# jatinagwal/kyverno

Measured on AMD Instinct MI355X. Metric: resource×rule evals/sec (background scan, PSS+best-practices) at 1/2/4/8 GPUs, higher is better.
Workload: dtype u32

## Files before the change

### __graft_entry__.py

```python
import os
import subprocess
import sys

ROOT = os.path.dirname(os.path.abspath(__file__))
if ROOT not in sys.path:
    sys.path.insert(0, ROOT)


def build():
    from kyverno_amd import build as B
    B.build()
    subprocess.run(["make", "-C", os.path.join(ROOT, "oracle"), "-j8"], check=True)
    import kyverno_amd
    from kyverno_amd import _lib
    _lib.lib()
    try:
        import concurrent.futures
        cache = os.path.join(ROOT, "kyverno_amd", "jitcache")
        jobs = [(wl, a) for wl in ("c3", "tests-c3", "c5", "c4", "c2") for a in (False, True)]
        try:
            sys.path.insert(0, os.path.join(ROOT, "tests"))
            import table_edge_cases
            jobs += [("tests-edges:%d" % i, False) for i in range(len(table_edge_cases.compiled_rulesets()))]
            import meta_keys_cases
            jobs += [("tests-metakeys%s:%d" % (off, i), a) for i in range(len(meta_keys_cases.compiled_rulesets()))
                     for off in ("", "-off") for a in (False, True)]
            import cond_preload_cases
            jobs += [("tests-condpre%s:%d" % (off, i), a) for i in range(len(cond_preload_cases.compiled_rulesets()))
                     for off in ("", "-off") for a in (False, True)]
            import pattern_vars_cases
            jobs += [("tests-patvars:%d" % i, False) for i in range(len(pattern_vars_cases.compiled_rulesets()))]
        except Exception as e:
            print("build: test rulesets not compiled ahead of time: %s" % e, file=sys.stderr)
        ctx = __import__("multiprocessing").get_context("spawn")
        with concurrent.futures.ProcessPoolExecutor(max_workers=min(len(jobs), os.cpu_count() or 1, 16), mp_context=ctx) as ex:
            list(ex.map(_aot_compile, jobs))
        t_start = {}
        ents = [f for f in os.listdir(cache) if f.endswith(".co")]
        for kind in ("walk", "acct"):
            newest = max((f for f in ents if f.startswith(kind + "-")), key=lambda f: os.path.getmtime(os.path.join(cache, f)))
            t_start[kind] = newest.split("-")[1]
        for f in os.listdir(cache):
            parts = f.split("-")
            if f.endswith(".co") and (len(parts) != 3 or t_start.get(parts[0]) != parts[1]):
                os.remove(os.path.join(cache, f))
    except Exception as e:
        print("build: ahead-of-time walk-kernel compile skipped: %s" % e, file=sys.stderr)
    try:
        _cache_bench_corpus()
    except Exception as e:
        print("build: bench corpus not prebuilt: %s" % e, file=sys.stderr)


def _cache_bench_corpus(total=10_000_000, need_free=14 << 30):
    import shutil
    import bench
    from kyverno_amd import synth
    if synth.corpus_is_cached(bench.CORPUS_CACHE, total, kind="mixed", seed=bench.SEED):
        return
    os.makedirs(bench.CORPUS_CACHE, exist_ok=True)
    free = shutil.disk_usage(bench.CORPUS_CACHE).free
    if free < need_free:
        raise RuntimeError("%.0f GB free under %s, %.0f GB wanted" % (free / 2**30, bench.CORPUS_CACHE, need_free / 2**30))
    synth.write_corpus_cache(bench.CORPUS_CACHE, total, kind="mixed", seed=bench.SEED)


def _aot_compile(job):
    if ROOT not in sys.path:
        sys.path.insert(0, ROOT)
    sys.path.insert(0, os.path.join(ROOT, "tests"))
    import bench
    import cases
    from kyverno_amd import engine as E
    wl, acct = job
    if wl.startswith("tests-edges:"):
        import table_edge_cases
        pols = table_edge_cases.compiled_rulesets()[int(wl.split(":")[1])]
    elif wl.startswith("tests-metakeys"):
        import meta_keys_cases
        pols = meta_keys_cases.compiled_rulesets()[int(wl.split(":")[1])]
        if wl.startswith("tests-metakeys-off:"):
            os.environ["KYV_META_KEYS"] = "0"
            try:
                return E.Ruleset(pols).jit_compile(accounting=acct)
            finally:
                del os.environ["KYV_META_KEYS"]
    elif wl.startswith("tests-patvars:"):
        import pattern_vars_cases
        pols = pattern_vars_cases.compiled_rulesets()[int(wl.split(":")[1])]
    elif wl.startswith("tests-condpre"):
        import cond_preload_cases
        pols = cond_preload_cases.compiled_rulesets()[int(wl.split(":")[1])]
        if wl.startswith("tests-condpre-off:"):
            os.environ["KYV_JC_PRELOAD"] = "0"
            try:
                return E.Ruleset(pols).jit_compile(accounting=acct)
            finally:
                del os.environ["KYV_JC_PRELOAD"]
    else:
        pols = cases.best_practices() + cases.chart_restricted() if wl == "tests-c3" else bench.load_policies(wl)
    return E.Ruleset(pols).jit_compile(accounting=acct)


def smoke():
    sys.path.insert(0, os.path.join(ROOT, "tests"))
    import cases
    import parity_util as PU
    from kyverno_amd import synth

    docs, nsl = synth.mixed(300, seed=5, edge=True)
    pols = cases.best_practices()[:4] + cases.chart_restricted()[:6] + cases.quirk_policies()[-2:]
    st, res = PU.compare(pols, docs, nsl, backend="gpu")
    if st["nbad"]:
        raise AssertionError("GPU verdicts differ from the oracle: %r" % (st["bad"][:5],))
    if st["compared"] == 0:
        raise AssertionError("smoke compared no pairs")
    print("smoke ok: %d pairs, %d compared bit-exact vs oracle, kernel %.3f ms" % (st["pairs"], st["compared"],
                                                                                   res.kernel_ms))


if __name__ == "__main__":
    build() if (len(sys.argv) > 1 and sys.argv[1] == "build") else smoke()
# ... 1 lines not shown
```

### include/kyvgpu.h

```cpp
#ifndef KYVGPU_H
#define KYVGPU_H

#include <stddef.h>
#include <stdint.h>

#ifdef __cplusplus
extern "C" {
#endif

#define KYV_ABI_VERSION 1u

typedef struct kyv_ruleset kyv_ruleset;
typedef struct kyv_batch kyv_batch;
typedef struct kyv_results kyv_results;

enum { KYV_OK = 0, KYV_EINVAL = 1, KYV_EPARSE = 2, KYV_EDEVICE = 3, KYV_EINTERNAL = 4, KYV_ERANGE = 5 };

enum {
  KYV_ST_NONE = 0,
  KYV_ST_PASS = 1,
  KYV_ST_FAIL = 2,
  KYV_ST_SKIP = 3,
  KYV_ST_ERROR = 4,
  KYV_ST_FALLBACK = 5,
// ... 59 lines not shown
  uint32_t path_template;
  uint16_t idx[4];
  uint32_t key[2];
} kyv_failure;

int kyv_ruleset_compile(const char* policies_json, size_t len, const kyv_compile_opts* opts, kyv_ruleset** out);
int kyv_ruleset_compile_ex(const char* policies_json, size_t len, const char* exceptions_json, size_t ex_len,
                           const kyv_compile_opts* opts, kyv_ruleset** out);
void kyv_ruleset_free(kyv_ruleset* rs);
uint32_t kyv_ruleset_num_rules(const kyv_ruleset* rs);
uint32_t kyv_ruleset_num_policies(const kyv_ruleset* rs);
int kyv_ruleset_rule_info(const kyv_ruleset* rs, uint32_t rule, kyv_rule_info* out);
int kyv_ruleset_policy_info(const kyv_ruleset* rs, uint32_t policy, kyv_policy_info* out);
int64_t kyv_ruleset_rule_kinds(const kyv_ruleset* rs, uint32_t rule, char* buf, size_t cap, int32_t* has_validate);
uint32_t kyv_ruleset_rule_flags(const kyv_ruleset* rs, uint32_t rule);
int64_t kyv_ruleset_jit_source(const kyv_ruleset* rs, char* buf, size_t cap, uint32_t* nrules_jit);
int kyv_ruleset_jit_compile(const kyv_ruleset* rs, double* seconds, size_t* code_bytes);
enum { KYV_JIT_ACCOUNTING = 1u };
int kyv_ruleset_jit_compile_ex(const kyv_ruleset* rs, uint32_t flags, double* seconds, size_t* code_bytes);

int kyv_batch_build(const kyv_ruleset* rs, const char* resources_json, size_t len, const char* ns_labels_json,
                    size_t ns_len, const kyv_batch_opts* opts, kyv_batch** out);
void kyv_batch_free(kyv_batch* b);
uint32_t kyv_batch_num_resources(const kyv_batch* b);
int kyv_batch_stats_get(const kyv_batch* b, kyv_batch_stats* out);
typedef struct kyv_wave_facts_out {
  uint32_t* facts; size_t facts_cap;
  uint32_t* hot; size_t hot_cap;
  uint32_t* order; size_t order_cap;
  char* bits; size_t bits_cap;
  size_t bits_len;
} kyv_wave_facts_out;
int kyv_batch_wave_facts(const kyv_batch* b, kyv_wave_facts_out* out);
typedef struct kyv_shape_keys_out {
  uint64_t* keys; size_t keys_cap;
  char* paths; size_t paths_cap;
  size_t paths_len;
} kyv_shape_keys_out;
int kyv_batch_shape_keys(const kyv_batch* b, kyv_shape_keys_out* out);
typedef struct kyv_meta_keys_out {
  uint32_t* rows; size_t rows_cap;
  char* desc; size_t desc_cap;
  size_t desc_len;
  uint32_t classes;
} kyv_meta_keys_out;
int kyv_batch_meta_keys(const kyv_batch* b, int device, kyv_meta_keys_out* out);

int kyv_col_entries_fit32(uint64_t entries);

int kyv_eval(const kyv_ruleset* rs, const kyv_batch* b, const kyv_eval_opts* opts, kyv_results** out);
void kyv_results_free(kyv_results* r);
int kyv_results_status(const kyv_results* r, uint8_t* out, size_t cap);
int64_t kyv_results_count(const kyv_results* r, int status);
int kyv_results_rule_counts(const kyv_results* r, int64_t* out, size_t cap);
double kyv_results_kernel_ms(const kyv_results* r);
double kyv_results_batch_ms(const kyv_results* r, int what);
int kyv_results_phase_ms(const kyv_results* r, double* out, size_t cap);
int kyv_results_jit(const kyv_results* r);
typedef struct {
  uint32_t gmask_patterns, cond_sets, gmask_words, unmasked_literals;
  uint32_t onemask;
  uint32_t tail_used[5], tail_candidates[5];
  uint32_t fast_records, fasteval_records, generic_rules;
  uint32_t slices;
} kyv_eval_plan;
typedef struct {
// ... 51 lines not shown
```

### kyverno_amd/_lib.py

```python
import ctypes
import os

HERE = os.path.dirname(os.path.abspath(__file__))
LIB_PATH = os.environ.get("KYV_LIB") or os.path.join(HERE, "libkyvgpu.so")

KYV_ABI_VERSION = 1
BACKEND_GPU, BACKEND_CPU = 0, 1
EVAL_NO_COPYBACK = 1
EVAL_ACCOUNT_BYTES = 2
EVAL_JIT_OFF = 4
EVAL_JIT_ON = 8
EVAL_SERIAL = 16

ST_NONE, ST_PASS, ST_FAIL, ST_SKIP, ST_ERROR, ST_FALLBACK, ST_PANIC, ST_ND = range(8)
STATUS_NAMES = ["none", "pass", "fail", "skip", "error", "fallback", "panic", "nondeterministic"]
RULE_KINDS = {1: "pattern", 2: "anyPattern", 3: "podSecurity", 4: "fallback", 5: "panic", 6: "error", 7: "deny",
              8: "foreach"}
RULE_USES_OPERATION = 1
TEXT_MESSAGE, TEXT_PATH = 0, 1


class CompileOpts(ctypes.Structure):
    _fields_ = [("abi_version", ctypes.c_uint32), ("flags", ctypes.c_uint32)]

# ... 9 lines not shown

class RuleInfo(ctypes.Structure):
    _fields_ = [("name", ctypes.c_char_p), ("policy", ctypes.c_uint32), ("kind", ctypes.c_int32), ("reason", ctypes.c_char_p)]


class PolicyInfo(ctypes.Structure):
    _fields_ = [("name", ctypes.c_char_p), ("namespace_", ctypes.c_char_p), ("first_rule", ctypes.c_uint32),
                ("nrules", ctypes.c_uint32), ("apply_one", ctypes.c_int32), ("scored_false", ctypes.c_int32)]


class Failure(ctypes.Structure):
    _fields_ = [("res", ctypes.c_uint32), ("rule", ctypes.c_uint32), ("alt", ctypes.c_uint32),
                ("path_template", ctypes.c_uint32), ("idx", ctypes.c_uint16 * 4), ("key", ctypes.c_uint32 * 2)]


class BatchStats(ctypes.Structure):
    _fields_ = [("resources", ctypes.c_uint64), ("nodes", ctypes.c_uint64), ("strings", ctypes.c_uint64),
                ("heap_bytes", ctypes.c_uint64), ("device_bytes", ctypes.c_uint64)]


EXPORTS = [
    "kyv_ruleset_compile", "kyv_ruleset_free", "kyv_ruleset_num_rules", "kyv_ruleset_num_policies",
    "kyv_ruleset_rule_info", "kyv_ruleset_policy_info", "kyv_batch_build", "kyv_batch_free",
    "kyv_batch_num_resources", "kyv_batch_stats_get", "kyv_eval", "kyv_results_free", "kyv_results_status",
    "kyv_results_count", "kyv_results_kernel_ms", "kyv_results_alg_bytes", "kyv_results_message", "kyv_results_path",
    "kyv_results_pss_mask", "kyv_last_error", "kyv_version", "kyv_results_jit", "kyv_ruleset_jit_source",
    "kyv_ruleset_jit_compile", "kyv_ruleset_jit_compile_ex", "kyv_results_rule_counts", "kyv_ruleset_compile_ex", "kyv_ruleset_rule_kinds",
    "kyv_results_fallback_reason", "kyv_results_pss_checks", "kyv_results_failures", "kyv_ruleset_rule_flags",
    "kyv_results_texts", "kyv_results_phase_ms", "kyv_results_alg_bytes_phase", "kyv_results_alg_bytes_class", "kyv_batch_export_status", "kyv_batch_copy_status",
    "kyv_batch_export_failures", "kyv_comm_unique_id", "kyv_comm_init", "kyv_comm_free", "kyv_comm_gather_results",
    "kyv_comm_gathered_status", "kyv_comm_gathered_failures", "kyv_comm_gather_report", "kyv_comm_reduce_counts", "kyv_results_batch_ms",
    "kyv_calibrate_fetch", "kyv_batch_wave_facts", "kyv_col_entries_fit32", "kyv_results_plan",
    "kyv_results_plan_slices", "kyv_batch_shape_keys", "kyv_batch_meta_keys",
]


class WaveFactsOut(ctypes.Structure):
    _fields_ = [("facts", ctypes.c_void_p), ("facts_cap", ctypes.c_size_t), ("hot", ctypes.c_void_p),
                ("hot_cap", ctypes.c_size_t), ("order", ctypes.c_void_p), ("order_cap", ctypes.c_size_t),
                ("bits", ctypes.c_void_p), ("bits_cap", ctypes.c_size_t), ("bits_len", ctypes.c_size_t)]


class ShapeKeysOut(ctypes.Structure):
    _fields_ = [("keys", ctypes.c_void_p), ("keys_cap", ctypes.c_size_t), ("paths", ctypes.c_void_p),
                ("paths_cap", ctypes.c_size_t), ("paths_len", ctypes.c_size_t)]


class MetaKeysOut(ctypes.Structure):
    _fields_ = [("rows", ctypes.c_void_p), ("rows_cap", ctypes.c_size_t), ("desc", ctypes.c_void_p),
                ("desc_cap", ctypes.c_size_t), ("desc_len", ctypes.c_size_t), ("classes", ctypes.c_uint32)]


class EvalPlan(ctypes.Structure):
    _fields_ = [("gmask_patterns", ctypes.c_uint32), ("cond_sets", ctypes.c_uint32), ("gmask_words", ctypes.c_uint32),
                ("unmasked_literals", ctypes.c_uint32), ("onemask", ctypes.c_uint32),
                ("tail_used", ctypes.c_uint32 * 5), ("tail_candidates", ctypes.c_uint32 * 5),
                ("fast_records", ctypes.c_uint32), ("fasteval_records", ctypes.c_uint32),
                ("generic_rules", ctypes.c_uint32), ("slices", ctypes.c_uint32)]


class SlicePlan(ctypes.Structure):
    _fields_ = [("k0", ctypes.c_uint32), ("k1", ctypes.c_uint32), ("fused_rules", ctypes.c_uint32),
                ("chunk_rules", ctypes.c_uint32), ("cond_rules", ctypes.c_uint32)]


class GatherStats(ctypes.Structure):
    _fields_ = [("status_ms", ctypes.c_double), ("failures_ms", ctypes.c_double),
                ("status_bytes_per_rank", ctypes.c_uint64), ("failure_rows_per_rank_max", ctypes.c_uint64),
                ("failure_rows_total", ctypes.c_uint64)]

_lib = None


# ... 26 lines not shown
    L.kyv_batch_copy_status.argtypes = [vp, ctypes.c_int, ctypes.c_uint64, ctypes.c_uint64, vp, sz]
    L.kyv_batch_copy_status.restype = i64
    L.kyv_batch_export_failures.argtypes = [vp, ctypes.c_int, i64, vp, sz, vp]
    L.kyv_batch_export_failures.restype = i64
    L.kyv_comm_unique_id.argtypes = [vp, sz]
    L.kyv_comm_init.argtypes = [vp, sz, ctypes.c_int, ctypes.c_int, ctypes.c_int, ctypes.POINTER(vp)]
    L.kyv_comm_free.argtypes = [vp]
    L.kyv_comm_free.restype = None
    L.kyv_comm_gather_results.argtypes = [vp, vp, i64, ctypes.POINTER(GatherStats)]
    L.kyv_comm_gathered_status.argtypes = [vp, ctypes.c_int, vp, sz]
    L.kyv_comm_gathered_status.restype = i64
    L.kyv_comm_gathered_failures.argtypes = [vp, ctypes.c_int, vp, sz]
    L.kyv_comm_gathered_failures.restype = i64
    L.kyv_comm_gather_report.argtypes = [vp, vp, i64, ctypes.c_int, ctypes.POINTER(GatherStats)]
    L.kyv_comm_reduce_counts.argtypes = [vp, vp, vp, sz]
    L.kyv_comm_reduce_counts.restype = i64
    L.kyv_results_batch_ms.argtypes = [vp, ctypes.c_int]
    L.kyv_results_batch_ms.restype = ctypes.c_double
    L.kyv_ruleset_rule_flags.argtypes = [vp, u32]
    L.kyv_ruleset_rule_flags.restype = u32
    L.kyv_ruleset_free.argtypes = [vp]
    L.kyv_ruleset_num_rules.argtypes = [vp]
    L.kyv_ruleset_num_rules.restype = u32
    L.kyv_ruleset_num_policies.argtypes = [vp]
    L.kyv_ruleset_num_policies.restype = u32
    L.kyv_ruleset_rule_info.argtypes = [vp, u32, ctypes.POINTER(RuleInfo)]
    L.kyv_ruleset_policy_info.argtypes = [vp, u32, ctypes.POINTER(PolicyInfo)]
    L.kyv_batch_build.argtypes = [vp, ctypes.c_char_p, sz, ctypes.c_char_p, sz, ctypes.POINTER(BatchOpts), ctypes.POINTER(vp)]
    L.kyv_batch_free.argtypes = [vp]
    L.kyv_batch_num_resources.argtypes = [vp]
    L.kyv_batch_num_resources.restype = u32
    L.kyv_batch_stats_get.argtypes = [vp, ctypes.POINTER(BatchStats)]
    L.kyv_batch_wave_facts.argtypes = [vp, ctypes.POINTER(WaveFactsOut)]
    L.kyv_batch_shape_keys.argtypes = [vp, ctypes.POINTER(ShapeKeysOut)]
    L.kyv_batch_meta_keys.argtypes = [vp, ctypes.c_int, ctypes.POINTER(MetaKeysOut)]
    L.kyv_eval.argtypes = [vp, vp, ctypes.POINTER(EvalOpts), ctypes.POINTER(vp)]
    L.kyv_results_free.argtypes = [vp]
    L.kyv_results_status.argtypes = [vp, ctypes.c_void_p, sz]
    L.kyv_results_rule_counts.argtypes = [vp, vp, ctypes.c_size_t]
    L.kyv_results_rule_counts.restype = i32
    L.kyv_results_count.argtypes = [vp, i32]
    L.kyv_results_count.restype = i64
    L.kyv_results_kernel_ms.argtypes = [vp]
    L.kyv_results_kernel_ms.restype = ctypes.c_double
    L.kyv_calibrate_fetch.argtypes = [i32, ctypes.c_uint64, i32]
    L.kyv_calibrate_fetch.restype = ctypes.c_double
    L.kyv_col_entries_fit32.argtypes = [ctypes.c_uint64]
    L.kyv_col_entries_fit32.restype = i32
    L.kyv_results_plan.argtypes = [vp, ctypes.POINTER(EvalPlan)]
    L.kyv_results_plan_slices.argtypes = [vp, ctypes.c_void_p, sz]
    L.kyv_results_plan_slices.restype = i64
    L.kyv_results_alg_bytes.argtypes = [vp]
    L.kyv_results_alg_bytes.restype = ctypes.c_uint64
    L.kyv_results_message.argtypes = [vp, vp, vp, u32, u32, ctypes.c_char_p, sz]
    L.kyv_results_message.restype = i64
    L.kyv_results_path.argtypes = [vp, vp, vp, u32, u32, ctypes.c_char_p, sz]
    L.kyv_results_path.restype = i64
    L.kyv_results_alg_bytes_phase.argtypes = [vp, ctypes.c_void_p, sz]
    L.kyv_results_alg_bytes_phase.restype = i32
    L.kyv_results_alg_bytes_class.argtypes = [vp, ctypes.c_void_p, sz]
    L.kyv_results_alg_bytes_class.restype = i32
    L.kyv_results_phase_ms.argtypes = [vp, ctypes.c_void_p, sz]
    L.kyv_results_phase_ms.restype = i32
    L.kyv_results_texts.argtypes = [vp, vp, vp, u32, u32, u32, u32, i32, ctypes.c_void_p, sz, ctypes.c_void_p]
    L.kyv_results_texts.restype = i64
    L.kyv_results_pss_mask.argtypes = [vp, vp, u32, u32]
# ... 21 lines not shown
```

### kyverno_amd/csrc/batch.cpp

```cpp
#include <algorithm>
#include <cstdio>
#include <cstdlib>
#include <atomic>
#include <chrono>
#include <cstring>
#include <deque>
#include <emmintrin.h>
#include <memory>
#include <string_view>
#include <thread>
#include <unordered_set>

#include "kyv_host.h"
#include "kyv_pss.h"

namespace kyv {
using pj::T;
using pj::Value;

Batch::~Batch() {}

namespace {

template <class F>
// ... 1131 lines not shown
        for (size_t s2 = ns * k / nk; s2 < ns * (k + 1) / nk; s2++) {
          const std::string& x = b->dict.strs[s2];
          uint32_t bits = 0;
          for (size_t q = 0; q < rs->rxs.size(); q++) {
            const int m = rx_match(rs->rxs[q], (const uint8_t*)x.data(), x.size());
            if (m < 0) { bits = RX_FB; break; }
            if (m) bits |= 1u << q;
          }
          b->str_rx[s2] = bits;
        }
      });
      phase("regex");
    }
    if ((!b->str_upper.empty() && b->str_upper.size() != b->dict.strs.size()) ||
        (!b->str_rx.empty() && b->str_rx.size() != b->dict.strs.size()))
      throw std::runtime_error("internal: per-string JMESPath columns do not cover the dictionary");
    return b.release();
  } catch (std::exception& e) {
    if (err) *err = e.what();
    return nullptr;
  }
}

namespace {
struct Resolver {
  const Ruleset& rs;
  const std::vector<std::vector<std::pair<uint32_t, uint32_t>>>& kids;
  Node* R;
  uint64_t* colv;
  const uint32_t* col_off;
  uint32_t* next;
  const int8_t* space_bit;
  uint32_t notmaps = 0;
  uint64_t entry(uint32_t x) const {
    return ((uint64_t)R[x].a << 32) | ((uint64_t)node_type(R[x]) << COL_TYPE_SHIFT) | x;
  }
  static uint32_t find(const Node* R, const Node& m, uint32_t key) {
    uint32_t lo = m.a, hi = m.a + m.b;
    while (lo < hi) {
      uint32_t mid = (lo + hi) >> 1, k = node_key(R[mid]);
      if (k == key) return mid;
      if (k < key) lo = mid + 1; else hi = mid;
    }
    return NONE;
  }
  void go(uint32_t m, uint32_t t, uint32_t row) {
    const Ruleset::TrieNode& T = rs.trie[t];
    const Node mn = R[m];
    if (node_type(mn) == N_MAP) {
      const auto& K = kids[t];
      auto hit = [&](uint32_t x, uint32_t kid) {
        if (colv) colv[(size_t)col_off[rs.trie[kid].col] + row] = entry(x);
        go(x, kid, row);
      };
      if (mn.b <= 2 * K.size() + 4) {
        uint32_t a = mn.a, e = mn.a + mn.b;
        size_t j = 0;
        while (a < e && j < K.size()) {
          uint32_t k = node_key(R[a]);
          if (k < K[j].first) a++;
          else if (k > K[j].first) j++;
          else { hit(a, K[j].second); a++; j++; }
        }
      } else {
        for (auto& kv : K) {
          uint32_t x = find(R, mn, kv.first);
          if (x != NONE) hit(x, kv.second);
        }
      }
    } else if (node_type(mn) == N_ARR && T.star != NONE) {
      uint32_t space = rs.trie[T.star].rowspace;
      uint32_t base = next[space];
      next[space] += mn.b;
      if (colv) {
        R[m].c = base;
        colv[(size_t)col_off[T.lencol] + row] = (uint64_t)mn.b | ((uint64_t)base << 32);
        const size_t self = col_off[rs.trie[T.star].col];
        for (uint32_t i = 0; i < mn.b; i++) colv[self + base + i] = entry(mn.a + i);
      }
      if (space_bit[space] >= 0)
        for (uint32_t i = 0; i < mn.b; i++)
          if (node_type(R[mn.a + i]) != N_MAP) notmaps |= 1u << space_bit[space];
      for (uint32_t i = 0; i < mn.b; i++) go(mn.a + i, T.star, base + i);
    }
  }
// ... 57 lines not shown
}

void shape_keys(Batch& b, int threads) {
  b.shape_key.clear();
  const char* e = getenv("KYV_SHAPE_ORDER");
  if (e && atoi(e) == 0) return;
  const size_t n = b.hdr.size();
  b.shape_key.assign(n, 0);
  const ShapeWalk sw(*b.rs);
  if (!sw.nfields || n == 0) return;
  const size_t per = 4096;
  parallel_for((n + per - 1) / per, std::max(1, threads), [&](size_t k) {
    uint8_t len[SHAPE_KEY_MAX_NODES];
    for (size_t r = k * per, end = std::min(n, r + per); r < end; r++) {
      const ResHeader& h = b.hdr[r];
      if (h.nnodes >= (1u << COL_TYPE_SHIFT)) continue;
      memset(len, 0, sw.nfields);
      sw.go(b.nodes.data() + h.root, 0, 0, len);
      uint64_t key = 0;
      for (uint32_t f = 0; f < sw.nfields; f++) key = (key << SHAPE_KEY_BITS) | len[f];
      b.shape_key[r] = key;
    }
  });
}

void resolve_path_columns(Batch& b, int threads) {
  const Ruleset& rs = *b.rs;
  size_t n = b.hdr.size();
  uint32_t nsp = rs.nrowspaces;
  b.rs_rows.assign(nsp, 0);
  b.col_off.assign(rs.ncols, 0);
  b.colv.clear();
  b.facts.assign((n + 63) / 64, WaveFacts{0u});
  if (rs.ncols == 0 || n == 0) return;
  std::vector<int8_t> space_bit(nsp, -1);
  for (size_t i = 0; i < rs.fact_spaces.size(); i++) space_bit[rs.fact_spaces[i]] = (int8_t)i;
  int T = std::max(1, threads);
  std::vector<std::vector<std::pair<uint32_t, uint32_t>>> kids(rs.trie.size());
  for (size_t t = 0; t < rs.trie.size(); t++) {
    kids[t] = rs.trie[t].kids;
    std::sort(kids[t].begin(), kids[t].end());
  }
  size_t nch = std::min(n, (size_t)T * 8);
  std::vector<std::vector<uint32_t>> cnt(nch, std::vector<uint32_t>(nsp, 0));
  auto eligible = [&](const ResHeader& h) { return h.nnodes < (1u << COL_TYPE_SHIFT); };
  auto run = [&](bool fill, std::vector<std::vector<uint32_t>>& nexts) {
    std::atomic<size_t> nx{0};
    auto work = [&]() {
      for (;;) {
        size_t c = nx.fetch_add(1);
        if (c >= nch) break;
        size_t r0 = n * c / nch, r1 = n * (c + 1) / nch;
        for (size_t r = r0; r < r1; r++) {
          ResHeader& h = b.hdr[r];
          if (!eligible(h)) continue;
          Resolver rv{rs, kids, b.nodes.data() + h.root, fill ? b.colv.data() : nullptr, b.col_off.data(), nexts[c].data(),
                      space_bit.data()};
          rv.go(0, 0, (uint32_t)r);
          if (fill && rv.notmaps) __atomic_fetch_or(&b.facts[r / 64].maps, rv.notmaps, __ATOMIC_RELAXED);
        }
      }
    };
    std::vector<std::thread> th;
    for (int t = 0; t < T; t++) th.emplace_back(work);
    for (auto& t : th) t.join();
  };
  const auto tc0 = std::chrono::steady_clock::now();
  run(false, cnt);
  if (getenv("KYV_DEBUG_STATS"))
    fprintf(stderr, "[kyvgpu] flatten %-12s %8.1f ms (within path-cols)\n", "col-count",
            std::chrono::duration<double, std::milli>(std::chrono::steady_clock::now() - tc0).count());
  std::vector<std::vector<uint32_t>> base(nch, std::vector<uint32_t>(nsp, 0));
  std::vector<uint64_t> tot(nsp, 0);
  for (size_t c = 0; c < nch; c++)
    for (uint32_t s = 1; s < nsp; s++) {
      if (!col_entries_fit32(tot[s] + cnt[c][s])) throw std::runtime_error("path-column row space exceeds 2^32 rows; split the batch");
      base[c][s] = (uint32_t)tot[s];
      tot[s] += cnt[c][s];
    }
  b.rs_rows[0] = (uint32_t)n;
  for (uint32_t s = 1; s < nsp; s++) b.rs_rows[s] = (uint32_t)tot[s];
  uint64_t total = 0;
  for (uint32_t c = 0; c < rs.ncols; c++) {
    b.col_off[c] = (uint32_t)total;
    total += b.rs_rows[rs.col_rowspace[c]];
    if (!col_entries_fit32(total)) throw std::runtime_error("path columns exceed 2^32 entries; split the batch");
  }
  b.colv.resize(total + 1);
  {
    const size_t per = (1u << 20);
    parallel_for((total + per) / per, T, [&](size_t k) {
      size_t lo = k * per, hi = std::min<size_t>(total + 1, lo + per);
      std::fill(b.colv.begin() + lo, b.colv.begin() + hi, (uint64_t)NONE);
    });
  }
  if (getenv("KYV_DEBUG_STATS")) {
    fprintf(stderr, "[kyvgpu] path columns: %u columns, %u row spaces, %llu entries (rows:", rs.ncols, nsp,
            (unsigned long long)total);
    for (uint32_t sp = 0; sp < nsp; sp++) fprintf(stderr, " %u", b.rs_rows[sp]);
    fprintf(stderr, ")\n");
  }
  run(true, base);
  for (auto& h : b.hdr) if (!eligible(h)) h.flags |= RF_MAGIC;
  const uint32_t defined = rs.fact_spaces.size() >= 32 ? 0xFFFFFFFFu : (1u << rs.fact_spaces.size()) - 1u;
  for (auto& f : b.facts) f.maps = ~f.maps & defined;
}

uint32_t wave_maps_mask() {
  const char* e = getenv("KYV_FACT_MAPS");
  return e && atoi(e) == 0 ? 0u : 0xFFFFFFFFu;
}

std::string format_path(const Ruleset& rs, const Batch& b, uint32_t tmpl, const uint16_t* idx, const uint32_t* key) {
  if (tmpl == NONE) return "";
  const std::string& t = rs.templates[tmpl];
  std::string out;
  for (size_t i = 0; i < t.size(); i++) {
    if (t[i] == '\x01' && i + 1 < t.size()) { out += std::to_string(idx[t[i + 1] - '0']); i++; continue; }
    if (t[i] == '\x02' && i + 1 < t.size()) {
      uint32_t k = key[t[i + 1] - '0'];
      out += k < b.dict.strs.size() ? b.dict.strs[k] : std::string("?");
      i++;
      continue;
    }
    out += t[i];
  }
  return out;
}

}
```

### kyverno_amd/csrc/capi.cpp

```cpp
#include <algorithm>
#include <array>
#include <atomic>
#include <cstring>
#include <map>
#include <mutex>
#include <thread>
#include <sched.h>
#include <cstring>

#include "../../include/kyvgpu.h"
#include "kyv_host.h"

namespace kyv {
void eval_gpu(const Ruleset& rs, const Batch& b, int device, int iters, Results* out, double* kernel_ms_avg, bool copy_back,
              int jit_mode, bool account, bool serial);
void eval_cpu(const Ruleset& rs, const Batch& b, int threads, Results* out, bool account);
void free_device_images(Ruleset& rs, Batch* b);
std::string fallback_why(const Ruleset& rs, const Batch& b, uint32_t res, uint32_t rule);
bool pattern_error_text(const Ruleset& rs, const Batch& b, uint32_t res, uint32_t rule, uint32_t root, uint8_t* status,
                        std::string* path, std::string* text);
int64_t export_status(const Batch& b, int device, uint8_t* dst, size_t cap, void* stream);
int64_t export_failures(const Batch& b, int device, int64_t off, int64_t* dst, size_t cap_rows, void* stream);
int64_t copy_status(const Batch& b, int device, size_t res0, size_t n, uint8_t* host_dst, size_t cap);
int64_t export_report_rows(const Batch& b, int device, uint32_t* rows, uint32_t* wide, uint32_t* nwide_dev,
// ... 285 lines not shown
  };
  std::function<void(uint32_t, const std::string&)> go = [&](uint32_t t, const std::string& path) {
    const Ruleset::TrieNode& T = rs.trie[t];
    if (T.star != NONE) {
      const std::string p = path + (path.empty() ? "" : ",") + "\"[*]\"";
      space_path[rs.trie[T.star].rowspace] = p;
      go(T.star, p);
    }
    for (const auto& kv : T.kids) go(kv.second, path + (path.empty() ? "" : ",") + quote(rs.dict.strs[kv.first]));
  };
  if (!rs.trie.empty()) go(0, "");
  std::string js = "{\"maps\":[";
  for (size_t i = 0; i < rs.fact_spaces.size(); i++) js += (i ? ",[" : "[") + space_path[rs.fact_spaces[i]] + "]";
  return js + "]}";
}

int kyv_batch_wave_facts(const kyv_batch* b, kyv_wave_facts_out* out) {
  if (!b || !out) return fail(KYV_EINVAL, "null argument");
  try {
    const Batch& x = *b->b;
    const size_t n = x.hdr.size(), nw = (n + 63) / 64;
    if ((out->facts && out->facts_cap < nw) || (out->hot && out->hot_cap < 4 * n) || (out->order && out->order_cap < n))
      return fail(KYV_EINVAL, "buffer too small");
    if (out->facts) {
      const uint32_t m = wave_maps_mask();
      for (size_t w = 0; w < nw; w++) out->facts[w] = (w < x.facts.size() ? x.facts[w].maps : 0u) & m;
    }
    if (out->hot) {
      if (x.hot.size() != n) return fail(KYV_EINTERNAL, "batch has no hot header plane");
      memcpy(out->hot, x.hot.data(), n * sizeof(HotHdr));
    }
    if (out->order) for (size_t p = 0; p < n; p++) out->order[p] = p < x.order.size() ? x.order[p] : (uint32_t)p;
    const std::string js = wave_fact_bits_json(*x.rs);
    out->bits_len = js.size();
    if (out->bits) {
      if (out->bits_cap < js.size() + 1) return fail(KYV_EINVAL, "buffer too small");
      memcpy(out->bits, js.c_str(), js.size() + 1);
    }
    return KYV_OK;
  } catch (std::exception& e) {
    return fail(KYV_EINTERNAL, e.what());
  }
}

static std::string shape_key_paths_json(const Ruleset& rs, bool ordered) {
  const std::vector<uint32_t> nodes = shape_key_nodes(rs);
  std::vector<std::string> node_path(rs.trie.size());
  std::function<void(uint32_t, const std::string&)> go = [&](uint32_t t, const std::string& path) {
    const Ruleset::TrieNode& T = rs.trie[t];
    const std::string sep = path.empty() ? "" : ",";
    if (T.star != NONE) {
      node_path[t] = path + sep + "\"[*]\"";
      go(T.star, node_path[t]);
    }
    for (const auto& kv : T.kids) {
      std::string q = "\"";
      for (unsigned char ch : rs.dict.strs[kv.first]) {
        if (ch == '"' || ch == '\\') { q += '\\'; q += (char)ch; }
        else if (ch < 0x20) { char b[8]; snprintf(b, sizeof b, "\\u%04x", ch); q += b; }
        else q += (char)ch;
      }
      go(kv.second, path + sep + q + "\"");
    }
  };
  if (!rs.trie.empty()) go(0, "");
  std::string js = "{\"bits\":" + std::to_string(SHAPE_KEY_BITS) + ",\"ordered\":" + (ordered ? "true" : "false") + ",\"paths\":[";
// ... 1060 lines not shown
```

### kyverno_amd/csrc/compiler.cpp

```cpp
#include <algorithm>
#include <cmath>
#include <list>
#include <map>
#include <set>

#include "kyv_host.h"

namespace kyv {
using pj::T;
using pj::Value;

void seed_dict(Dict& d) {
  const char* fixed[] = {"", "0", "true", "false", "*"};
  for (const char* s : fixed) d.intern(s);
  const char* wk[] = {
#define KYV_WK_STR(id, s) s,
      KYV_WELL_KNOWN(KYV_WK_STR)
#undef KYV_WK_STR
  };
  for (const char* s : wk) d.intern(s);
  const char* vs[] = {
#define KYV_VS_STR(id) #id,
      KYV_VOLUME_SOURCES(KYV_VS_STR)
#undef KYV_VS_STR
// ... 2590 lines not shown
    set.erase(std::unique(set.begin(), set.end()), set.end());
    auto it = seen.find(set);
    if (it == seen.end()) {
      if (rs.gpats.size() + rs.gsets.size() >= MAX_GMASK) continue;
      it = seen.emplace(set, (uint32_t)rs.gsets.size()).first;
      rs.gsets.push_back(set);
    }
    rs.cond_set[ci] = it->second + 1;
  }
}

void build_path_trie(Ruleset& rs) {
  rs.trie.assign(1, Ruleset::TrieNode{});
  rs.ncols = 0;
  rs.nrowspaces = 1;
  rs.col_rowspace.clear();
  for (auto& E : rs.pentries) E.col = NONE;
  for (auto& P : rs.pnodes) P.flags &= (uint8_t)~PF_NEEDROW;
  rs.pn_self.assign(rs.pnodes.size(), NONE);
  rs.pe_self.assign(rs.pentries.size(), NONE);
  rs.pn_len.assign(rs.pnodes.size(), NONE);
  rs.pe_len.assign(rs.pentries.size(), NONE);
  TrieBuilder tb{rs, std::vector<uint32_t>(rs.pnodes.size(), TrieBuilder::UNSET)};
  for (auto& rd : rs.rules) {
    if (rd.kind == RK_PATTERN) tb.walk(rd.root, 0, 0);
    else if (rd.kind == RK_ANYPATTERN)
      for (uint32_t a = 0; a < rd.nalts; a++) tb.walk(rs.pool[rd.root + a], 0, 0);
  }
  for (auto& rd : rs.rules) tb.cond_rule(rd);
  for (auto& rd : rs.rules) tb.dyn_rule(rd);
  if (!getenv("KYV_PSS_NOCOLS"))
    for (auto& rd : rs.rules) tb.pss_rule(rd);
  assign_wave_facts(rs);
  assign_meta_classes(rs);
}

void assign_wave_facts(Ruleset& rs) {
  rs.fact_spaces.clear();
  std::set<uint32_t> spaces;
  for (size_t pn = 0; pn < rs.pnodes.size(); pn++) {
    const PNode& P = rs.pnodes[pn];
    if (rs.pn_self[pn] == NONE) continue;
    bool map_child = false;
    if (P.kind == P_ARR_MAPS) map_child = P.first < rs.pnodes.size() && rs.pnodes[P.first].kind == P_MAP;
    else if (P.kind == P_ARR_POS)
      for (uint32_t i = 0; i < P.n; i++) {
        const uint32_t ch = rs.pool[P.first + i];
        map_child = map_child || (ch < rs.pnodes.size() && rs.pnodes[ch].kind == P_MAP);
      }
    if (map_child) spaces.insert(rs.col_rowspace[rs.pn_self[pn]]);
  }
  for (uint32_t s2 : spaces) if (rs.fact_spaces.size() < FACT_BITS) rs.fact_spaces.push_back(s2);
}

void assign_meta_classes(Ruleset& rs) {
  rs.meta_classes.clear();
  rs.meta_class_of.assign(rs.metas.size(), (int8_t)-1);
  const uint32_t S = KSID(SPEC), T = KSID(TEMPLATE), J = KSID(JOBTEMPLATE);
  std::function<void(uint32_t, uint32_t, const uint32_t*, int)> walk = [&](uint32_t pn, uint32_t mbase, const uint32_t* k, int depth) {
    if (pn == NONE || pn >= rs.pnodes.size() || depth > 4) return;
    const PNode& P = rs.pnodes[pn];
    if (P.kind != P_MAP) return;
    const int pos = depth == 0 ? 0 : (depth == 2 && k[0] == S && k[1] == T) ? 1 :
                    (depth == 4 && k[0] == S && k[1] == J && k[2] == S && k[3] == T) ? 2 : -1;
    if ((P.flags & PF_META) && pos >= 0 && (size_t)mbase + P.meta < rs.metas.size()) {
      const MetaSite& ms = rs.metas[mbase + P.meta];
      const uint32_t nw = ms.nwild_l + ms.nwild_a;
      if (nw && ms.nwild_l <= 1 && ms.nwild_a <= 1 && nw <= (uint32_t)MAX_SLOTS) {
        MetaClass mc{};
        mc.pos = (uint32_t)pos;
        mc.site = ms;
        mc.site.slot_l = 0;
        mc.site.slot_a = ms.nwild_l;
        auto same = [&](const MetaClass& o) {
          if (o.pos != mc.pos || o.site.has_labels != ms.has_labels || o.site.has_ann != ms.has_ann ||
              o.site.nwild_l != ms.nwild_l || o.site.nwild_a != ms.nwild_a)
            return false;
          for (uint32_t i = 0; i < 2 * ms.nwild_l; i++) if (rs.pool[o.site.wild_l + i] != rs.pool[ms.wild_l + i]) return false;
          for (uint32_t i = 0; i < 2 * ms.nwild_a; i++) if (rs.pool[o.site.wild_a + i] != rs.pool[ms.wild_a + i]) return false;
          return true;
        };
        size_t c = 0;
        while (c < rs.meta_classes.size() && !same(rs.meta_classes[c])) c++;
        if (c == rs.meta_classes.size() && c < MAX_META_CLASSES) rs.meta_classes.push_back(mc);
        if (c < rs.meta_classes.size()) rs.meta_class_of[mbase + P.meta] = (int8_t)c;
// ... 22 lines not shown
```

### kyverno_amd/csrc/jit.cpp

```cpp
#include <dlfcn.h>
#include <sys/stat.h>
#include <unistd.h>
#include <hip/hip_runtime.h>
#include <hip/hiprtc.h>

#include <algorithm>
#include <chrono>
#include <cstdio>
#include <cstdlib>
#include <functional>
#include <map>
#include <mutex>
#include <utime.h>
#include <set>
#include <sstream>
#include <unordered_map>
#include <stdexcept>
#include <string>
#include <vector>

#include "kyv_host.h"

namespace kyv {

int pattern_depth(const Ruleset& rs, uint32_t pn, int guard);

bool jit_meta_keys_on() {
  const char* e = getenv("KYV_META_KEYS");
  return !e || atoi(e) != 0;
}

int jit_jc_chains_mode() {
  const char* e = getenv("KYV_JC_PRELOAD");
  return e ? (atoi(e) != 0) : jit_meta_keys_on() ? 1 : 0;
}

namespace {

struct Gen {
  const Ruleset& rs;
  std::ostringstream out;
  std::vector<uint8_t> emitted;
  std::vector<uint32_t> emitted_log;
  bool ok = true;
  const bool use_len = !getenv("KYV_JIT_LEN") || atoi(getenv("KYV_JIT_LEN")) != 0;
  const size_t batch_max = getenv("KYV_JIT_BATCH") ? (size_t)std::max(1, atoi(getenv("KYV_JIT_BATCH"))) : 1;
  const bool leaf_fast = !getenv("KYV_JIT_LEAF_FAST") || atoi(getenv("KYV_JIT_LEAF_FAST")) != 0;
  const bool meta_keys;
  static constexpr uint32_t MK_COL = 0x80000000u;
  struct WildSrc { int pc = -1; bool two = false; uint32_t cs = 0; };
  std::vector<int> slot_meta;
  std::vector<WildSrc> wild_src;
  WildSrc cur_src[MAX_SLOTS];
  int class_of(uint32_t pn) const {
    const PNode& P = rs.pnodes[pn];
    if (!meta_keys || !(P.flags & PF_META) || node_mbase[pn] == NONE || meta_pos[pn] < 0) return -1;
    const size_t s = (size_t)node_mbase[pn] + P.meta;
    return s < rs.meta_class_of.size() ? rs.meta_class_of[s] : -1;
  }

  std::vector<int> slot;
  std::vector<int> slot_alen;
  std::vector<int> slot_elen;
  std::vector<std::vector<uint32_t>> scope_of;
  std::vector<uint8_t> scoped;
  std::vector<uint32_t> node_mbase;
  std::vector<int8_t> meta_pos;

  explicit Gen(const Ruleset& r, int meta_keys_mode = -1)
      : rs(r), meta_keys(meta_keys_mode < 0 ? jit_meta_keys_on() : meta_keys_mode != 0), emitted(r.pnodes.size(), 0), slot_meta(r.pnodes.size(), -1), wild_src(r.pentries.size()),
        slot(r.pentries.size(), -1), slot_alen(r.pnodes.size(), -1),
        slot_elen(r.pentries.size(), -1), scope_of(r.pnodes.size()), scoped(r.pnodes.size(), 0),
        node_mbase(r.pnodes.size(), NONE), meta_pos(r.pnodes.size(), -1) {}

  void mark_paths(uint32_t pn, uint32_t mbase, uint32_t k0, uint32_t k1, uint32_t k2, uint32_t k3, int depth) {
    if (pn == NONE || pn >= rs.pnodes.size() || depth > 4) return;
    const PNode& P = rs.pnodes[pn];
    if (P.kind != P_MAP) return;
    node_mbase[pn] = mbase;
    const uint32_t S = SID_FIRST_FREE + K_SPEC, T = SID_FIRST_FREE + K_TEMPLATE, J = SID_FIRST_FREE + K_JOBTEMPLATE;
    if (depth == 0) meta_pos[pn] = 0;
    else if (depth == 2 && k0 == S && k1 == T) meta_pos[pn] = 1;
    else if (depth == 4 && k0 == S && k1 == J && k2 == S && k3 == T) meta_pos[pn] = 2;
    for (uint32_t e = 0; e < P.n; e++) {
      const PEntry& E = rs.pentries[P.first + e];
      if ((E.flags & EF_WILD) || E.child == NONE || E.handler == H_STAR || E.handler == H_NEGATION ||
          E.handler == H_EXISTENCE || E.handler == H_EXIST_BADPAT)
        continue;
      const uint32_t k[4] = {k0, k1, k2, k3};
      uint32_t nk[4] = {k[0], k[1], k[2], k[3]};
      if (depth < 4) nk[depth] = E.key;
      mark_paths(E.child, mbase, nk[0], nk[1], nk[2], nk[3], depth + 1);
    }
  }

  int add(std::vector<uint32_t>& list, uint32_t col) {
    list.push_back(col);
    return (int)list.size() - 1;
  }
  void collect(uint32_t pn, std::vector<uint32_t>& list, int guard) {
    if (pn == NONE || pn >= rs.pnodes.size() || guard > 4 * MAX_DEPTH) return;
    const PNode& P = rs.pnodes[pn];
    if (P.kind == P_ARR_MAPS || P.kind == P_ARR_POS || P.kind == P_ARR_SCALAR) {
      if (rs.pn_len[pn] != NONE && use_len) {
        if (slot_alen[pn] >= 0) { ok = false; return; }
        slot_alen[pn] = add(list, rs.pn_len[pn]);
// ... 31 lines not shown
  }
  void scope(uint32_t root) {
    if (root == NONE || root >= rs.pnodes.size() || scoped[root]) return;
    scoped[root] = 1;
    for (auto& c : cur_src) c = WildSrc{};
    collect(root, scope_of[root], 0);
  }
  void scopes_below(uint32_t pn, int guard) {
    if (pn == NONE || pn >= rs.pnodes.size() || guard > 4 * MAX_DEPTH) return;
    const PNode& P = rs.pnodes[pn];
    switch (P.kind) {
      case P_MAP:
        for (uint32_t e = 0; e < P.n; e++) {
          const PEntry& E = rs.pentries[P.first + e];
          if (E.handler == H_STAR || E.handler == H_NEGATION || E.handler == H_EXIST_BADPAT || E.child == NONE) continue;
          if (E.handler == H_EXISTENCE) {
            for (uint32_t j = 0; j < rs.pool[E.child]; j++) {
              scope(rs.pool[E.child + 1 + j]);
              scopes_below(rs.pool[E.child + 1 + j], guard + 1);
            }
          } else {
            scopes_below(E.child, guard + 1);
          }
        }
        break;
      case P_ARR_MAPS: scope(P.first); scopes_below(P.first, guard + 1); break;
      case P_ARR_POS:
        for (uint32_t i = 0; i < P.n; i++) { scope(rs.pool[P.first + i]); scopes_below(rs.pool[P.first + i], guard + 1); }
        break;
      default: break;
    }
  }
  const std::vector<uint32_t>& scope_cols(uint32_t root) { scope(root); return scope_of[root]; }
  std::string preload(uint32_t root, const std::string& name, const std::string& rowx, const char* rd = "jself(w, ") {
    scope(root);
    const auto& L = scope_of[root];
    std::ostringstream o;
    o << "uint64_t " << name << "[" << std::max<size_t>(1, L.size()) << "];";
    for (size_t i = 0; i < L.size(); i++) {
      if (L[i] & MK_COL) { o << meta_load(L, i, name, rowx); continue; }
      o << " " << name << "[" << i << "] = " << rd << u(L[i]) << ", " << rowx << ");";
    }
    return o.str();
  }
  static std::string meta_load(const std::vector<uint32_t>& L, size_t i, const std::string& name, const std::string& rowx) {
    if (L[i] & 1u) return std::string();
    std::ostringstream o;
    o << " { const kyv_u32x4 mq = jc_meta(v, " << u((L[i] & ~MK_COL) >> 1) << ", " << rowx << "); " << name << "[" << i
      << "] = (uint64_t)mq.x | ((uint64_t)mq.y << 32); " << name << "[" << i + 1 << "] = (uint64_t)mq.z | ((uint64_t)mq.w << 32); }";
    return o.str();
  }

  static std::string u(uint32_t x) { return std::to_string(x) + "u"; }
  static std::string i64(int64_t x) { return "(int64_t)" + std::to_string(x) + "ll"; }

  uint32_t cur_root = NONE;
  uint32_t cur_dyn = NONE;
  std::string dyn_sig(uint32_t dyn) const {
    std::ostringstream o;
    const uint32_t n = rs.pool[dyn];
    uint32_t at = dyn + 1;
    for (uint32_t q = 0; q < n; q++) {
      o << (q ? "; " : "") << "column " << rs.pool[at + 1] << " keys";
      for (uint32_t s = 0; s < rs.pool[at]; s++) o << " " << rs.pool[at + 2 + s];
      at += 2 + rs.pool[at];
    }
    return o.str();
  }
  std::string dyn_preload(uint32_t dyn) const {
    if (dyn == NONE) return std::string();
    std::ostringstream o;
    const uint32_t n = std::min(rs.pool[dyn], MAX_DYN);
    uint32_t at = dyn + 1;
    o << "  uint64_t dq[" << n << "];";
// ... 386 lines not shown
                << (rs.pe_self[P.first + e] != NONE ? "        ei = jdec(jself(w, " + u(rs.pe_self[P.first + e]) + ", er), &et, &ea);\n"
                                                      : std::string())
                << "        if (ei == NONE) { ei = aa + i; et = T_UNK; }\n"
                << "        Ret r = p" << rs.pool[E.child + 1 + j] << "(w, ei, et, ea, er, pe);\n"
                << "        if (w.ost) return r;\n"
                << "        if (!r.err) { hit = true; break; }\n"
                << "      }\n"
                << "      if (!hit) return mkerr(EC_NONE, 0, " << ET << "); }\n";
          }
          out << "  }\n";
          break;
        }
        default:
          out << "  {\n";
          call("");
          out << "  }\n";
      }
    }
    out << "  return ok_ret();\n";
  }
};

struct CondGen {
  const Ruleset& rs;
  std::ostringstream defs;
  std::ostringstream out;
  bool ok = true;
  uint32_t uid = 0;
  uint32_t nslots = 1;
  bool lds_used = false;
  uint32_t cur_etpos = NONE;
  std::unordered_map<uint64_t, std::string> progs;

  CondGen(const Ruleset& r, int mode) : rs(r), chains(mode < 0 ? jit_jc_chains_mode() != 0 : mode != 0) {}
  static std::string u(uint32_t x) { return std::to_string(x) + "u"; }
  std::string fresh(const char* p) { return std::string(p) + std::to_string(uid++); }

  uint32_t tchild(uint32_t t, uint32_t key) const {
    if (t == NONE) return NONE;
    for (auto& kv : rs.trie[t].kids) if (kv.first == key) return kv.second;
    return NONE;
  }
  uint32_t tstar(uint32_t t) const { return t == NONE ? NONE : rs.trie[t].star; }
  uint32_t tcol(uint32_t t) const { return t == NONE ? NONE : rs.trie[t].col; }
  uint32_t tlen(uint32_t t) const { return t == NONE || rs.trie[t].star == NONE ? NONE : rs.trie[t].lencol; }

  struct V {
    std::string i, t, a, row;
    uint32_t tpos;
    bool key;
    std::vector<uint32_t> lz;
  };
  const bool chains;
  V force(const V& x) {
    if (x.lz.empty()) return x;
    V y{fresh("vi"), fresh("vt"), fresh("va"), x.row, x.tpos, false, {}};
    out << "  uint32_t " << y.i << ", " << y.t << ", " << y.a << ";\n"
        << "  if (" << x.row << " != NONE) jc_field_e(jc_col(v, " << u(tcol(x.tpos)) << ", " << x.row << "), &" << y.i << ", &"
        << y.t << ", &" << y.a << ");\n"
        << "  else {\n    " << y.i << " = " << x.i << ";\n";
    for (uint32_t key : x.lz)
      out << "    jc_field(v, R, " << y.i << ", NONE, NONE, " << u(key) << ", &" << y.i << ", &" << y.t << ", &" << y.a << ");\n";
    out << "  }\n";
    return y;
  }
  V decl(const std::string& i, const std::string& t, const std::string& a, const std::string& row, uint32_t tpos,
         bool key) {
    V x{fresh("vi"), fresh("vt"), fresh("va"), fresh("vr"), tpos, key};
    out << "  uint32_t " << x.i << " = " << i << ", " << x.t << " = " << t << ", " << x.a << " = " << a << ", " << x.row
        << " = " << row << ";\n";
    return x;
  }
  V field(const V& x0, uint32_t key) {
    if (x0.key) return decl("NONE", "T_UNK", "0u", "NONE", NONE, false);
    if (chains && tcol(tchild(x0.tpos, key)) != NONE) {
      V y = x0;
      y.tpos = tchild(x0.tpos, key);
      y.lz.push_back(key);
      return y;
    }
    const V x = force(x0);
    const uint32_t ct = tchild(x.tpos, key), col = tcol(ct);
    V y{fresh("vi"), fresh("vt"), fresh("va"), fresh("vr"), col == NONE ? NONE : ct, false};
    out << "  uint32_t " << y.i << ", " << y.t << ", " << y.a << ";\n"
        << "  jc_field(v, R, " << x.i << ", " << x.row << ", " << (col == NONE ? "NONE" : u(col)) << ", " << u(key) << ", &"
        << y.i << ", &" << y.t << ", &" << y.a << ");\n"
        << "  const uint32_t " << y.row << " = " << (col == NONE ? std::string("NONE") : x.row) << ";\n";
    return y;
  }
  bool unroll = false;
  V open_elems(const V& x, const std::string& notarr_then, const char* on_arr = "") {
    const std::string cnt = fresh("cn"), aa = fresh("aa"), eb = fresh("eb"), j = fresh("j");
    const uint32_t st = tstar(x.tpos);
    out << "  { uint32_t " << cnt << " = 0u, " << aa << " = 0u, " << eb << " = NONE;\n"
        << "  if (" << (x.key ? "false" : "jc_arr(v, R, " + x.i + ", " + x.t + ", " + x.a + ", " + x.row + ", " +
                                              (tlen(x.tpos) == NONE ? std::string("NONE") : u(tlen(x.tpos))) + ", &" + cnt +
                                              ", &" + aa + ", &" + eb + ")")
        << ") {\n" << on_arr << (unroll ? "  KYV_JC_UNROLL\n" : "")
        << "  for (uint32_t " << j << " = 0; " << j << " < " << cnt << "; " << j << "++) {\n";
    V e{fresh("vi"), fresh("vt"), fresh("va"), fresh("vr"), st, false};
    out << "  uint32_t " << e.i << ", " << e.t << ", " << e.a << ", " << e.row << ";\n"
        << "  jc_elem(v, R, " << aa << ", " << (st == NONE ? std::string("NONE") : eb) << ", " << j << ", "
        << (tcol(st) == NONE ? std::string("NONE") : u(tcol(st))) << ", &" << e.i << ", &" << e.t << ", &" << e.a << ", &"
        << e.row << ");\n";
    pending_else.push_back(notarr_then);
    return e;
  }
  std::vector<std::string> pending_else;
  void close_loop() {
    out << "  }\n  }";
    std::string e = pending_else.back();
    pending_else.pop_back();
    if (!e.empty()) out << " else {\n" << e << "  }";
    out << "\n  }\n";
  }

  const uint32_t* P = nullptr;
  uint32_t PN = 0, PEND = 0;
  bool streaming = false;
  std::string sacc;
  void jend(const V& x, bool list, bool proj) {
    if (!list) {
      out << "  *cur = " << (x.key ? "(" + x.i + " | JMES_KEYBIT)" : x.i) << ";\n";
      return;
    }
    if (streaming) {
      std::string sx;
      if (x.key) sx = "(gtk(R + " + x.i + ") >> 4)";
// ... 71 lines not shown
            << "  { const Node " << m << " = gnode(R + " << x.i << ");\n  *lst = true;\n"
            << "  for (uint32_t " << j << " = 0; " << j << " < " << m << ".b; " << j << "++) {\n";
        V k = decl(m + ".a + " + j, "T_UNK", "0u", "NONE", NONE, true);
        jgen(pos + 1, k, true, proj, guard + 1);
        out << "  }\n  }\n";
        return;
      }
      case JO_KEYS_FLAT: {
        if (!list) { jgen(pos + 1, x, false, proj, guard + 1); return; }
        const std::string m = fresh("mn"), j = fresh("j");
        out << "  if (" << (x.key ? std::string("true") : x.i + " == NONE || jc_type(R, " + x.i + ", " + x.t + ") != N_MAP")
            << ") return JS_FB;\n"
            << "  { const Node " << m << " = gnode(R + " << x.i << ");\n"
            << "  KYV_JC_UNROLL\n"
            << "  for (uint32_t " << j << " = 0; " << j << " < " << m << ".b; " << j << "++) {\n";
        V k = decl(m + ".a + " + j, "T_UNK", "0u", "NONE", NONE, true);
        jgen(pos + 1, k, true, true, guard + 1);
        out << "  }\n  }\n";
        return;
      }
      default: ok = false; return;
    }
  }
  std::string operand_fn(const CondOperand& o, uint32_t etpos) {
    const uint32_t* p = rs.pool.data() + o.a;
    const uint32_t n = o.nseg, root = p[0] & 0xFFu;
    const bool pure = (p[0] & JF_PURE) != 0;
    const std::string name = fresh("jo");
    const uint32_t* saveP = P;
    const uint32_t savePEND = PEND;
    std::ostringstream save;
    save.swap(out);
    out << "static __device__ __forceinline__ int " << name
        << "(const View& v, const Node* R, uint32_t r, uint32_t ei, uint32_t et, uint32_t ea, uint32_t erow, uint32_t* L, "
           "bool* lst, uint32_t* cur, uint32_t* ln, uint32_t* lit) {\n"
           "  *lst = false; *cur = NONE; *ln = 0u; *lit = NONE;\n";
    uint32_t i = 1, orlit = NONE;
    if (root == JR_OPERATION) {
      uint32_t lit = p[1];
      if (n > 2 && p[2] == JO_OR) {
        const Node& c = rs.cnodes[lit];
        bool f = node_type(c) == N_NULL || node_type(c) == N_FALSE || (node_type(c) == N_STR && c.a == SID_EMPTY) ||
                 ((node_type(c) == N_ARR || node_type(c) == N_MAP) && c.b == 0);
        if (f) lit = p[3];
      } else if (n > 2) {
        ok = false;
      }
      out << "  *lit = " << u(lit) << ";\n  return JS_OK;\n}\n";
    } else if (pure) {
      out << "  uint32_t c = " << (root == JR_OBJECT ? "0u" : "ei") << ", f = 0u;\n";
      for (; i + 1 < n; i += 2) {
        if (p[i] != JO_FIELD) { ok = false; break; }
        out << "  if (c != NONE) {\n"
               "    const Node m = gnode(R + c);\n"
               "    if (node_type(m) != N_MAP) c = NONE;\n"
               "    else { const uint32_t x = wmap_find(R, m.a, m.b, " << u(p[i + 1]) << ");\n"
               "      if (x == NONE) { *lit = f; return JS_NOTFOUND; }\n"
               "      c = (gtk(R + x) & 0xFu) == N_NULL ? NONE : x; }\n"
               "  }\n  f++;\n";
      }
      out << "  *cur = c;\n  return JS_OK;\n}\n";
    } else {
      V x = root == JR_OBJECT ? decl("0u", "T_UNK", "0u", "r", 0u, false) : decl("ei", "et", "ea", "erow", etpos, false);
      PEND = n;
      for (uint32_t q = 1; q < n;) {
        if (p[q] == JO_OR) { PEND = q; orlit = p[q + 1]; if (q + 2 < n) ok = false; break; }
        if (p[q] == JO_UPPER || p[q] == JO_REGEX) ok = false;
        q += jop_width(p + q);
      }
      P = p;
      const bool su = unroll;
      unroll = true;
      jgen(1, x, false, false, 0);
      unroll = su;
      if (orlit != NONE)
        out << "  if (*lst ? *ln == 0u : jc_false1(R, *cur)) { *lst = false; *cur = NONE; *lit = " << u(orlit) << "; }\n";
      out << "  return JS_OK;\n}\n";
    }
    std::string fn = out.str();
    out.swap(save);
    defs << fn;
    P = saveP;
    PEND = savePEND;
    return name;
  }
  std::string stream_fn(const CondOperand& o, uint32_t etpos, const std::string& acc) {
    const uint32_t* p = rs.pool.data() + o.a;
    const uint32_t n = o.nseg, root = p[0] & 0xFFu;
    if (root == JR_OPERATION || (p[0] & JF_PURE) || jmes_chain_form(p, n)) return "";
    const std::string name = fresh("js");
    const uint32_t* saveP = P;
    const uint32_t savePEND = PEND;
    std::ostringstream save;
    save.swap(out);
    out << "static __device__ __forceinline__ int " << name
        << "(const View& v, const Node* R, uint32_t r, uint32_t ei, uint32_t et, uint32_t ea, uint32_t erow, "
           "bool* lst, uint32_t* cur, uint32_t* ln, uint32_t* lit, uint32_t* sm, uint32_t* sf) {\n"
           "  *lst = false; *cur = NONE; *ln = 0u; *lit = NONE; (void)sm; (void)sf;\n";
    V x = root == JR_OBJECT ? decl("0u", "T_UNK", "0u", "r", 0u, false) : decl("ei", "et", "ea", "erow", etpos, false);
    uint32_t orlit = NONE;
    PEND = n;
    for (uint32_t q = 1; q < n;) {
      if (p[q] == JO_OR) { PEND = q; orlit = p[q + 1]; break; }
      q += jop_width(p + q);
    }
    P = p;
    const bool su = unroll, ss = streaming;
    const std::string sa = sacc;
    unroll = true;
    streaming = true;
    sacc = acc;
    jgen(1, x, false, false, 0);
    unroll = su;
    streaming = ss;
    sacc = sa;
    if (orlit != NONE)
      out << "  if (*lst ? *ln == 0u : jc_false1(R, *cur)) { *lst = false; *cur = NONE; *lit = " << u(orlit) << "; }\n";
    out << "  return JS_OK;\n}\n";
    std::string fn = out.str();
    out.swap(save);
    P = saveP;
    PEND = savePEND;
    if (!ok) return "";
    defs << fn;
    return name;
  }
  std::unordered_map<uint32_t, std::string> set_names;
  std::string set_array(uint32_t q) {
    auto it = set_names.find(q);
    if (it != set_names.end()) return it->second;
    std::string nm = "kyv_cset" + std::to_string(q);
    defs << "__device__ const uint32_t " << nm << "[" << rs.gsets[q].size() << "] = {";
    for (size_t i = 0; i < rs.gsets[q].size(); i++) defs << (i ? ", " : "") << rs.gsets[q][i] << "u";
    defs << "};\n";
    set_names[q] = nm;
    return nm;
  }
  bool stream_cond(uint32_t ci, const std::string& K, const std::string& X) {
    if (ci >= rs.cond_set.size() || !rs.cond_set[ci] || getenv("KYV_JIT_NOSTREAM")) return false;
    const Cond& c = rs.conds[ci];
    const uint32_t q = rs.cond_set[ci] - 1;
    const uint32_t bit = (uint32_t)rs.gpats.size() + q;
    const bool shapeA = c.key.kind == OK_JMES && c.value.kind == OK_LIT;
    const CondOperand& lo = shapeA ? c.key : c.value;
    const std::string S = set_array(q);
    const std::string test = "jc_inset(v, " + u(bit) + ", " + S + ", " + u((uint32_t)rs.gsets[q].size()) + ", es)";
    const std::string acc = shapeA ? "if (es == NONE) *sf = 1u; else if (" + test + ") (*sm)++;"
                                   : "if (!*sf) { if (es == NONE) *sf = 2u; else if (" + test + ") *sf = 1u; }";
    const std::string f = stream_fn(lo, cur_etpos, acc);
    if (f.empty()) return false;
    const std::string l = fresh("jl"), cc = fresh("jc"), n = fresh("jn"), t = fresh("jt"), s = fresh("js"), m = fresh("sm"),
                      fb = fresh("sf");
    out << "  bool " << l << "; uint32_t " << cc << ", " << n << ", " << t << ", " << m << " = 0u, " << fb << " = 0u;\n"
        << "  const int " << s << " = " << f << "(v, R, r, ei, et, ea, erow, &" << l << ", &" << cc << ", &" << n << ", &" << t
        << ", &" << m << ", &" << fb << ");\n"
        << "  if (" << s << " == JS_FB) return CR_FB;\n  if (" << s << " == JS_NOTFOUND) return CP_ERROR;\n"
        << "  if (" << l << ") {\n";
    if (shapeA) {
      std::string dec;
      switch (c.op) {
        case CO_ANYIN: dec = m + " > 0u"; break;
        case CO_ANYNOTIN: dec = m + " < " + n; break;
        case CO_ALLIN: dec = m + " == " + n; break;
        default: dec = m + " == 0u"; break;
      }
      out << "    rc = " << fb << " ? CR_FB : (" << dec << ") ? CR_TRUE : CR_FALSE;\n";
    } else {
      const bool neg = c.op == CO_NOTIN || c.op == CO_ANYNOTIN || c.op == CO_ALLNOTIN;
      out << "    rc = " << fb << " == 2u ? CR_FB : ((" << fb << " == 1u) != " << (neg ? "true" : "false")
          << ") ? CR_TRUE : CR_FALSE;\n";
    }
    out << "  } else {\n";
    const std::string one = "jc_cv(v, R, false, " + cc + ", " + t + ", nullptr, 0u)";
    if (shapeA) out << "    const CV " << K << " = " << one << ";\n    const CV " << X << " = jc_lit(v, " << u(c.value.a) << ");\n";
    else out << "    const CV " << K << " = jc_lit(v, " << u(c.key.a) << ");\n    const CV " << X << " = " << one << ";\n";
    out << "    rc = " << cond_call(ci, K, X) << ";\n  }\n";
    return true;
  }

  bool infallible(const CondOperand& o) const {
    if (o.kind == OK_LIT || o.kind == OK_NIL) return true;
    if (o.kind == OK_PATH) return false;
    const uint32_t* p = rs.pool.data() + o.a;
    const uint32_t root = p[0] & 0xFFu;
    if (root == JR_OPERATION) return true;
    if (p[0] & JF_PURE) return false;
    for (uint32_t q = 1; q < o.nseg;) {
// ... 8 lines not shown
    const uint32_t* p = rs.pool.data() + o.a;
    for (uint32_t q = 1; q < o.nseg;) {
      if (p[q] == JO_MULTI || p[q] == JO_FLAT || p[q] == JO_KEYS || p[q] == JO_KEYS_FLAT || p[q] == JO_FILTER) return true;
      if (p[q] == JO_OR) return false;
      q += jop_width(p + q);
    }
    return false;
  }
  void operand_cv(const CondOperand& o, uint32_t ci, int side, uint32_t etpos, const std::string& cv, const std::string& slot,
                  bool check) {
    const std::string C = "v.conds[" + u(ci) + "]." + (side ? "value" : "key");
    switch (o.kind) {
      case OK_LIT: out << "  const CV " << cv << " = jc_lit(v, " << u(o.a) << ");\n"; return;
      case OK_PATH: {
        const std::string m = fresh("ms");
        out << "  CV " << cv << "; uint32_t " << m << ";\n"
            << "  " << (check ? "if (!" : "(void)(") << "cv_operand(v, NodeTab{R}, " << C << ", &" << cv << ", &" << m << ", r)"
            << (check ? ") return CP_ERROR;\n" : ");\n");
        return;
      }
      case OK_JMES: {
        if (jmes_chain_form(rs.pool.data() + o.a, o.nseg)) {
          const std::string m = fresh("ms"), s = fresh("js");
          out << "  CV " << cv << "; uint32_t " << m << ";\n"
              << "  const int " << s << " = jmes_chain_cv(v, NodeTab{R}, " << C << ", &" << cv << ", &" << m << ", r);\n";
          if (check) out << "  if (" << s << " == JS_FB) return CR_FB;\n  if (" << s << " != JS_OK) return CP_ERROR;\n";
          else out << "  (void)" << s << ";\n";
          return;
        }
        lds_used = true;
        const std::string f = operand_fn(o, etpos);
        const std::string l = fresh("jl"), c = fresh("jc"), n = fresh("jn"), t = fresh("jt"), s = fresh("js");
        out << "  bool " << l << "; uint32_t " << c << ", " << n << ", " << t << ";\n"
            << "  const int " << s << " = " << f << "(v, R, r, ei, et, ea, erow, " << slot << ", &" << l << ", &" << c
            << ", &" << n << ", &" << t << ");\n";
        if (check) out << "  if (" << s << " == JS_FB) return CR_FB;\n  if (" << s << " == JS_NOTFOUND) return CP_ERROR;\n";
        else out << "  (void)" << s << ";\n";
        out << "  const CV " << cv << " = jc_cv(v, R, " << l << ", " << c << ", " << t << ", " << slot << ", " << n << ");\n";
        return;
      }
      default: out << "  const CV " << cv << " = cv_node(Node{N_NULL, 0, 0, 0}, false);\n"; return;
    }
  }
  static std::string opnd_init(const CondOperand& o) {
    return "{" + std::to_string(o.kind) + ", " + std::to_string(o.sv) + ", " + std::to_string(o.nseg) + ", " + u(o.a) +
           ", " + u(o.list) + ", " + u(o.nlist) + "}";
  }
  std::string cond_call(uint32_t ci, const std::string& K, const std::string& X) {
    const Cond& c = rs.conds[ci];
    const std::string C = "Cond{" + std::to_string(c.op) + ", {0, 0, 0}, " + u(c.leaf) + ", " + u(c.leaf_neg) + ", 0u, " +
                          opnd_init(c.key) + ", " + opnd_init(c.value) + "}";
    const std::string a = "v, NodeTab{R}, " + C + ", " + K + ", " + X;
    switch (c.op) {
      case CO_EQ: return "op_equal(v, NodeTab{R}, " + K + ", " + X + ", false)";
      case CO_NE: return "op_equal(v, NodeTab{R}, " + K + ", " + X + ", true)";
      case CO_IN: return "op_in(" + a + ", false)";
      case CO_NOTIN: return "op_in(" + a + ", true)";
      case CO_ANYIN: return "op_any_all(" + a + ", false, false)";
      case CO_ALLIN: return "op_any_all(" + a + ", true, false)";
      case CO_ANYNOTIN: return "op_any_all(" + a + ", false, true)";
      case CO_ALLNOTIN: return "op_any_all(" + a + ", true, true)";
      case CO_GT: case CO_GE: case CO_LT: case CO_LE:
        return "op_numeric(v, " + K + ", " + X + ", " + std::to_string(c.op) + ")";
      case CO_DGT: case CO_DGE: case CO_DLT: case CO_DLE:
        return "op_duration(v, " + K + ", " + X + ", " + std::to_string(c.op) + ")";
      default: return "CR_FALSE";
    }
// ... 28 lines not shown
      out << "  rc = " << cond_call(ci, K, X) << ";\n";
    };
    out << "  int rc = CR_TRUE;\n  (void)rc;\n";
    if (!fused) {
      for (uint32_t ci : cis) {
        const Cond& c = rs.conds[ci];
        for (int side = 0; side < 2; side++) {
          const CondOperand& o = side ? c.value : c.key;
          if (infallible(o)) continue;
          out << "  {\n";
          operand_cv(o, ci, side, etpos, fresh("pc"), "L", true);
          out << "  }\n";
        }
      }
    }
    if (p.nany != NONE) {
      out << "  { bool any = false;\n  do {\n";
      for (uint32_t i = 0; i < nany; i++) {
        out << "  {\n";
        cond_code(p.any0 + i, fused);
        out << "  if (rc == CR_FB || rc == CR_PANIC) return rc;\n  if (rc == CR_TRUE) { any = true; break; }\n  }\n";
      }
      out << "  } while (0);\n  if (!any) return CR_FALSE; }\n";
    }
    for (uint32_t i = 0; i < p.nall; i++) {
      out << "  {\n";
      cond_code(p.all0 + i, fused);
      out << "  if (rc == CR_FB || rc == CR_PANIC) return rc;\n  if (rc == CR_FALSE) return CR_FALSE;\n  }\n";
    }
    out << "  return CR_TRUE;\n";
    const std::string b = out.str();
    out.swap(save);
    defs << "static __device__ __forceinline__ int " << name
         << "(const View& v, const Node* R, uint32_t r, uint32_t ei, uint32_t et, uint32_t ea, uint32_t erow, uint32_t* L) {\n"
         << "  (void)ei; (void)et; (void)ea; (void)erow;\n"
         << b << "}\n";
    progs[key] = name;
    return name;
  }

  const ForeachEntry* FE = nullptr;
  void elem_body(const V& e) {
    out << "  do {\n";
    if (FE->scope == 2) out << "  if (jc_type(R, " << e.i << ", " << e.t << ") != N_MAP) return ST_ERROR | ST_MARK_SCOPE;\n";
    out << "  bool err = false;\n";
    const std::string args = "(v, R, r, " + e.i + ", " + e.t + ", " + e.a + ", " + e.row + ", L)";
    if (FE->pre != NONE) {
      const std::string f = prog_fn(FE->pre, e.tpos);
      out << "  { const int c = " << f << args << ";\n"
          << "    if (c == CR_FB) return ST_FALLBACK;\n    if (c == CR_PANIC) return ST_PANIC;\n"
          << "    if (c == CR_FALSE) break;\n    err = c == CP_ERROR; }\n";
    }
    const std::string f = prog_fn(FE->deny, e.tpos);
    out << "  if (!err) { const int c = " << f << args << ";\n"
        << "    if (c == CR_FB) return ST_FALLBACK;\n    if (c == CR_PANIC) return ST_PANIC;\n"
        << "    if (c == CR_TRUE) return ST_FAIL;\n    if (c != CP_ERROR) { count++; break; } }\n"
        << "  pend = true;\n  } while (0);\n";
  }
  void fend(const V& x, bool list, bool proj) {
    if (x.key) { ok = false; return; }
    if (list) {
      if (proj) {
        out << "  if (" << x.i << " != NONE) {\n  pend = false;\n";
        elem_body(x);
        out << "  }\n";
      } else {
        out << "  pend = false;\n  if (" << x.i << " != NONE) {\n";
        elem_body(x);
        out << "  }\n";
      }
      return;
    }
    std::ostringstream save;
    save.swap(out);
    out << "  pend = false;\n  if (" << (x.i == "NONE" ? std::string("false") : x.i + " != NONE && jc_type(R, " + x.i + ", " + x.t + ") != N_NULL")
        << ") {\n";
    elem_body(x);
    out << "  }\n";
    const std::string single = out.str();
// ... 91 lines not shown
    } else {
      ok = false;
      return;
    }
    out << "  if (pend) return ST_ERROR;\n  applied += count; }\n";
  }

  bool kind_only(const RuleDesc& rd) const {
    if (rd.empty_may_match || rd.exclude.mode != MM_NONE || rd.exc != NONE) return false;
    const MatchBlock& m = rd.match;
    if (m.mode == MM_NONE || m.nfilters == 0 || (m.mode != MM_ANY && m.nfilters != 1)) return false;
    for (uint32_t i = 0; i < m.nfilters; i++) {
      const Filter& f = rs.filters[m.filters + i];
      if (f.nkinds == 0 || f.name != NONE || f.nnames || f.nnss || f.nann ||
          (f.flags & (FF_HAS_SEL | FF_HAS_NSSEL | FF_ZERO_RD | FF_USERINFO)))
        return false;
      for (uint32_t j = 0; j < f.nkinds; j++) {
        const KindDesc& kd = rs.kinds[f.kinds + j];
        if (kd.kind != NONE && kd.gv_mode != 0) return false;
      }
    }
    return true;
  }
  void rule_fn(uint32_t k) {
    const RuleDesc& rd = rs.rules[k];
    std::ostringstream save;
    save.swap(out);
    if (kind_only(rd)) out << "  // match block = the kind gate (checked by the kernel)\n";
    else out << "  { const int m = jc_match(v, r, " << u(k) << "); if (m >= 0) return (uint8_t)m; }\n";
    out << "#ifdef KYV_EXP_JC_EMPTY\n  return ST_PASS;\n#endif\n";
    out << "  if (hnn >= (1u << COL_TYPE_SHIFT)) return ST_FALLBACK;  // no path columns for this resource\n"
        << "  const Node* R = v.nodes + hroot;\n"
        << "  const uint32_t ei = NONE, et = T_UNK, ea = 0u, erow = NONE;\n";
    const std::string args = "(v, R, r, ei, et, ea, erow, L)";
    if (rd.pre != NONE) {
      const std::string f = prog_fn(rd.pre, NONE);
      out << "  { const int c = " << f << args << ";\n"
          << "    if (c == CR_FB) return ST_FALLBACK;\n    if (c == CR_PANIC) return ST_PANIC;\n"
          << "    if (c == CP_ERROR) return ST_ERROR | ST_MARK_PRE;\n    if (c == CR_FALSE) return ST_SKIP | ST_MARK_PRE; }\n";
    }
    if (rd.kind == RK_DENY) {
      const std::string f = prog_fn(rd.root, NONE);
      out << "  { const int c = " << f << args << ";\n"
          << "    if (c == CR_FB) return ST_FALLBACK;\n    if (c == CR_PANIC) return ST_PANIC;\n"
          << "    if (c == CP_ERROR) return ST_ERROR;\n    return c == CR_TRUE ? ST_FAIL : ST_PASS; }\n";
    } else if (rd.kind == RK_FOREACH) {
      const uint32_t nent = rs.pool[rd.root];
      std::vector<ForeachEntry> ents(nent);
      bool deny_only = true;
      for (uint32_t e = 0; e < nent; e++) {
        memcpy(&ents[e], rs.pool.data() + rd.root + 1 + e * (sizeof(ForeachEntry) / 4), sizeof(ForeachEntry));
        deny_only = deny_only && ents[e].kind == FE_DENY;
      }
      if (deny_only) {
        out << "  uint32_t applied = 0u;\n";
        for (uint32_t e = 0; e < nent && ok; e++) foreach_entry(ents[e]);
        out << "  return applied ? ST_PASS : ST_SKIP;\n";
      } else {
        out << "  (void)ei; (void)et; (void)ea; (void)erow; (void)L;\n"
            << "  return eval_foreach(v, NodeTab{R}, v.rules[" << u(k) << "], r);\n";
      }
    } else {
      ok = false;
    }
    const std::string b = out.str();
    out.swap(save);
    defs << "static __device__ __forceinline__ uint8_t jr" << k << "(const View& v, uint32_t r, uint32_t hroot, uint32_t hnn, uint32_t* L) {\n" << b << "}\n";
  }
};

static bool heavy_jmes(const Ruleset& rs, const CondOperand& o) {
  return o.kind == OK_JMES && !jmes_chain_form(rs.pool.data() + o.a, o.nseg);
}
bool prog_has_jmes(const Ruleset& rs, uint32_t prog) {
  if (prog == NONE) return false;
  const CondProg& p = rs.cprogs[prog];
  const uint32_t nany = p.nany == NONE ? 0u : p.nany;
  for (uint32_t i = 0; i < nany; i++)
    if (heavy_jmes(rs, rs.conds[p.any0 + i].key) || heavy_jmes(rs, rs.conds[p.any0 + i].value)) return true;
  for (uint32_t i = 0; i < p.nall; i++)
    if (heavy_jmes(rs, rs.conds[p.all0 + i].key) || heavy_jmes(rs, rs.conds[p.all0 + i].value)) return true;
  return false;
}

std::string self_dir() {
  Dl_info info;
  if (dladdr((void*)&self_dir, &info) && info.dli_fname) {
    std::string p = info.dli_fname;
    size_t s = p.rfind('/');
    return s == std::string::npos ? std::string(".") : p.substr(0, s);
  }
  return ".";
}

}

constexpr uint32_t kFusedGW = 8;
bool jit_rule_fused(const Ruleset& rs, uint32_t k) {
  static const bool on = !getenv("KYV_FUSED") || atoi(getenv("KYV_FUSED")) != 0;
  if (!on || k >= rs.rules.size() || rs.rules.size() > 32u * kFusedGW) return false;
  const RuleDesc& rd = rs.rules[k];
  return (rd.kind == RK_PATTERN || rd.kind == RK_ANYPATTERN) && (rd.flags & RD_GATE_EXACT);
}

bool jit_shape_eligible(const Ruleset& rs, uint32_t k) {
  static const bool on = !getenv("KYV_SHAPES") || atoi(getenv("KYV_SHAPES")) != 0;
  if (!on || k >= rs.rules.size()) return false;
  const RuleDesc& rd = rs.rules[k];
  return rd.kind == RK_PATTERN && rd.pre == NONE && !(rd.flags & RD_GATE_EXACT) && !jit_rule_fused(rs, k);
}

static std::string meta_signature(const Ruleset& rs, const RuleDesc& rd) {
  std::string o;
  if (!rd.uses_meta) return o;
  auto pool = [&](uint32_t at, uint32_t n) {
    for (uint32_t i = 0; i < 2 * n && at + i < rs.pool.size(); i++) o += std::to_string(rs.pool[at + i]) + ",";
  };
  for (uint32_t i = 0; i < rd.nmeta && rd.meta_sites + i < rs.metas.size(); i++) {
    const MetaSite& m = rs.metas[rd.meta_sites + i];
    o += "[" + std::to_string(m.has_labels) + "," + std::to_string(m.has_ann) + "," + std::to_string(m.nwild_l) + ":";
    pool(m.wild_l, m.nwild_l);
    o += std::to_string(m.nwild_a) + ":";
    pool(m.wild_a, m.nwild_a);
    o += std::to_string(m.slot_l) + "," + std::to_string(m.slot_a) + "]";
  }
  return o;
}

std::string jit_source(const Ruleset& rs, std::vector<uint8_t>* jit_rules, std::vector<uint8_t>* jit_cond,
                       std::vector<uint16_t>* jit_shape, int meta_keys, int jc_chains) {
  Gen g(rs, meta_keys);
  jit_rules->assign(rs.rules.size(), 0);
  if (jit_shape) jit_shape->assign(rs.rules.size(), 0);
  if (jit_cond) jit_cond->assign(rs.rules.size(), 0);
  const size_t cap = getenv("KYV_JIT_MAX_RULES") ? (size_t)atol(getenv("KYV_JIT_MAX_RULES")) : 1024;
  CondGen cg(rs, jc_chains);
  std::vector<uint32_t> crules;
  const bool cond_on = !getenv("KYV_JIT_COND") || atoi(getenv("KYV_JIT_COND")) != 0;
  for (size_t k = 0; k < rs.rules.size() && cond_on && crules.size() < cap; k++) {
    const RuleDesc& rd = rs.rules[k];
    if (rd.kind != RK_DENY && rd.kind != RK_FOREACH) continue;
    if (rd.kind == RK_DENY && !prog_has_jmes(rs, rd.pre) && !prog_has_jmes(rs, rd.root)) continue;
    const std::string mark = cg.defs.str();
    const auto progs = cg.progs;
    cg.ok = true;
    cg.rule_fn((uint32_t)k);
    if (!cg.ok) {
      cg.defs.str("");
      cg.defs.clear();
      cg.defs << mark;
      cg.progs = progs;
      continue;
    }
    crules.push_back((uint32_t)k);
  }
  std::vector<std::pair<uint32_t, std::vector<uint32_t>>> rule_roots;
  std::ostringstream body;
  std::unordered_map<std::string, uint32_t> shapes;
  std::unordered_map<uint32_t, uint32_t> rep_of;
  std::unordered_map<uint32_t, uint32_t> root_dyn;
  auto dyn_of = [&](uint32_t r) { auto it = root_dyn.find(r); return it == root_dyn.end() ? NONE : it->second; };
  auto canon = [](const std::string& t) {
    std::unordered_map<std::string, size_t> ids;
    std::string o;
    o.reserve(t.size());
    for (size_t i = 0; i < t.size();) {
      if (t[i] == 'p' && (i == 0 || !(isalnum((unsigned char)t[i - 1]) || t[i - 1] == '_')) && i + 1 < t.size() &&
          isdigit((unsigned char)t[i + 1])) {
        size_t j = i + 1;
// ... 156 lines not shown
      (*jit_rules)[rule_roots[i].first] = (uint8_t)(gi + 1);
      const bool f = jit_rule_fused(rs, rule_roots[i].first);
      if (f) fused.push_back(i);
      for (uint32_t r : rule_roots[i].second) { roots.push_back(r); if (!f) chunk_roots.push_back(r); }
    }
    static const int forder = getenv("KYV_FUSED_ORDER") ? atoi(getenv("KYV_FUSED_ORDER")) : 0;
    if (forder) {
      std::map<size_t, std::pair<std::vector<uint32_t>, std::vector<uint32_t>>> key;
      for (size_t i : fused) {
        KindGate kg = rule_gate(rs, rs.rules[rule_roots[i].first]);
        std::sort(kg.kinds.begin(), kg.kinds.end());
        if (kg.any) kg.kinds.clear();
        std::set<uint32_t> cols;
        for (uint32_t r : rule_roots[i].second) {
          g.scope(rep_of[r]);
          for (uint32_t c : g.scope_of[rep_of[r]]) cols.insert(c);
        }
        std::vector<uint32_t> cv(cols.begin(), cols.end());
        key[i] = forder == 2 ? std::make_pair(cv, kg.kinds) : std::make_pair(kg.kinds, cv);
      }
      std::stable_sort(fused.begin(), fused.end(), [&](size_t a, size_t b) { return key[a] < key[b]; });
      if (forder == 3) {
        const size_t np = std::max<size_t>(1, std::min<size_t>(fused.size(), getenv("KYV_FUSED_SPLIT") ? (size_t)atoi(getenv("KYV_FUSED_SPLIT")) : 3));
        std::vector<size_t> dealt;
        for (size_t p = 0; p < np; p++)
          for (size_t j = p; j < fused.size(); j += np) dealt.push_back(fused[j]);
        fused.swap(dealt);
      }
    }
    for (uint32_t r : roots)
      if (rep_of[r] == r)
      src << "static __device__ __forceinline__ void root" << r
          << "(const View& v, const Node* R, const ResHeader* hp, uint32_t row, uint32_t mbase, bool rootmap, bool walk,\n"
             "    PatOut& out, const uint32_t am) {\n"
             "  " << g.preload(r, "pc", "row", "jc_col(v, ") << "\n"
          << g.dyn_preload(dyn_of(r)) <<
             "  if (!walk) return;\n"
             "#ifdef KYV_EXP_JIT_PRELOAD\n  { uint64_t x = 0; for (auto q : pc) x ^= q; out.status = x == 0x123456789ull ? ST_FAIL : ST_PASS; return; }\n#endif\n"
          << g.dyn_decode(dyn_of(r)) <<
             "  JW w{v, R, hp, 0ull, 0ull, Keys{NONE, NONE}, 0ull, mbase, (uint8_t)ST_NONE, am" << (dyn_of(r) != NONE ? ", dv" : "") << "};\n"
             "  Ret r = p" << r << "(w, 0u, rootmap ? (uint32_t)N_MAP : T_UNK, 0u, row, pc);\n"
             "  jfinish(w, r, out);\n"
             "}\n";
    static const uint32_t cc_max = getenv("KYV_COLCACHE") ? (uint32_t)std::max(0, atoi(getenv("KYV_COLCACHE"))) : 4u;
    std::map<uint32_t, uint32_t> cslot;
    std::map<size_t, std::vector<uint32_t>> rule_cols;
    uint32_t ncslots = 0;
    if (cc_max && !fused.empty()) {
      std::map<uint32_t, size_t> cnt;
      std::map<uint32_t, std::set<uint32_t>> ckinds;
      std::set<uint32_t> call;
      for (size_t i : fused) {
        std::set<uint32_t> cols;
        for (uint32_t r : rule_roots[i].second) {
          g.scope(rep_of[r]);
          for (uint32_t c : g.scope_of[rep_of[r]]) cols.insert(c);
        }
        rule_cols[i].assign(cols.begin(), cols.end());
        const KindGate kg = rule_gate(rs, rs.rules[rule_roots[i].first]);
        for (uint32_t c : cols) {
          cnt[c]++;
          if (kg.any || kg.kinds.empty()) call.insert(c);
          else ckinds[c].insert(kg.kinds.begin(), kg.kinds.end());
        }
      }
      std::vector<uint32_t> cand;
      for (const auto& e : cnt) if (e.second >= 2 && !(e.first & Gen::MK_COL)) cand.push_back(e.first);
      std::stable_sort(cand.begin(), cand.end(), [&](uint32_t a, uint32_t b) { return cnt[a] > cnt[b]; });
      std::vector<std::vector<uint32_t>> slots;
      for (uint32_t c : cand) {
        for (uint32_t s = 0; s < cc_max; s++) {
          if (s == slots.size()) slots.emplace_back();
          bool ok = true;
          for (uint32_t c2 : slots[s]) {
            if (call.count(c) || call.count(c2)) ok = false;
            else for (uint32_t kk : ckinds[c]) if (ckinds[c2].count(kk)) { ok = false; break; }
            if (!ok) break;
          }
          if (ok) { slots[s].push_back(c); cslot[c] = s; break; }
        }
      }
      ncslots = (uint32_t)slots.size();
      if (cslot.empty()) ncslots = 0;
    }
    if (ncslots) {
      std::set<uint32_t> reps;
      for (size_t i : fused) for (uint32_t r : rule_roots[i].second) reps.insert(rep_of[r]);
      for (uint32_t r : reps) {
        const auto& L = g.scope_of[r];
        src << "static __device__ __forceinline__ void rootc" << r << "_" << gi
            << "(const View& v, const Node* R, const ResHeader* hp, uint32_t row, uint32_t mbase, bool rootmap, bool walk,\n"
               "    PatOut& out, const uint64_t* jcc, const uint32_t am) {\n"
               "  const uint32_t lane = threadIdx.x & 63u;\n"
               "  (void)lane;\n"
               "  uint64_t pc[" << std::max<size_t>(1, L.size()) << "];";
        for (size_t i = 0; i < L.size(); i++) {
          auto it = cslot.find(L[i]);
          if (it != cslot.end()) src << " pc[" << i << "] = jcc[" << it->second * 64u << "u + lane];";
          else if (L[i] & Gen::MK_COL) src << Gen::meta_load(L, i, "pc", "row");
          else src << " pc[" << i << "] = jc_col(v, " << Gen::u(L[i]) << ", row);";
        }
        src << "\n"
            << g.dyn_preload(dyn_of(r)) <<
               "  if (!walk) return;\n"
            << g.dyn_decode(dyn_of(r)) <<
               "  JW w{v, R, hp, 0ull, 0ull, Keys{NONE, NONE}, 0ull, mbase, (uint8_t)ST_NONE, am" << (dyn_of(r) != NONE ? ", dv" : "") << "};\n"
               "  Ret r = p" << r << "(w, 0u, rootmap ? (uint32_t)N_MAP : T_UNK, 0u, row, pc);\n"
               "  jfinish(w, r, out);\n"
               "}\n";
      }
    }
    if (roots.size() > 256) {
      std::map<uint32_t, std::vector<uint32_t>> br2;
      for (uint32_t r : roots) br2[rep_of[r]].push_back(r);
      std::vector<uint16_t> tab(rs.pnodes.size(), 0xFFFF);
      uint16_t si = 0;
      for (auto& b : br2) { for (uint32_t r : b.second) tab[r] = si; si++; }
      src << "__device__ const unsigned short kyv_shape" << gi << "[" << std::max<size_t>(1, tab.size()) << "] = {";
      for (size_t i = 0; i < tab.size(); i++) src << (i ? "," : "") << tab[i];
      src << "};\n";
    }
    src << "struct JitWalker" << gi << " {\n"
           "  bool rootmap;\n"
           "  uint32_t am;\n"
           "  __device__ __forceinline__ void run(const View& v, uint32_t root, bool walk, const Node* R, const ResHeader* hp,\n"
           "                                     uint32_t row, const RuleDesc& rd, PatOut& out) {\n"
           "    out.status = ST_NONE; out.idx = 0; out.tmpl = NONE; out.key0 = NONE; out.key1 = NONE;\n"
           "#ifdef KYV_EXP_JIT_EMPTY\n    if (walk) out.status = ST_PASS; return;\n#endif\n"
           << (roots.size() <= 256 ? std::string("    switch (root) {\n") : "    switch (root < " + std::to_string(rs.pnodes.size()) +
                                                                "u ? (uint32_t)kyv_shape" + std::to_string(gi) +
                                                                "[root] : 0xFFFFu) {\n");
    std::map<uint32_t, std::vector<uint32_t>> by_rep;
    for (uint32_t r : chunk_roots) by_rep[rep_of[r]].push_back(r);
    if (roots.size() <= 256) {
      for (auto& br : by_rep) {
        for (uint32_t r : br.second) src << "      case " << r << "u:";
        src << " root" << br.first << "(v, R, hp, row, rd.meta_sites, rootmap, walk, out, am); break;\n";
      }
    } else {
      uint32_t si = 0;
      for (auto& br : by_rep) {
        src << "      case " << si++ << "u: root" << br.first << "(v, R, hp, row, rd.meta_sites, rootmap, walk, out, am); break;\n";
      }
    }
    src << "      default: if (walk) out.status = ST_FALLBACK;\n"
           "    }\n"
           "  }\n"
           "};\n";
    if (fused.empty()) continue;
    const bool heavy_grp = gwpe[gi] == -1 && std::count(gwpe.begin(), gwpe.end(), -2);
    const char* split_env = heavy_grp ? getenv("KYV_FUSED_SPLIT_HEAVY") : getenv("KYV_FUSED_SPLIT");
    const size_t nparts = std::max<size_t>(1, std::min<size_t>(fused.size(), split_env ? (size_t)atoi(split_env) : heavy_grp ? 1 : 3));
    for (size_t pi = 0; pi < nparts; pi++) {
      const std::vector<size_t> part(fused.begin() + fused.size() * pi / nparts, fused.begin() + fused.size() * (pi + 1) / nparts);
      const std::string sname = "JitFused" + std::to_string(gi) + (pi ? "p" + std::to_string(pi) : std::string());
      std::vector<uint32_t> conds;
      if (gi == fold_group)
        for (size_t j = 0; j < folded.size(); j++)
          if (fold_mode == 2 ? pi + 1 == nparts : j % nparts == pi) conds.push_back(folded[j]);
      src << "struct " << sname << " {\n"
             "  __device__ __forceinline__ void run(const View& v, const DevOut& o, uint32_t nwaves, uint32_t w, uint32_t r,\n"
             "                                     bool active, uint32_t hflags, uint32_t hroot, uint32_t hnn, const uint32_t* gw) {\n"
             "    const uint32_t lane = threadIdx.x & 63u;\n"
             "    const Node* R = v.nodes + hroot;\n"
             "    const ResHeader* hp = v.hdr + r;\n"
             "    const uint32_t row = r < v.nres ? r : NONE;\n"
             "    const bool rootmap = (hflags & RF_ROOT_MAP) != 0;\n"
             "    const uint32_t am = wave_maps(v, w);\n"
             "    (void)lane; (void)hp; (void)rootmap; (void)hnn; (void)am;\n";
      if (!conds.empty()) src << "    __shared__ uint32_t jl[" << jc_lds << "];\n";
      if (ncslots) {
        std::map<uint32_t, std::vector<uint32_t>> users;
        for (size_t i : part)
          for (uint32_t c : rule_cols[i]) if (cslot.count(c)) users[c].push_back(rule_roots[i].first);
        src << "    __shared__ uint64_t jcc[" << ncslots * 64u << "u];\n"
               "    uint32_t jsl[KYV_FUSED_GW];\n"
               "#pragma unroll\n"
               "    for (uint32_t i = 0; i < KYV_FUSED_GW; i++) {\n"
               "      const uint32_t b0 = 32u * i, lo = o.rule_lo > b0 ? o.rule_lo - b0 : 0u, hi = o.rule_hi > b0 ? o.rule_hi - b0 : 0u;\n"
               "      const uint32_t mlo = lo >= 32u ? 0u : (0xFFFFFFFFu << lo), mhi = hi >= 32u ? 0xFFFFFFFFu : ((1u << hi) - 1u);\n"
               "      jsl[i] = active ? (gw[i] & mlo & mhi) : 0u;\n"
               "    }\n";
        for (const auto& cu : users) {
          std::map<uint32_t, uint32_t> wm;
          for (uint32_t k : cu.second) wm[k / 32] |= 1u << (k % 32);
          src << "    if (";
          size_t j = 0;
          for (const auto& e : wm) src << (j++ ? " | " : "") << "(jsl[" << e.first << "] & " << e.second << "u)";
          src << ") jcc[" << cslot[cu.first] * 64u << "u + lane] = jc_col(v, " << Gen::u(cu.first) << ", row);\n";
        }
      }
      for (size_t j = 0; j < part.size(); j++) {
      const size_t i = part[j];
      const uint32_t k = rule_roots[i].first;
      const RuleDesc& rd = rs.rules[k];
      const bool pat = rd.kind == RK_PATTERN;
      const uint32_t nalts = pat ? 1u : rd.nalts, alts = pat ? 1u : std::min<uint32_t>(rd.nalts, MAX_ALTS);
      const std::string K = Gen::u(k);
      src << "    if (" << K << " >= o.rule_lo && " << K << " < o.rule_hi) {\n"
             "      const bool gated = active && ((gw[" << k / 32 << "] >> " << k % 32 << "u) & 1u);\n"
             "      if (__ballot(gated)) {\n"
             "        const View& vl = KYV_RULE_VIEW(v);\n";
      src << "        const bool magic = gated && (hflags & RF_MAGIC);\n"
             "        WaveSink sink{o.stage + sld32(o.rbase + (" << K << " - o.rule_lo)) + (size_t)w * 64u * " << alts
          << "u, 0u, " << (rd.uses_meta ? "true" : "false") << "};\n"
             "        uint8_t st = pair_walk_alts(" << (pat ? "true" : "false") << ", " << nalts << "u, gated && !magic, r, " << K
          << ", sink, [&](uint32_t a, bool wk, PatOut& po) {\n"
             "          po.status = ST_NONE; po.idx = 0; po.tmpl = NONE; po.key0 = NONE; po.key1 = NONE;\n"
             "          switch (a) {\n";
      for (uint32_t a = 0; a < nalts; a++) {
        const uint32_t root = rule_roots[i].second[a];
        if (ncslots)
          src << "            case " << a << "u: rootc" << rep_of[root] << "_" << gi << "(vl, R, hp, row, " << Gen::u(rd.meta_sites)
              << ", rootmap, wk, po, jcc, am); break;\n";
        else
          src << "            case " << a << "u: root" << rep_of[root] << "(vl, R, hp, row, " << Gen::u(rd.meta_sites)
              << ", rootmap, wk, po, am); break;\n";
      }
      src << "            default: break;\n"
             "          }\n"
             "        });\n"
             "        if (magic) st = ST_FALLBACK;\n"
             "        if (gated) { o.status[(size_t)" << K << " * v.nres + r] = st; KYV_ACCT_ADD(1, 1); }\n"
             "        if (sink.n && lane == 0) {\n"
             "          o.rcnt[(size_t)(" << K << " - o.rule_lo) * nwaves + w] = (uint16_t)sink.n; KYV_ACCT_ADD(1, 2);\n"
             "        }\n"
             "      }\n"
             "    }\n";
    }
      for (uint32_t k : conds) {
        const std::string K = Gen::u(k);
        src << "    if (" << K << " >= o.rule_lo && " << K << " < o.rule_hi) {\n"
               "      const bool gated = active && ((gw[" << k / 32 << "] >> " << k % 32 << "u) & 1u);\n"
               "      if (__ballot(gated)) {\n"
               "        uint8_t st = ST_NONE;\n"
               "        if (gated) st = jr" << k << "(KYV_RULE_VIEW(v), r, hroot, hnn, jl + lane);\n"
               "        if (gated && st != ST_NONE) { o.status[(size_t)" << K << " * v.nres + r] = st; KYV_ACCT_ADD(1, 1); }\n"
               "      }\n"
               "    }\n";
      }
      src << "  }\n"
             "};\n";
      fused_kernels.push_back(std::make_pair(gi, pi));
    }
    if (nparts > 1 && getenv("KYV_FUSED_MERGE") && atoi(getenv("KYV_FUSED_MERGE")) != 0) {
      src << "struct JitFusedM" << gi << " {\n"
             "  __device__ __forceinline__ void run(const View& v, const DevOut& o, uint32_t nwaves, uint32_t w, uint32_t r,\n"
             "                                     bool active, uint32_t hflags, uint32_t hroot, uint32_t hnn, const uint32_t* gw) {\n";
      for (size_t pi = 0; pi < nparts; pi++) {
        const std::string sname = "JitFused" + std::to_string(gi) + (pi ? "p" + std::to_string(pi) : std::string());
        src << "    {\n"
               "      uint32_t r2 = r, h2 = hroot;\n"
               "      asm volatile(\"\" : \"+v\"(r2), \"+v\"(h2));\n"
               "      " << sname << " f;\n"
               "      f.run(v, o, nwaves, w, r2, active, hflags, h2, hnn, gw);\n"
               "    }\n";
      }
      src << "  }\n"
             "};\n";
      merged_groups.push_back(gi);
    }
  }
  std::vector<std::pair<uint32_t, uint32_t>> shape_list;
  {
    std::map<std::pair<uint32_t, std::string>, uint32_t> sid;
    for (const auto& rr : rule_roots) {
      const uint32_t k = rr.first;
      if (!jit_shape_eligible(rs, k) || rr.second.size() != 1) continue;
      const auto key = std::make_pair(rep_of[rr.second[0]], meta_signature(rs, rs.rules[k]));
      auto it = sid.find(key);
      if (it == sid.end()) {
        if (shape_list.size() >= JIT_MAX_SHAPES) continue;
        it = sid.emplace(key, (uint32_t)shape_list.size()).first;
        shape_list.push_back(std::make_pair(rep_of[rr.second[0]], rs.rules[k].meta_sites));
      }
      if (jit_shape) (*jit_shape)[k] = (uint16_t)(it->second + 1);
    }
  }
  if (!shape_list.empty()) {
    src << "struct JitShapes {\n"
           "  __device__ __forceinline__ void run(const View& v, const ShapeOut& so, uint32_t r, bool active, uint32_t hflags,\n"
           "                                     uint32_t hroot, uint32_t cls, const uint32_t am) {\n"
           "    const Node* R = v.nodes + hroot;\n"
           "    const ResHeader* hp = v.hdr + r;\n"
           "    const uint32_t row = r < v.nres ? r : NONE;\n"
           "    const bool rootmap = (hflags & RF_ROOT_MAP) != 0;\n"
           "    (void)hp; (void)rootmap;\n";
    for (size_t si = 0; si < shape_list.size(); si++) {
      const std::string S = Gen::u((uint32_t)si);
      src << "    {\n"
             "      const bool gated = active && ((so.gate[(size_t)cls * so.words + " << si / 32 << "u] >> " << si % 32 << "u) & 1u);\n"
             "      if (__ballot(gated)) {\n"
             "        const bool magic = gated && (hflags & RF_MAGIC);\n"
             "        ShapeSink sink{so.rec + (size_t)" << S << " * v.nres + r};\n"
             "        uint8_t st = pair_walk_alts(true, 1u, gated && !magic, r, 0u, sink, [&](uint32_t, bool wk, PatOut& po) {\n"
             "          po.status = ST_NONE; po.idx = 0; po.tmpl = NONE; po.key0 = NONE; po.key1 = NONE;\n"
             "          root" << shape_list[si].first << "(v, R, hp, row, " << Gen::u(shape_list[si].second) << ", rootmap, wk, po, am);\n"
             "        });\n"
             "        if (magic) st = ST_FALLBACK;\n"
             "        if (gated) { so.st[(size_t)" << S << " * v.nres + r] = st; KYV_ACCT_ADD(1, 1); }\n"
             "      }\n"
             "    }\n";
    }
    src << "  }\n"
           "};\n";
  }
  src << "}  // namespace kyv\n"
         "#ifndef KYV_JIT_WPE\n#define KYV_JIT_WPE 4\n#endif\n";
  if (!shape_list.empty())
    src << "extern \"C\" __global__ void __launch_bounds__(64) __attribute__((amdgpu_waves_per_eu(KYV_JIT_WPE)))\n"
           "kyv_jit_shapes(const kyv::View* __restrict__ vp, kyv::ShapeOut so) {\n"
           "  kyv::JitShapes f;\n"
           "  kyv::walk_shapes(*vp, so, f);\n"
           "}\n";
  if (!crules.empty()) {
    src << "#ifndef KYV_JC_WPE\n#define KYV_JC_WPE 8\n#endif\n";
    const bool grouped = !getenv("KYV_JC_GROUP") || atoi(getenv("KYV_JC_GROUP")) != 0;
    const std::string& lds = jc_lds;
    std::vector<uint32_t> kept;
    for (uint32_t k : crules) if (std::find(folded.begin(), folded.end(), k) == folded.end()) kept.push_back(k);
    auto member = [&](uint32_t k, const std::string& on) {
      src << "  {\n"
             "    const bool gated = " << on << "((gw[" << k / 32 << "u] >> " << k % 32 << "u) & 1u);\n"
             "    if (__ballot(gated)) {\n"
             "      uint8_t st = kyv::ST_NONE;\n"
             "      if (gated) st = kyv::jr" << k << "(KYV_RULE_VIEW(v), r, hh.root, hh.nnodes, jl + lane);\n"
             "      if (gated && st != kyv::ST_NONE) { o.status[(size_t)" << k << "u * v.nres + r] = st; KYV_ACCT_ADD(1, 1); }\n"
             "    }\n"
             "  }\n";
    };
// ... 2 lines not shown
        src << "extern \"C\" __global__ void __launch_bounds__(64) __attribute__((amdgpu_waves_per_eu(KYV_JC_WPE)))\n"
               "kyv_jit_condg_" << grp[0] << "(const kyv::View* __restrict__ vp, kyv::DevOut o, uint32_t w0, uint32_t mask) {\n"
               "  __shared__ uint32_t jl[" << lds << "];\n"
               "  const kyv::View& v = *vp;\n"
               "  const uint32_t lane = threadIdx.x, r = (w0 + blockIdx.x) * 64u + lane;\n"
               "  kyv::HotHdr hh{0u, 0u, 0u, 0u};\n"
               "  if (r < v.nres) hh = kyv::ghot(v, r);  // header: kind class, and root and node count for the rules\n"
               "  const uint32_t* gw = r < v.nres ? v.gate + (size_t)hh.kclass * v.gate_words : nullptr;\n";
        for (size_t i = 0; i < grp.size(); i++) member(grp[i], "gw && (mask & " + std::to_string(1u << i) + "u) && ");
        src << "}\n";
      }
    } else {
      for (uint32_t k : kept) {
        src << "extern \"C\" __global__ void __launch_bounds__(64) __attribute__((amdgpu_waves_per_eu(KYV_JC_WPE)))\n"
               "kyv_jit_cond_" << k << "(const kyv::View* __restrict__ vp, kyv::DevOut o, uint32_t w0) {\n"
               "  __shared__ uint32_t jl[" << lds << "];\n"
               "  const kyv::View& v = *vp;\n"
               "  const uint32_t lane = threadIdx.x, r = (w0 + blockIdx.x) * 64u + lane;\n"
               "  kyv::HotHdr hh{0u, 0u, 0u, 0u};\n"
               "  if (r < v.nres) hh = kyv::ghot(v, r);  // header: kind class, and root and node count for the rules\n"
               "  const uint32_t* gw = r < v.nres ? v.gate + (size_t)hh.kclass * v.gate_words : nullptr;\n";
        member(k, "gw && ");
        src << "}\n";
      }
    }
    for (uint32_t k : crules) if (jit_cond) (*jit_cond)[k] = 1;
    for (uint32_t k : folded) if (jit_cond) (*jit_cond)[k] = (uint8_t)(2 + fold_group);
  }
  src << "#ifndef KYV_JIT_WPE_LIGHT\n#define KYV_JIT_WPE_LIGHT 8\n#endif\n";
  for (size_t gi = 0; gi < ngroups; gi++)
    src << "extern \"C\" __global__ void __launch_bounds__(64) __attribute__((amdgpu_waves_per_eu("
        << (gwpe[gi] == -2 ? "KYV_JIT_WPE_LIGHT" : "KYV_JIT_WPE") << ")))\n"
           "kyv_jit_walk_" << gi << "(const kyv::View* __restrict__ vp, kyv::DevOut o, kyv::WorkLists wl, kyv::ChunkMap cm) {\n"
           "  kyv::JitWalker" << gi << " wk{false, 0u};\n"
           "  kyv::walk_chunks(*vp, o, wl, cm, wk);\n"
           "}\n";
  src << "#ifndef KYV_JIT_WPE_FUSED\n#define KYV_JIT_WPE_FUSED 8\n#endif\n"
         "#ifndef KYV_JIT_WPE_FUSED_HEAVY\n#define KYV_JIT_WPE_FUSED_HEAVY 4\n#endif\n";
  for (const auto& gp : fused_kernels) {
    const std::string sfx = std::to_string(gp.first) + (gp.second ? "p" + std::to_string(gp.second) : std::string());
    src << "extern \"C\" __global__ void __launch_bounds__(64) __attribute__((amdgpu_waves_per_eu("
        << (gwpe[gp.first] == -1 && std::count(gwpe.begin(), gwpe.end(), -2) ? "KYV_JIT_WPE_FUSED_HEAVY" : "KYV_JIT_WPE_FUSED")
        << ")))\n"
           "kyv_jit_fused_" << sfx << "(const kyv::View* __restrict__ vp, kyv::DevOut o, uint32_t nwaves) {\n"
           "  kyv::JitFused" << sfx << " f;\n"
           "  kyv::walk_fused(*vp, o, nwaves, f);\n"
           "}\n";
  }
  for (size_t gi : merged_groups) {
    src << "extern \"C\" __global__ void __launch_bounds__(64) __attribute__((amdgpu_waves_per_eu("
        << (gwpe[gi] == -1 && std::count(gwpe.begin(), gwpe.end(), -2) ? "KYV_JIT_WPE_FUSED_HEAVY" : "KYV_JIT_WPE_FUSED")
        << ")))\n"
           "kyv_jit_fusedm_" << gi << "(const kyv::View* __restrict__ vp, kyv::DevOut o, uint32_t nwaves) {\n"
           "  kyv::JitFusedM" << gi << " f;\n"
           "  kyv::walk_fused(*vp, o, nwaves, f);\n"
           "}\n";
  }
  return src.str();
}

std::vector<std::vector<uint32_t>> jit_cond_groups(const Ruleset& rs, const std::vector<uint32_t>& crules) {
  std::vector<std::vector<uint32_t>> out;
  std::map<std::pair<bool, std::vector<uint32_t>>, size_t> open;
  for (uint32_t k : crules) {
    KindGate g = rule_gate(rs, rs.rules[k]);
    std::sort(g.kinds.begin(), g.kinds.end());
    g.kinds.erase(std::unique(g.kinds.begin(), g.kinds.end()), g.kinds.end());
// ... 122 lines not shown
```

### kyverno_amd/csrc/kyv_engine.hip

```cpp
#define KYV_SEL_INLINE 1
#include <hip/hip_runtime.h>

#include <algorithm>
#include <array>
#include <map>
#include <chrono>
#include <cmath>
#include <functional>
#include <cstdlib>
#include <mutex>
#include <set>
#include <cstdio>
#include <cstring>
#include <stdexcept>
#include <string>
#include <thread>
#include <vector>

#include "kyv_acct.h"
#include "kyv_host.h"
#define KYV_NO_KERNELS 1
#include "kyv_kernels.h"

namespace kyv {
// ... 307 lines not shown
};

struct DeviceResults {
  uint8_t* status = nullptr;
  uint32_t* pss_fails = nullptr;
  uint32_t* pss_slot = nullptr;
  FailRec* recs = nullptr;
  uint32_t* nrecs = nullptr;
  bool recs_resident = false;
  std::vector<FailRec> host_recs;
  FailRec* hrecs_dev = nullptr;
  size_t hrecs_cap = 0;
  FailRec* stage = nullptr;
  uint16_t* rcnt = nullptr;
  uint32_t* tsum = nullptr;
  uint32_t* tseg = nullptr;
  uint32_t* ttot = nullptr;
  unsigned long long* counts = nullptr;
  size_t max_recs = 0;
  size_t recs_cap = 0;
  uint32_t npss = 0;
  size_t nres = 0, nrules = 0;
  size_t max_slice_rules = 0;
  hipStream_t stream = nullptr;
  hipEvent_t e0 = nullptr, e1 = nullptr;
  hipStream_t cstream = nullptr;
  hipEvent_t cfork = nullptr, cjoin = nullptr;
  hipStream_t wstream = nullptr;
  hipEvent_t wfork = nullptr, wjoin = nullptr;
  View* view = nullptr;
  const MetaKeyRow* view_meta = nullptr;
  const HotHdr* view_hot = nullptr;
  uint32_t view_fact_and = 0;
  uint8_t* shape_st = nullptr;
  FailRec* shape_rec = nullptr;
  uint32_t* shape_gate = nullptr;
  uint32_t nshapes = 0, shape_words = 0;
  int shape_state = -1;
  TailCfg* tcfg = nullptr;
  ResFacts* facts = nullptr;
  bool facts_on = false;
  EvalPlan plan;
  bool plan_ruleset_done = false;
  WorkLists wl{};
  std::vector<SliceSched> slices;
  int cus = 256;
};

static void free_dev_results(DeviceResults& d, int dev) {
  dfree(d.view); dfree(d.status); dfree(d.pss_fails); dfree(d.pss_slot); dfree(d.recs); dfree(d.nrecs); dfree(d.counts);
  dfree(d.hrecs_dev);
  dfree(d.stage); dfree(d.rcnt); dfree(d.tsum); dfree(d.tseg);
  dfree(d.shape_st); dfree(d.shape_rec); dfree(d.shape_gate); dfree(d.tcfg); dfree(d.facts);
  dfree(d.wl.items); dfree(d.wl.cnt);
  for (auto& sl : d.slices) {
    dfree(sl.rbase); dfree(sl.mrules); dfree(sl.mrec); dfree(sl.mcls); dfree(sl.mcrec); dfree(sl.tails); dfree(sl.sched);
    if (sl.evs) hipEventDestroy(sl.evs);
    for (auto e : sl.ev) if (e) hipEventDestroy(e);
    for (auto e : sl.cev) if (e) hipEventDestroy(e);
  }
  stream_put(dev, d.stream, d.e0, d.e1);
  stream_put(dev, d.cstream, d.cfork, d.cjoin);
  stream_put(dev, d.wstream, d.wfork, d.wjoin);
  d = DeviceResults();
}

struct DevBatch {
  int device = -1;
  DeviceResults* out = nullptr;
  uint8_t* base = nullptr;
  size_t bytes = 0;
  size_t o_nodes, o_hdr, o_hot, o_facts, o_faux, o_soff, o_slen, o_sflags, o_sdur, o_sqty, o_sf64, o_heap, o_nsloff, o_nslkv, o_gate,
      o_colv, o_coloff, o_pe, o_supper = SIZE_MAX, o_srx = SIZE_MAX;
  uint32_t* gmask = nullptr;
  uint32_t gmask_words = 0;
  uint32_t* inv = nullptr;
  uint32_t* order = nullptr;
  double upload_ms = 0;
  double gmask_ms = 0;
  MetaKeyRow* meta_rows = nullptr;
  size_t meta_bytes = 0;
  double meta_ms = 0;
};

static DevRuleset* upload_ruleset(const Ruleset& rs, int device) {
  HIP_OK(hipSetDevice(device));
  auto* d = new DevRuleset();
  d->device = device;
  Packer p;
  d->o_rules = p.add(rs.rules);
  d->o_filters = p.add(rs.filters);
  d->o_kinds = p.add(rs.kinds);
  d->o_sels = p.add(rs.sels);
  d->o_reqs = p.add(rs.reqs);
  d->o_pn = p.add(rs.pnodes);
  d->o_pe = p.add(rs.pentries);
  d->o_leaves = p.add(rs.leaves);
  d->o_atoms = p.add(rs.atoms);
  d->o_metas = p.add(rs.metas);
  d->o_pss = p.add(rs.pss);
  d->o_pool = p.add(rs.pool);
  d->o_cnodes = p.add(rs.cnodes);
  d->o_conds = p.add(rs.conds);
  d->o_cprogs = p.add(rs.cprogs);
  d->o_gpats = p.add(rs.gpats);
  std::vector<uint32_t> gs(rs.gsets.size() + 1, 0);
  for (size_t q = 0; q < rs.gsets.size(); q++) gs[q + 1] = gs[q] + (uint32_t)rs.gsets[q].size();
  for (auto& st : rs.gsets) gs.insert(gs.end(), st.begin(), st.end());
  d->o_gsets = p.add(gs);
  d->o_mclasses = p.add(rs.meta_classes);
  d->bytes = p.size;
  HIP_OK(hipMalloc(&d->base, d->bytes));
  HIP_OK(p.copy_to(d->base));
  return d;
}

static DevBatch* upload_batch(const Batch& b, int device) {
  HIP_OK(hipSetDevice(device));
  auto t0 = std::chrono::steady_clock::now();
  auto* d = new DevBatch();
  d->device = device;
  Packer p;
  d->o_nodes = p.add(b.nodes);
  d->o_hdr = p.add(b.hdr);
  d->o_hot = p.add(b.hot);
  d->o_facts = p.add(b.facts);
  d->o_faux = p.add(b.faux);
  d->o_soff = p.add(b.str_off);
  d->o_slen = p.add(b.str_len);
  d->o_sflags = p.add(b.str_flags);
  d->o_sdur = p.add(b.str_dur);
  d->o_sqty = p.add(b.str_qty);
  d->o_sf64 = p.add(b.str_f64);
  d->o_heap = p.add(b.heap);
  d->o_nsloff = p.add(b.nsl_off);
  d->o_nslkv = p.add(b.nsl_kv);
  d->o_gate = p.add(b.gate);
  d->o_supper = b.str_upper.empty() ? SIZE_MAX : p.add(b.str_upper);
  d->o_srx = b.str_rx.empty() ? SIZE_MAX : p.add(b.str_rx);
  d->o_colv = p.add(b.colv);
  d->o_coloff = p.add(b.col_off);
  std::vector<PEntry> pe = b.rs->pentries;
  for (auto& E : pe) if (E.col != NONE) E.col = b.col_off[E.col];
  d->o_pe = p.add(pe);
  d->bytes = p.size;
  HIP_OK(dmalloc(&d->base, d->bytes));
  HIP_OK(p.copy_to(d->base));
  d->upload_ms = std::chrono::duration<double, std::milli>(std::chrono::steady_clock::now() - t0).count();
  return d;
}

static bool hot_plane_on() {
  const char* e = getenv("KYV_HOTHDR");
  return !e || atoi(e) != 0;
}

static View make_view(const Ruleset& rs, const Batch& b, const uint8_t* rbase, const DevRuleset* dr, const uint8_t* bbase,
                      const DevBatch* db) {
  View v{};
  if (db) {
    v.nodes = (const Node*)(bbase + db->o_nodes);
    v.hdr = (const ResHeader*)(bbase + db->o_hdr);
    v.hot = hot_plane_on() && b.hot.size() == b.hdr.size() ? (const HotHdr*)(bbase + db->o_hot) : nullptr;
    v.facts = b.facts.size() == (b.hdr.size() + 63) / 64 ? (const WaveFacts*)(bbase + db->o_facts) : nullptr;
    v.faux = (const FloatAux*)(bbase + db->o_faux);
    v.str_off = (const uint32_t*)(bbase + db->o_soff);
    v.str_len = (const uint32_t*)(bbase + db->o_slen);
    v.str_flags = (const uint32_t*)(bbase + db->o_sflags);
    v.str_dur = (const int64_t*)(bbase + db->o_sdur);
    v.str_qty = (const int64_t*)(bbase + db->o_sqty);
    v.str_f64 = (const double*)(bbase + db->o_sf64);
    v.heap = bbase + db->o_heap;
    v.nsl_off = (const uint32_t*)(bbase + db->o_nsloff);
    v.nsl_kv = (const uint32_t*)(bbase + db->o_nslkv);
    v.gate = (const uint32_t*)(bbase + db->o_gate);
    v.colv = (const uint64_t*)(bbase + db->o_colv);
    v.col_off = (const uint32_t*)(bbase + db->o_coloff);
    v.str_upper = db->o_supper == SIZE_MAX ? nullptr : (const uint32_t*)(bbase + db->o_supper);
    v.str_rx = db->o_srx == SIZE_MAX ? nullptr : (const uint32_t*)(bbase + db->o_srx);
    v.str_gmask = db->gmask;
    v.gmask_words = db->gmask_words;
    v.meta_rows = db->meta_rows;
  } else {
    v.str_gmask = nullptr;
    v.gmask_words = 0;
    v.nodes = b.nodes.data(); v.hdr = b.hdr.data(); v.faux = b.faux.data();
    v.hot = hot_plane_on() && b.hot.size() == b.hdr.size() ? b.hot.data() : nullptr;
    v.facts = b.facts.size() == (b.hdr.size() + 63) / 64 ? b.facts.data() : nullptr;
    v.str_off = b.str_off.data(); v.str_len = b.str_len.data(); v.str_flags = b.str_flags.data();
    v.str_dur = b.str_dur.data(); v.str_qty = b.str_qty.data(); v.str_f64 = b.str_f64.data();
    v.heap = b.heap.data(); v.nsl_off = b.nsl_off.data(); v.nsl_kv = b.nsl_kv.data();
    v.gate = b.gate.data();
    v.str_upper = b.str_upper.empty() ? nullptr : b.str_upper.data();
    v.str_rx = b.str_rx.empty() ? nullptr : b.str_rx.data();
    v.colv = b.colv.data();
    v.col_off = b.col_off.data();
  }
  v.gate_words = b.gate_words;
  v.nres = (uint32_t)b.hdr.size();
  v.fact_and = wave_maps_mask();
  v.nrules = (uint32_t)rs.rules.size();
  if (dr) {
    v.rules = (const RuleDesc*)(rbase + dr->o_rules);
    v.filters = (const Filter*)(rbase + dr->o_filters);
    v.kinds = (const KindDesc*)(rbase + dr->o_kinds);
    v.sels = (const SelDesc*)(rbase + dr->o_sels);
    v.reqs = (const SelReq*)(rbase + dr->o_reqs);
    v.pn = (const PNode*)(rbase + dr->o_pn);
    v.pe = (const PEntry*)(rbase + dr->o_pe);
    v.leaves = (const Leaf*)(rbase + dr->o_leaves);
    v.atoms = (const Atom*)(rbase + dr->o_atoms);
    v.metas = (const MetaSite*)(rbase + dr->o_metas);
    v.pss = (const PssDesc*)(rbase + dr->o_pss);
    v.pool = (const uint32_t*)(rbase + dr->o_pool);
    v.cnodes = (const Node*)(rbase + dr->o_cnodes);
    v.conds = (const Cond*)(rbase + dr->o_conds);
    v.cprogs = (const CondProg*)(rbase + dr->o_cprogs);
  } else {
    v.rules = rs.rules.data(); v.filters = rs.filters.data(); v.kinds = rs.kinds.data(); v.sels = rs.sels.data();
    v.reqs = rs.reqs.data(); v.pn = rs.pnodes.data(); v.pe = rs.pentries.data(); v.leaves = rs.leaves.data();
    v.atoms = rs.atoms.data(); v.metas = rs.metas.data(); v.pss = rs.pss.data(); v.pool = rs.pool.data();
    v.cnodes = rs.cnodes.data(); v.conds = rs.conds.data(); v.cprogs = rs.cprogs.data();
  }
  if (db) v.pe = (const PEntry*)(bbase + db->o_pe);
  return v;
}


__device__ __forceinline__ const FailRec* chunk_stage(const FailRec* stage, const uint32_t* rbase, const RuleDesc* rules,
                                                      uint32_t nwaves, size_t c) {
  const uint32_t k = (uint32_t)(c / nwaves), w = (uint32_t)(c % nwaves);
  const uint32_t alts = rules[k].kind == RK_PATTERN ? 1u : min(rules[k].nalts, (uint32_t)MAX_ALTS);
  return stage + rbase[k] + (size_t)w * WAVE * alts;
// ... 410 lines not shown
      return 1 + d;
    case P_ARR_MAPS: return 1 + pattern_depth(rs, P.first, guard + 1);
    case P_ARR_POS:
      for (uint32_t i = 0; i < P.n; i++) d = std::max(d, pattern_depth(rs, rs.pool[P.first + i], guard + 1));
      return 1 + d;
    default: return 0;
  }
}

static int ruleset_depth(const Ruleset& rs) {
  int d = 1;
  for (auto& rd : rs.rules) {
    if (rd.kind == RK_PATTERN) d = std::max(d, pattern_depth(rs, rd.root, 0));
    else if (rd.kind == RK_ANYPATTERN)
      for (uint32_t a = 0; a < rd.nalts; a++) d = std::max(d, pattern_depth(rs, rs.pool[rd.root + a], 0));
  }
  return std::min(d, (int)MAX_DEPTH);
}


static std::mutex g_jit_mu;
static void mrs_clear_shapes(Ruleset& rs) {
  std::fill(rs.jit_shape.begin(), rs.jit_shape.end(), (uint16_t)0);
  rs.jit_nshapes = 0;
}
static bool ensure_jit(Ruleset& rs, DevRuleset* dr) {
  if (dr->jloaded) return true;
  std::lock_guard<std::mutex> lk(g_jit_mu);
  if (!rs.jit_tried) {
    rs.jit_tried = true;
    try {
      rs.jit_meta_keys = jit_meta_keys_on() && !rs.meta_classes.empty();
      rs.jit_jc_chains = jit_jc_chains_mode();
      std::string src = jit_source(rs, &rs.jit_rules, &rs.jit_cond, &rs.jit_shape, rs.jit_meta_keys ? 1 : 0, rs.jit_jc_chains);
      rs.jit_nshapes = 0;
      for (auto x : rs.jit_shape) rs.jit_nshapes = std::max<uint32_t>(rs.jit_nshapes, x);
      bool any = false;
      for (auto x : rs.jit_rules) any |= x != 0;
      for (auto x : rs.jit_cond) any |= x != 0;
      if (any) rs.jit_code = jit_compile(src, &rs.jit_compile_s);
    } catch (std::exception& e) {
      rs.jit_error = e.what();
      rs.jit_code.clear();
      fprintf(stderr, "[kyvgpu] runtime-compiled walk kernel unavailable, using the interpreted one: %s\n", e.what());
    }
  }
  if (rs.jit_code.empty()) return false;
  HIP_OK(hipModuleLoadData(&dr->jmod, rs.jit_code.data()));
  uint32_t ng = 0;
  for (auto x : rs.jit_rules) ng = std::max<uint32_t>(ng, x);
  dr->jfns.resize(ng);
  dr->ffns.assign(ng, nullptr);
  for (uint32_t g = 0; g < ng; g++) {
    HIP_OK(hipModuleGetFunction(&dr->jfns[g], dr->jmod, ("kyv_jit_walk_" + std::to_string(g)).c_str()));
    if (hipModuleGetFunction(&dr->ffns[g], dr->jmod, ("kyv_jit_fused_" + std::to_string(g)).c_str()) != hipSuccess)
      dr->ffns[g] = nullptr;
    dr->fparts.resize(ng);
    for (int p = 1; dr->ffns[g]; p++) {
      hipFunction_t f = nullptr;
      if (hipModuleGetFunction(&f, dr->jmod, ("kyv_jit_fused_" + std::to_string(g) + "p" + std::to_string(p)).c_str()) != hipSuccess)
        break;
      dr->fparts[g].push_back(f);
    }
    dr->fmfns.resize(ng, nullptr);
    if (hipModuleGetFunction(&dr->fmfns[g], dr->jmod, ("kyv_jit_fusedm_" + std::to_string(g)).c_str()) != hipSuccess)
      dr->fmfns[g] = nullptr;
  }
// ... 3 lines not shown
    dr->jshapes = nullptr;
    mrs_clear_shapes(rs);
  }
  (void)hipGetLastError();
  dr->jconds.assign(rs.rules.size(), nullptr);
  dr->jc_group.assign(rs.rules.size(), -1);
  dr->jcg.clear();
  dr->jcg_members.clear();
  {
    std::vector<uint32_t> crules;
    for (size_t k = 0; k < rs.jit_cond.size(); k++) if (rs.jit_cond[k] == 1) crules.push_back((uint32_t)k);
    for (auto& grp : jit_cond_groups(rs, crules)) {
      hipFunction_t f = nullptr;
      if (hipModuleGetFunction(&f, dr->jmod, ("kyv_jit_condg_" + std::to_string(grp[0])).c_str()) != hipSuccess) continue;
      for (uint32_t k : grp) dr->jc_group[k] = (int32_t)dr->jcg.size();
      dr->jcg.push_back(f);
      dr->jcg_members.push_back(grp);
    }
    (void)hipGetLastError();
  }
  for (size_t k = 0; k < rs.jit_cond.size(); k++)
    if (rs.jit_cond[k] == 1 && dr->jc_group[k] < 0)
      HIP_OK(hipModuleGetFunction(&dr->jconds[k], dr->jmod, ("kyv_jit_cond_" + std::to_string(k)).c_str()));
  dr->jloaded = true;
  return true;
}

static bool ensure_jit_acct(Ruleset& rs, DevRuleset* dr) {
  if (dr->aloaded) return true;
  if (!ensure_jit(rs, dr)) return false;
  std::lock_guard<std::mutex> lk(g_jit_mu);
  if (rs.jit_code_acct.empty()) {
    std::vector<uint8_t> jr, jc;
    rs.jit_code_acct = jit_compile(jit_source(rs, &jr, &jc, nullptr, rs.jit_meta_keys ? 1 : 0, rs.jit_jc_chains), nullptr, true);
  }
  HIP_OK(hipModuleLoadData(&dr->amod, rs.jit_code_acct.data()));
  dr->afns.resize(dr->jfns.size());
  dr->affns.assign(dr->jfns.size(), nullptr);
  for (size_t g = 0; g < dr->jfns.size(); g++) {
    HIP_OK(hipModuleGetFunction(&dr->afns[g], dr->amod, ("kyv_jit_walk_" + std::to_string(g)).c_str()));
    if (dr->ffns[g]) HIP_OK(hipModuleGetFunction(&dr->affns[g], dr->amod, ("kyv_jit_fused_" + std::to_string(g)).c_str()));
    dr->afparts.resize(dr->jfns.size());
    dr->afparts[g].assign(g < dr->fparts.size() ? dr->fparts[g].size() : 0, nullptr);
    for (size_t p = 0; p < dr->afparts[g].size(); p++)
      HIP_OK(hipModuleGetFunction(&dr->afparts[g][p], dr->amod,
                                  ("kyv_jit_fused_" + std::to_string(g) + "p" + std::to_string(p + 1)).c_str()));
    dr->afmfns.resize(dr->jfns.size(), nullptr);
    if (g < dr->fmfns.size() && dr->fmfns[g])
      HIP_OK(hipModuleGetFunction(&dr->afmfns[g], dr->amod, ("kyv_jit_fusedm_" + std::to_string(g)).c_str()));
  }
  dr->aconds.assign(dr->jconds.size(), nullptr);
  for (size_t k = 0; k < dr->jconds.size(); k++)
    if (dr->jconds[k]) HIP_OK(hipModuleGetFunction(&dr->aconds[k], dr->amod, ("kyv_jit_cond_" + std::to_string(k)).c_str()));
  dr->ajshapes = nullptr;
  if (dr->jshapes) HIP_OK(hipModuleGetFunction(&dr->ajshapes, dr->amod, "kyv_jit_shapes"));
  dr->ajcg.assign(dr->jcg.size(), nullptr);
  for (size_t g = 0; g < dr->jcg.size(); g++)
    HIP_OK(hipModuleGetFunction(&dr->ajcg[g], dr->amod, ("kyv_jit_condg_" + std::to_string(dr->jcg_members[g][0])).c_str()));
  hipDeviceptr_t p = nullptr;
  size_t bytes = 0;
  HIP_OK(hipModuleGetGlobal(&p, &bytes, dr->amod, "kyv_acct_bytes"));
  dr->acnt = (unsigned long long*)p;
  dr->aloaded = true;
  return true;
}

static size_t rule_slice_bytes(const RuleDesc& rd) {
// ... 708 lines not shown
    HIP_OK(hipEventCreate(&g0));
    HIP_OK(hipEventCreate(&g1));
    HIP_OK(hipEventRecord(g0, 0));
    hipLaunchKernelGGL(gmask_kernel, dim3((unsigned)((nstr + 255) / 256)), dim3(256), 0, 0, (const View*)dv, gp,
                       (uint32_t)rs.gpats.size(), gs, (uint32_t)rs.gsets.size(), (uint32_t)nstr, db->gmask_words, db->gmask);
    HIP_OK(hipGetLastError());
    HIP_OK(hipEventRecord(g1, 0));
    HIP_OK(hipDeviceSynchronize());
    float gms = 0;
    HIP_OK(hipEventElapsedTime(&gms, g0, g1));
    db->gmask_ms = gms;
    (void)hipEventDestroy(g0);
    (void)hipEventDestroy(g1);
    dfree(dv);
  }
  View v = make_view(rs, b, dr->base, dr, db->base, db);
  size_t nres = b.hdr.size(), nrules = rs.rules.size();
  if (!db->out) {
    auto* dd = new DeviceResults();
    DeviceResults& d = *dd;
    d.nres = nres;
    d.nrules = nrules;
    std::vector<uint32_t> pss_slot(nrules, NONE);
    for (size_t k = 0; k < nrules; k++) if (rs.rules[k].kind == RK_PSS) pss_slot[k] = d.npss++;
    HIP_OK(dmalloc(&d.status, std::max<size_t>(1, nres * nrules)));
    HIP_OK(dmalloc(&d.pss_fails, std::max<size_t>(4, (size_t)d.npss * nres * 4)));
    HIP_OK(dmalloc(&d.pss_slot, std::max<size_t>(4, nrules * 4)));
    HIP_OK(dmalloc(&d.nrecs, 16));
    HIP_OK(dmalloc(&d.counts, std::max<size_t>(1, nrules) * NSTATUS * 8));
    HIP_OK(hipMemcpy(d.pss_slot, pss_slot.data(), nrules * 4, hipMemcpyHostToDevice));
    stream_get(&d.stream, &d.e0, &d.e1);
    HIP_OK(dmalloc(&d.view, sizeof(View)));
    HIP_OK(hipMemcpy(d.view, &v, sizeof(View), hipMemcpyHostToDevice));
    d.view_hot = v.hot; d.view_fact_and = v.fact_and;
    d.wl.nwaves = (uint32_t)((nres + WAVE - 1) / WAVE);
    const size_t nwv = d.wl.nwaves;
    const size_t budget = slice_budget();
    for (size_t k = 0; k < nrules || (nrules == 0 && d.slices.empty());) {
      SliceSched sl;
      sl.k0 = (uint32_t)k;
      size_t bytes = 0, stage = 0;
      while (k < nrules) {
        const RuleDesc& rd = rs.rules[k];
        const size_t cost = rule_slice_bytes(rd) * nwv * WAVE + nwv * 2;
        const size_t alts = rd.kind == RK_PATTERN ? 1 : rd.kind == RK_ANYPATTERN ? std::min<uint32_t>(rd.nalts, MAX_ALTS) : 0;
        const size_t st2 = stage + alts * nwv * WAVE;
        const size_t nk = k + 1 - sl.k0;
        if (k > sl.k0 && (bytes + cost > budget || st2 > 0xFFFFFFF0ull || nk * nwv > 0xFFFFFFF0ull)) break;
        if (st2 > 0xFFFFFFF0ull) throw std::runtime_error("batch too large for one rule's failure-record staging");
        bytes += cost;
        stage = st2;
        k++;
      }
      sl.k1 = (uint32_t)k;
      sl.stage_tot = stage;
      std::vector<uint32_t> rb(std::max<size_t>(sl.k1 - sl.k0, 1), 0);
      size_t tot = 0;
      std::vector<uint32_t> ml, mj;
      for (uint32_t q = sl.k0; q < sl.k1; q++) {
        const RuleDesc& rd = rs.rules[q];
        rb[q - sl.k0] = (uint32_t)tot;
        tot += (rd.kind == RK_PATTERN ? 1 : rd.kind == RK_ANYPATTERN ? std::min<uint32_t>(rd.nalts, MAX_ALTS) : 0) * nwv * WAVE;
        const bool direct = (rd.kind == RK_PATTERN || rd.kind == RK_ANYPATTERN) && (rd.flags & RD_GATE_EXACT);
        if (!direct) (rule_needs_jmes(rs, rd) ? mj : ml).push_back(q);
      }
      sl.ml = ml;
      sl.mj = mj;
// ... 2 lines not shown
      d.max_slice_rules = std::max<size_t>(d.max_slice_rules, sl.k1 - sl.k0);
      d.max_recs = std::max<size_t>(d.max_recs, std::max<size_t>(sl.stage_tot, 1));
      d.slices.push_back(std::move(sl));
      if (nrules == 0) break;
    }
    const size_t msr = std::max<size_t>(d.max_slice_rules, 1);
    HIP_OK(dmalloc(&d.stage, d.max_recs * sizeof(FailRec)));
    HIP_OK(dmalloc(&d.recs, d.max_recs * sizeof(FailRec)));
    d.recs_cap = d.max_recs;
    HIP_OK(dmalloc(&d.rcnt, std::max<size_t>(msr * nwv, 1) * 2));
    const size_t max_tiles = std::max<size_t>((msr * nwv + WAVE - 1) / WAVE, 1);
    HIP_OK(dmalloc(&d.tsum, max_tiles * 8));
    d.ttot = d.tsum + max_tiles;
    HIP_OK(dmalloc(&d.tseg, std::max<size_t>((msr * nwv + WAVE - 1) / WAVE / SCAN_SEG + 1, 1) * 4));
    HIP_OK(dmalloc(&d.wl.items, std::max<size_t>(1, msr * nwv * WAVE) * sizeof(uint2)));
    HIP_OK(dmalloc(&d.wl.cnt, std::max<size_t>(4, msr * nwv + 4)));
    static std::mutex cu_mu;
    static std::vector<int> cu_count;
    int cus = 0;
    {
      std::lock_guard<std::mutex> g(cu_mu);
      if ((int)cu_count.size() <= device) cu_count.resize(device + 1, 0);
      if (!cu_count[device]) {
        int c = 0;
        if (hipDeviceGetAttribute(&c, hipDeviceAttributeMultiprocessorCount, device) != hipSuccess || c <= 0) c = 256;
        cu_count[device] = c;
      }
      cus = cu_count[device];
    }
    d.cus = cus;
    db->out = dd;
  }
  DeviceResults& d = *db->out;
  if (d.view_hot != v.hot || d.view_fact_and != v.fact_and) {
    HIP_OK(hipMemcpy(d.view, &v, sizeof(View), hipMemcpyHostToDevice));
    d.view_hot = v.hot; d.view_fact_and = v.fact_and;
  }
  hipStream_t stream = d.stream;
  const bool use_jit = jit_mode == JIT_ON || (jit_mode == JIT_AUTO && nres >= JIT_AUTO_MIN_RESOURCES);
  const bool jit = use_jit && ensure_jit(mrs, dr);
  if (jit && rs.jit_meta_keys && !db->meta_rows && nres) {
    const size_t nrows = rs.meta_classes.size() * nres;
    db->meta_bytes = nrows * sizeof(MetaKeyRow);
    HIP_OK(dmalloc(&db->meta_rows, db->meta_bytes));
    hipEvent_t g0, g1;
    HIP_OK(hipEventCreate(&g0));
    HIP_OK(hipEventCreate(&g1));
    HIP_OK(hipEventRecord(g0, 0));
    hipLaunchKernelGGL(meta_keys_kernel, dim3((unsigned)((nrows + 255) / 256)), dim3(256), 0, 0, (const View*)d.view,
                       (const MetaClass*)(dr->base + dr->o_mclasses), (uint32_t)rs.meta_classes.size(), db->meta_rows);
    HIP_OK(hipGetLastError());
    HIP_OK(hipEventRecord(g1, 0));
    HIP_OK(hipDeviceSynchronize());
    float gms = 0;
    HIP_OK(hipEventElapsedTime(&gms, g0, g1));
    db->meta_ms = gms;
    (void)hipEventDestroy(g0);
    (void)hipEventDestroy(g1);
  }
  if (d.view_meta != db->meta_rows) {
    v.meta_rows = db->meta_rows;
    HIP_OK(hipMemcpy(d.view, &v, sizeof(View), hipMemcpyHostToDevice));
    d.view_meta = db->meta_rows;
  }
  for (auto& sl : d.slices)
    if (sl.jit_state != (int)jit) layout_schedule(rs, b, dr, d, sl, jit);
  if (d.shape_state != (int)jit) setup_shapes(rs, b, d, jit && dr->jshapes);
  const bool multi = d.slices.size() > 1;
  int depth = ruleset_depth(rs);
// ... 1032 lines not shown
```

### kyverno_amd/csrc/kyv_eval.h

```cpp
#pragma once
#ifndef __HIPCC_RTC__
#include <hip/hip_runtime.h>
#endif

#include "kyv_layout.h"

namespace kyv {

#define KYV_HD __host__ __device__ inline
#define KYV_BIG __host__ __device__ inline __attribute__((noinline))
#ifndef KYV_FN_MATCH
#define KYV_FN_MATCH KYV_HD
#endif
#ifndef KYV_FN_PATTERN
#define KYV_FN_PATTERN KYV_HD
#endif
#ifndef KYV_FN_PSS
#define KYV_FN_PSS KYV_BIG
#endif

struct TouchAcct {
  uint8_t* seen;
  uint32_t n;
  uint64_t rows;
// ... 22 lines not shown
  } while (0)

#if defined(__HIP_DEVICE_COMPILE__)
KYV_HD void touch_row(uint32_t) { KYV_ACCT_ADDK(1u, 0, 16); }
#else
KYV_HD void touch_row(uint32_t i) {
  TouchAcct* t = g_touch;
  if (t && i < t->n && !t->seen[i]) { t->seen[i] = 1; t->rows++; }
}
#endif

enum FallbackWhy : int { FBW_NONE = 0, FBW_MATCH = 1, FBW_PHRASE = 2, FBW_COND = 3, FBW_DEPTH = 4, FBW_VALUE = 5,
                         FBW_META = 6, FBW_VAR = 7 };
inline thread_local int g_fb_why = FBW_NONE;
#if defined(__HIP_DEVICE_COMPILE__)
#define KYV_WHY(c) ((void)0)
#else
#define KYV_WHY(c) (::kyv::g_fb_why = (c))
#endif

struct NodeTab {
  const Node* p;
  KYV_HD const Node& operator[](uint32_t i) const { touch_row(i); return p[i]; }
  KYV_HD explicit operator bool() const { return p != nullptr; }
};

struct View {
  const Node* nodes;
  const ResHeader* hdr;
  const HotHdr* hot;
  uint32_t nres;
  const WaveFacts* facts;
  uint32_t fact_and;
  const FloatAux* faux;
  const uint32_t* str_off;
  const uint32_t* str_len;
  const uint32_t* str_flags;
  const int64_t* str_dur;
  const int64_t* str_qty;
  const double* str_f64;
  const uint8_t* heap;
  const uint32_t* nsl_off;
  const uint32_t* nsl_kv;
  const uint32_t* gate;
  uint32_t gate_words;
  const uint32_t* str_gmask;
  uint32_t gmask_words;
  const uint32_t* str_upper;
  const uint32_t* str_rx;
  const uint64_t* colv;
  const uint32_t* col_off;
  const MetaKeyRow* meta_rows;
  const RuleDesc* rules;
  uint32_t nrules;
  const Filter* filters;
  const KindDesc* kinds;
  const SelDesc* sels;
  const SelReq* reqs;
  const PNode* pn;
  const PEntry* pe;
  const Leaf* leaves;
  const Atom* atoms;
  const MetaSite* metas;
  const PssDesc* pss;
  const uint32_t* pool;
  const Node* cnodes;
// ... 839 lines not shown
```

### kyverno_amd/csrc/kyv_fused.h

```cpp
#pragma once
#include "kyv_wave.h"

namespace kyv {

#ifndef KYV_FUSED_GW
#define KYV_FUSED_GW 8
#endif

template <class Fused>
__device__ __forceinline__ void walk_fused(const View& v, DevOut o, uint32_t nwaves, Fused& f) {
  const uint32_t lane = threadIdx.x & (WAVE - 1);
#ifdef KYV_FUSED_STRIDE
  for (uint32_t w = blockIdx.x; w < nwaves; w += gridDim.x) {
#else
  if (const uint32_t w = blockIdx.x; w < nwaves) {
#endif
    const uint32_t r = w * WAVE + lane;
    const bool active = r < v.nres;
    uint32_t hflags = 0, hroot = 0, hnn = 0, cls = 0;
    if (active) {
      const HotHdr h = ghot(v, r);
      hflags = h.flags;
      hroot = h.root;
      hnn = h.nnodes;
// ... 8 lines not shown
      if (i < v.gate_words) {
        if (uniform) gw[i] = sld32(v.gate + (size_t)c0 * v.gate_words + i);
        else if (active) gw[i] = gld32(v.gate + (size_t)cls * v.gate_words + i);
      }
    }
    f.run(v, o, nwaves, w, r, active, hflags, hroot, hnn, gw);
  }
}

struct ShapeSink {
  FailRec* at;
  __device__ __forceinline__ void emit(bool has, const FailRec& f) {
    if (!has) return;
    *at = f;
    KYV_ACCT_ADD(1, sizeof(FailRec));
  }
};

template <class Shapes>
__device__ __forceinline__ void walk_shapes(const View& v, const ShapeOut& so, Shapes& f) {
  const uint32_t lane = threadIdx.x & (WAVE - 1);
  for (uint32_t w = blockIdx.x; w < so.nwaves; w += gridDim.x) {
    const uint32_t r = w * WAVE + lane;
    const bool active = r < v.nres;
    uint32_t hflags = 0, hroot = 0, hnn = 0, cls = 0;
    if (active) {
      const HotHdr h = ghot(v, r);
      hflags = h.flags;
      hroot = h.root;
      hnn = h.nnodes;
      cls = h.kclass;
    }
    (void)hnn;
    f.run(v, so, r, active, hflags, hroot, cls, wave_maps(v, w));
  }
}

}
```

### kyverno_amd/csrc/kyv_host.h

```cpp
#pragma once
#include <cstdint>
#include <functional>
#include <memory>
#include <string>
#include <unordered_map>
#include <vector>

#include "kyv_layout.h"
#include "pjson.h"

namespace kyv {

template <class T>
struct NoInitAlloc : std::allocator<T> {
  template <class U> struct rebind { using other = NoInitAlloc<U>; };
  NoInitAlloc() = default;
  template <class U> NoInitAlloc(const NoInitAlloc<U>&) noexcept {}
  template <class U> void construct(U* p) noexcept { ::new ((void*)p) U; }
  template <class U, class... A> void construct(U* p, A&&... a) { ::new ((void*)p) U(std::forward<A>(a)...); }
};
template <class T> using bulk_vector = std::vector<T, NoInitAlloc<T>>;

struct Dict {
  std::vector<std::string> strs;
// ... 70 lines not shown
  std::vector<PEntry> pentries;
  std::vector<Leaf> leaves;
  std::vector<Atom> atoms;
  std::vector<MetaSite> metas;
  std::vector<PssDesc> pss;
  std::vector<uint32_t> pool;
  std::vector<Node> cnodes;
  std::vector<Cond> conds;
  std::vector<CondProg> cprogs;
  std::vector<CondText> cond_text;
  std::vector<std::string> templates;
  std::unordered_map<std::string, uint32_t> template_ids;
  struct TrieNode {
    uint32_t col = NONE;
    uint32_t rowspace = 0;
    uint32_t star = NONE;
    uint32_t lencol = NONE;
    std::vector<std::pair<uint32_t, uint32_t>> kids;
  };
  std::vector<TrieNode> trie;
  std::vector<uint32_t> gpats;
  std::vector<std::vector<uint32_t>> gsets;
  std::vector<uint32_t> cond_set;
  std::vector<std::string> rx_src;
  std::vector<RxDfa> rxs;
  bool uses_upper = false;
  uint32_t ncols = 0, nrowspaces = 1;
  std::vector<uint32_t> col_rowspace;
  std::vector<uint32_t> pn_self;
  std::vector<uint32_t> pe_self;
  std::vector<uint32_t> pn_len;
  std::vector<uint32_t> pe_len;
  std::vector<uint32_t> fact_spaces;
  std::vector<MetaClass> meta_classes;
  std::vector<int8_t> meta_class_of;
  bool jit_meta_keys = false;
  int jit_jc_chains = 0;
  bool jit_tried = false;
  std::vector<uint8_t> jit_rules;
  std::vector<uint8_t> jit_cond;
  std::vector<uint16_t> jit_shape;
  uint32_t jit_nshapes = 0;
  std::vector<char> jit_code;
  std::vector<char> jit_code_acct;
  std::string jit_error;
  double jit_compile_s = 0;
  std::vector<void*> dev;
  ~Ruleset();
};

struct TypedDecoder {
  enum Target { POD = 0, DEPLOYMENT = 1, CRONJOB = 2 };
  explicit TypedDecoder(const std::function<uint32_t(const std::string&)>& find_sid);
  enum Outcome { DEC_OK = 0, DEC_ERR = 1, DEC_FOLD = 2 };
  int decode(const Node* R, const std::vector<std::string>& strs, int target) const;
  std::unordered_map<uint32_t, uint32_t> name_of_sid;
};

struct Batch {
  const Ruleset* rs = nullptr;
  Dict dict;
  bulk_vector<Node> nodes;
  bulk_vector<ResHeader> hdr;
  bulk_vector<HotHdr> hot;
  std::vector<FloatAux> faux;
  std::vector<uint32_t> str_off, str_len, str_flags;
  std::vector<uint32_t> str_upper, str_rx;
  std::vector<int64_t> str_dur, str_qty;
  std::vector<double> str_f64;
  std::vector<uint8_t> heap;
  std::vector<uint32_t> nsl_off, nsl_kv;
  std::vector<std::string> nsl_names;
  std::vector<uint32_t> order;
  std::vector<uint32_t> inv;
  std::vector<uint64_t> shape_key;
  std::shared_ptr<const std::vector<uint32_t>> inv_shared;
  std::vector<uint32_t> gate;
  uint32_t gate_words = 0, nclass = 0;
  bulk_vector<uint64_t> colv;
  std::vector<uint32_t> col_off, rs_rows;
  std::vector<WaveFacts> facts;
  std::vector<void*> dev;
  ~Batch();
};

struct FailPath {
  uint32_t res, rule, alt;
  uint32_t tmpl;
  uint16_t idx[MAX_IDX];
  uint32_t key[2];
};

struct SlicePlan { uint32_t k0 = 0, k1 = 0, fused = 0, chunk = 0, cond = 0; };
struct EvalPlan {
  uint32_t gmask_patterns = 0, cond_sets = 0, gmask_words = 0, unmasked = 0;
  uint32_t onemask = 0;
  uint32_t tail_used[5] = {0, 0, 0, 0, 0};
  uint32_t tail_cand[5] = {0, 0, 0, 0, 0};
  uint32_t fast = 0, fasteval = 0, generic = 0;
};
void plan_ruleset(const Ruleset& rs, EvalPlan* p);

struct Results {
  uint32_t nres = 0, nrules = 0;
  EvalPlan plan;
  std::vector<SlicePlan> slices;
  std::vector<uint8_t> status;
  std::vector<uint32_t> pss_fails;
  std::vector<FailRec> fails;
  int64_t counts[NSTATUS] = {0};
  std::vector<int64_t> rule_counts;
  double kernel_ms = 0, h2d_ms = 0, d2h_ms = 0;
  double gmask_ms = 0;
  double meta_keys_ms = 0;
  double phase_ms[5] = {0, 0, 0, 0, 0};
  uint64_t alg_bytes = 0;
  uint64_t alg_bytes_phase[5] = {0, 0, 0, 0, 0};
  uint64_t alg_bytes_class[3] = {0, 0, 0};
  int jit_used = 0;
};

Ruleset* compile_ruleset(const char* json, size_t len, std::string* err, const char* exceptions = nullptr,
                         size_t ex_len = 0, bool background = false);
Batch* build_batch(const Ruleset* rs, const char* json, size_t len, const char* nsl_json, size_t nsl_len, int threads,
                   std::string* err);
void derive_strings(Batch& b, size_t from, int threads);
void build_path_trie(Ruleset& rs);
void assign_wave_facts(Ruleset& rs);
void assign_meta_classes(Ruleset& rs);
bool jit_meta_keys_on();
std::vector<MetaKeyRow> meta_key_rows_host(const Ruleset& rs, const Batch& b);
std::vector<MetaKeyRow> meta_key_rows_device(const Batch& b, int device);
size_t meta_key_plane_bytes(const Batch& b);
uint32_t wave_maps_mask();
void assign_glob_masks(Ruleset& rs);
void assign_cond_sets(Ruleset& rs);
int jit_jc_chains_mode();
std::string jit_source(const Ruleset& rs, std::vector<uint8_t>* jit_rules, std::vector<uint8_t>* jit_cond = nullptr,
                       std::vector<uint16_t>* jit_shape = nullptr, int meta_keys = -1, int jc_chains = -1);
bool jit_shape_eligible(const Ruleset& rs, uint32_t k);
constexpr uint32_t JIT_MAX_SHAPES = 64;
std::vector<char> jit_compile(const std::string& src, double* seconds, bool acct = false);
bool jit_rule_fused(const Ruleset& rs, uint32_t k);
std::vector<std::vector<uint32_t>> jit_cond_groups(const Ruleset& rs, const std::vector<uint32_t>& crules);
struct KindGate {
  bool any = false;
  std::vector<uint32_t> kinds;
};
KindGate rule_gate(const Ruleset& rs, const RuleDesc& rd);
enum JitMode { JIT_AUTO = 0, JIT_OFF = 1, JIT_ON = 2 };
constexpr size_t JIT_AUTO_MIN_RESOURCES = 65536;
void resolve_path_columns(Batch& b, int threads);
constexpr uint32_t SHAPE_KEY_BITS = 3, SHAPE_KEY_MAX_NODES = 64 / SHAPE_KEY_BITS;
std::vector<uint32_t> shape_key_nodes(const Ruleset& rs);
std::string format_path(const Ruleset& rs, const Batch& b, uint32_t tmpl, const uint16_t* idx, const uint32_t* key);

}
```

### kyverno_amd/csrc/kyv_jcond.h

```cpp
#pragma once
#include "kyv_wave.h"
#include "kyv_cond.h"
#include "kyv_pss.h"

namespace kyv {

constexpr uint32_t JCAP = 16;

__device__ __forceinline__ uint64_t jc_col(const View& v, uint32_t col, uint32_t row) {
  if (row == NONE) return COL_NONE;
  KYV_ACCT_ADDK(2u, 0, 8);
  const uint32_t off = sld32(v.col_off + col);
  return gcol(v.colv, off, row);
}
__device__ __forceinline__ kyv_u32x4 jc_meta(const View& v, uint32_t cls, uint32_t row) {
  if (row == NONE) return kyv_u32x4{0u, NONE, NONE, NONE};
  KYV_ACCT_ADD(0, 16);
  return *(const KYV_AS_GLOBAL kyv_u32x4*)(v.meta_rows + ((size_t)cls * v.nres + row));
}
__device__ __forceinline__ uint32_t jc_dec(uint64_t x, uint32_t* t, uint32_t* a) {
  const uint32_t lo = (uint32_t)x;
  *a = (uint32_t)(x >> 32);
  if (lo == NONE) { *t = T_UNK; *a = 0; return NONE; }
  *t = lo >> COL_TYPE_SHIFT;
  return lo & COL_INDEX_MASK;
}
__device__ __forceinline__ uint32_t jc_type(const Node* R, uint32_t i, uint32_t t) {
  if (i == NONE) return N_NULL;
  return t != T_UNK ? t : (gtk(R + i) & 0xFu);
}
__device__ __forceinline__ void jc_field(const View& v, const Node* R, uint32_t i, uint32_t row, uint32_t col, uint32_t key,
                                         uint32_t* oi, uint32_t* ot, uint32_t* oa) {
  *ot = T_UNK;
  *oa = 0;
  if (col != NONE && row != NONE) {
    uint32_t x = jc_dec(jc_col(v, col, row), ot, oa);
    if (x != NONE && *ot == N_NULL) { x = NONE; *ot = T_UNK; *oa = 0; }
    *oi = x;
    return;
  }
  if (i == NONE) { *oi = NONE; return; }
  const Node m = gnode(R + i);
  if (node_type(m) != N_MAP) { *oi = NONE; return; }
  const uint32_t x = wmap_find(R, m.a, m.b, key);
  if (x == NONE) { *oi = NONE; return; }
  const Node n = gnode(R + x);
// ... 103 lines not shown
```

### kyverno_amd/csrc/kyv_layout.h

```cpp
#pragma once
#ifndef __HIPCC_RTC__
#include <cstdint>
#else
typedef __hip_internal::uint8_t uint8_t;
typedef __hip_internal::uint16_t uint16_t;
typedef __hip_internal::uint32_t uint32_t;
typedef __hip_internal::uint64_t uint64_t;
typedef __hip_internal::int32_t int32_t;
typedef __hip_internal::int64_t int64_t;
typedef __hip_internal::size_t size_t;
#ifndef INT64_MAX
#define INT64_MAX 9223372036854775807LL
#define INT64_MIN (-INT64_MAX - 1)
#define INT32_MAX 2147483647
#define INT32_MIN (-INT32_MAX - 1)
#endif
#endif

namespace kyv {

constexpr uint32_t NONE = 0xFFFFFFFFu;

enum NodeType : uint32_t { N_NULL = 0, N_FALSE = 1, N_TRUE = 2, N_INT = 3, N_FLOAT = 4, N_STR = 5, N_MAP = 6, N_ARR = 7 };

// ... 49 lines not shown
  RF_PSS_DONE = 1u << 9,
  RF_PSS_DEC_ERR = 1u << 10,
  RF_PSS_FOLD = 1u << 19,
};
constexpr uint32_t RF_META_SHIFT = 5, RF_TMETA1_SHIFT = 11, RF_TMETA2_SHIFT = 15;

struct ResHeader {
  uint32_t root;
  uint32_t nnodes;
  uint32_t kind;
  uint32_t gvk_kind;
  uint32_t group, version;
  uint32_t gv;
  uint32_t name, gen_name, ns;
  uint32_t labels;
  uint32_t ann;
  uint32_t nsl;
  uint32_t flags;
  uint32_t orig;
  uint32_t kclass;
};
static_assert(sizeof(ResHeader) == 64, "header size");

struct HotHdr {
  uint32_t root, nnodes, flags, kclass;
};
static_assert(sizeof(HotHdr) == 16, "hot header row size");

constexpr uint32_t FACT_BITS = 32;
struct WaveFacts {
  uint32_t maps;
};
static_assert(sizeof(WaveFacts) == 4, "wave facts row size");

enum MatchMode : uint8_t { MM_NONE = 0, MM_PLAIN = 1, MM_ANY = 2, MM_ALL = 3,
                           MM_EXC_ALL = 4 };

enum FilterFlag : uint16_t {
  FF_ZERO_RD = 1 << 0,
  FF_USERINFO = 1 << 1,
  FF_KINDS_STAR = 1 << 2,
  FF_SEL_INVALID = 1 << 3,
  FF_NSSEL_INVALID = 1 << 4,
  FF_HAS_SEL = 1 << 5,
  FF_HAS_NSSEL = 1 << 6,
};

struct KindDesc {
  uint32_t kind;
  uint32_t gv_mode;
  uint32_t g, v;
};

struct Filter {
  uint16_t flags;
  uint16_t nkinds;
  uint32_t kinds;
  uint32_t name;
  uint32_t names, nnames;
  uint32_t nss, nnss;
  uint32_t ann, nann;
  uint32_t sel, nsel;
};

enum ReqOp : uint32_t { RQ_EQ = 0, RQ_IN = 1, RQ_NOTIN = 2, RQ_EXISTS = 3, RQ_NOTEXISTS = 4, RQ_WILD = 5 };
struct SelReq {
// ... 313 lines not shown
```

### kyverno_amd/csrc/kyv_wave.h

```cpp
#pragma once
#include "kyv_eval.h"
#include "kyv_walk.h"

namespace kyv {

#define KYV_AS_CONST __attribute__((address_space(4)))
#define KYV_AS_GLOBAL __attribute__((address_space(1)))

template <class T>
__device__ __forceinline__ T sld(const T* p) {
  static_assert(sizeof(T) % 4 == 0, "sld: 4-byte multiple");
  uint32_t w[sizeof(T) / 4];
  const KYV_AS_CONST uint32_t* q = (const KYV_AS_CONST uint32_t*)p;
#pragma unroll
  for (int i = 0; i < (int)(sizeof(T) / 4); i++) w[i] = q[i];
  T out;
  __builtin_memcpy(&out, w, sizeof(T));
  return out;
}
__device__ __forceinline__ uint32_t sld32(const uint32_t* p) { return *(const KYV_AS_CONST uint32_t*)p; }
typedef uint32_t kyv_u32x4 __attribute__((ext_vector_type(4)));
__device__ __forceinline__ Node gnode(const Node* p) {
  KYV_ACCT_ADDK(1u, 0, 16);
  const KYV_AS_GLOBAL kyv_u32x4* q = (const KYV_AS_GLOBAL kyv_u32x4*)p;
// ... 13 lines not shown
__device__ __forceinline__ uint64_t wballot(bool p) { return __ballot(p); }

__device__ __forceinline__ uint32_t wmap_find(const Node* R, uint32_t a, uint32_t n, uint32_t key) {
  uint32_t lo = a, hi = a + n;
  while (lo < hi) {
    uint32_t mid = (lo + hi) >> 1;
    uint32_t k = gtk(R + mid) >> 4;
    if (k == key) return mid;
    if (k < key) lo = mid + 1; else hi = mid;
  }
  return NONE;
}

constexpr uint32_t T_UNK = 0xE;

__device__ __forceinline__ uint32_t gld32(const uint32_t* p) { return *(const KYV_AS_GLOBAL uint32_t*)p; }

__device__ __forceinline__ HotHdr ghot(const View& v, uint32_t r) {
  HotHdr h;
  if (v.hot) {
    const kyv_u32x4 x = *(const KYV_AS_GLOBAL kyv_u32x4*)(v.hot + r);
    h.root = x.x; h.nnodes = x.y; h.flags = x.z; h.kclass = x.w;
    KYV_ACCT_ADD(0, 16);
  } else {
    const ResHeader* p = v.hdr + r;
    h.root = gld32(&p->root); h.nnodes = gld32(&p->nnodes); h.flags = gld32(&p->flags); h.kclass = gld32(&p->kclass);
    KYV_ACCT_ADD(0, 16);
  }
  return h;
}
__device__ __forceinline__ uint32_t wave_maps(const View& v, uint32_t w) {
  return v.facts ? (sld32(&v.facts[w].maps) & v.fact_and) : 0u;
}
__device__ __forceinline__ uint32_t ghot_flags(const View& v, const ResHeader* hp) {
  KYV_ACCT_ADD(0, 4);
  return v.hot ? gld32(&v.hot[hp - v.hdr].flags) : gld32(&hp->flags);
}

__device__ __forceinline__ uint32_t wcol(const View& v, const PEntry& E, bool al, uint32_t row) {
  if (al) KYV_ACCT_ADDK(2u, 0, 4);
  return al ? gld32((const uint32_t*)(v.colv + (size_t)E.col + row)) : NONE;
}
__device__ __forceinline__ uint32_t col_decode(uint32_t enc, uint32_t* ctype) {
  if (enc == NONE) { *ctype = T_UNK; return NONE; }
  *ctype = enc >> COL_TYPE_SHIFT;
  return enc & COL_INDEX_MASK;
}
__device__ __forceinline__ uint32_t wlookup(const View& v, const PEntry& E, bool al, const Node* R, uint32_t a, uint32_t b,
                                            uint32_t row, const Keys& keys, uint32_t* ctype) {
  *ctype = T_UNK;
  if (!al) return NONE;
  if (E.col != NONE) return col_decode(wcol(v, E, al, row), ctype);
  uint32_t key = (E.flags & EF_WILD) ? keys.get(E.slot) : E.key;
  return wmap_find(R, a, b, key);
}

__device__ __forceinline__ Val wvalue_node(const View& v, Node n) {
  Val x;
  x.wsid = NONE; x.nsid = NONE; x.sid = NONE; x.i = 0; x.f = 0;
  x.t = node_type(n);
  switch (x.t) {
    case N_NULL: x.nsid = SID_ZERO; break;
    case N_FALSE: x.wsid = SID_FALSE; break;
    case N_TRUE: x.wsid = SID_TRUE; break;
    case N_INT: x.i = (int64_t)(((uint64_t)n.b << 32) | n.a); x.wsid = n.c; x.nsid = n.c; break;
    case N_FLOAT: {
// ... 522 lines not shown
      }
    }
#undef KYV_PUSH
#undef KYV_POP
#ifdef KYV_EXP_STEPS
    if (lane == 0) atomicAdd(&kyv_exp_steps, (unsigned long long)nsteps);
#endif

    out.key0 = keys.k0;
    out.key1 = keys.k1;
    if (!walk) { out.status = ST_NONE; return; }
    if (dead & lbit) { out.status = ost; return; }
    if (!ret.err) { out.status = ST_PASS; out.tmpl = NONE; return; }
    if (ret_is_skip(ret)) { out.status = ST_SKIP; out.tmpl = NONE; return; }
    if (ret_is_neg(ret)) { out.status = ST_FAIL; out.tmpl = ret.tmpl; return; }
    if (seen & ~found) { out.status = ST_ERROR; out.tmpl = NONE; return; }
    out.tmpl = ret.tmpl;
    out.status = ret.tmpl == NONE ? ST_ERROR : ST_FAIL;
  }
};
template <> struct walker_takes_dyn<WaveWalker> { static constexpr bool value = true; };

struct JW {
  const View& v;
  const Node* R;
  const ResHeader* hp;
  uint64_t seen, found;
  Keys keys;
  uint64_t idx;
  uint32_t mbase;
  uint8_t ost;
  uint32_t am;
  const Val* dyn = nullptr;
};
template <uint8_t OP, uint8_t FLAGS, uint8_t GLOB, uint32_t GI1 = 0>
__device__ __forceinline__ bool jatom(const View& v, const Val& x, uint32_t pat, uint32_t lit, int64_t dur, int64_t qlo,
                                      int64_t qhi, bool* fb) {
  if ((FLAGS & AF_DUR) && x.nsid != NONE && (gld32(v.str_flags + x.nsid) & SF_DUR)) {
    int64_t d = *(const KYV_AS_GLOBAL int64_t*)(v.str_dur + x.nsid);
    if (cmp_op(OP, d < dur ? -1 : (d > dur ? 1 : 0))) return true;
  }
  if ((FLAGS & AF_QTY) && x.nsid != NONE) {
    uint32_t f = gld32(v.str_flags + x.nsid);
    if (f & SF_QTY_BIG) { *fb = true; return false; }
    if (f & SF_QTY) {
      const KYV_AS_GLOBAL int64_t* q = (const KYV_AS_GLOBAL int64_t*)(v.str_qty + 2 * (size_t)x.nsid);
      if (cmp_op(OP, cmp128(q[1], (uint64_t)q[0], qhi, (uint64_t)qlo))) return true;
    }
  }
  if ((OP == A_EQ || OP == A_NE) && x.wsid != NONE) {
    bool r = wglob(v, GLOB, pat, lit, x.wsid, GI1);
    return OP == A_NE ? !r : r;
  }
  return false;
}
constexpr uint64_t COL_NONE = 0xFFFFFFFFull;
__device__ __forceinline__ uint64_t gcol(const uint64_t* colv, uint32_t off, uint32_t row) {
#ifdef KYV_COL64
  return *(const KYV_AS_GLOBAL uint64_t*)(colv + (size_t)off + row);
#else
  return *(const KYV_AS_GLOBAL uint64_t*)(colv + (uint32_t)(off + row));
#endif
}
__device__ __forceinline__ uint64_t jraw(const JW& w, uint32_t e, uint32_t row) {
  const uint32_t off = sld32(&w.v.pe[e].col);
  if (row != NONE) KYV_ACCT_ADDK(4u, 0, 8);
// ... 128 lines not shown
    const bool uniform = (kw.y & SLOT_UNIFORM) != 0;
    const size_t list = (size_t)(k - o.rule_lo) * wl.nwaves + w;
    const RuleDesc rd = sld(v.rules + k);
    bool active;
    uint32_t r;
    uint2 it = make_uint2(0u, 0u);
    bool magic = false;
    if (rd.flags & RD_GATE_EXACT) {
      r = w * WAVE + lane;
      bool gated = false;
      if (r < v.nres) {
        const HotHdr h = ghot(v, r);
        const uint32_t fl = h.flags;
        if (uniform) {
          gated = true;
        } else {
          gated = (gld32(v.gate + (size_t)h.kclass * v.gate_words + (k >> 5)) >> (k & 31)) & 1u;
        }
        magic = gated && (fl & RF_MAGIC);
        it = make_uint2(r | ((fl & RF_ROOT_MAP) ? ITEM_ROOT_MAP : 0u), h.root);
      }
      active = gated && !magic;
      if (!uniform && !__ballot(gated)) continue;
    } else {
      const uint32_t n = sld8(wl.cnt + list);
      if (lane == 0) KYV_ACCT_ADD(0, 1);
      if (!n) continue;
      active = lane < n;
      if (active) { it = wl.items[list * WAVE + lane]; KYV_ACCT_ADD(0, 8); }
      r = it.x & ~ITEM_ROOT_MAP;
    }
    wk.rootmap = (it.x & ITEM_ROOT_MAP) != 0;
    wk.am = wave_maps(v, w);
    const uint32_t alts = rd.kind == RK_PATTERN ? 1u : min(rd.nalts, (uint32_t)MAX_ALTS);
    WaveSink sink{o.stage + sld32(o.rbase + (k - o.rule_lo)) + (size_t)w * WAVE * alts, 0u, rd.uses_meta != 0};
    uint8_t st = pair_walk(v, rd, active, r, k, v.nodes + it.y, wk, sink);
    if (magic) st = ST_FALLBACK;
    if (active || magic) { o.status[(size_t)k * v.nres + r] = st; KYV_ACCT_ADD(1, 1); }
    if (sink.n && lane == 0) { o.rcnt[list] = (uint16_t)sink.n; KYV_ACCT_ADD(1, 2); }
  }
}

}
```

### kyverno_amd/engine.py

```python
import ctypes
import json

import numpy as np

from . import _lib as K


def _dumps(x):
    if isinstance(x, (bytes, bytearray)):
        return bytes(x)
    if isinstance(x, str):
        return x.encode()
    return json.dumps(x, separators=(",", ":")).encode()


class Ruleset:
    def __init__(self, policies, exceptions=None, background=False):
        L = K.lib()
        data = _dumps(policies if not isinstance(policies, dict) else [policies])
        ex = _dumps(exceptions) if exceptions else None
        h = ctypes.c_void_p()
        opts = K.CompileOpts(K.KYV_ABI_VERSION, 1 if background else 0)
        K.check(L.kyv_ruleset_compile_ex(data, len(data), ex, len(ex) if ex else 0, ctypes.byref(opts), ctypes.byref(h)))
        self.h = h
# ... 57 lines not shown
            raise K.KyvError(L.kyv_last_error().decode(errors="replace"))
        out = np.empty(max(1, total), dtype=np.uint8)
        if L.kyv_batch_copy_status(self.h, device, res0, nres, out.ctypes.data, out.size) < 0:
            raise K.KyvError(L.kyv_last_error().decode(errors="replace"))
        nr = len(self.ruleset.rules)
        return out[:total].reshape(nr, total // max(1, nr))

    def stats(self):
        s = K.BatchStats()
        K.check(K.lib().kyv_batch_stats_get(self.h, ctypes.byref(s)))
        return {f: getattr(s, f) for f, _ in K.BatchStats._fields_}

    def wave_facts(self):
        L = K.lib()
        o = K.WaveFactsOut()
        K.check(L.kyv_batch_wave_facts(self.h, ctypes.byref(o)))
        nw = (self.n + 63) // 64
        facts = np.zeros(nw, dtype=np.uint32)
        hot = np.zeros((self.n, 4), dtype=np.uint32)
        order = np.zeros(self.n, dtype=np.uint32)
        bits = ctypes.create_string_buffer(o.bits_len + 1)
        o = K.WaveFactsOut(facts.ctypes.data, facts.size, hot.ctypes.data, hot.size, order.ctypes.data, order.size,
                           ctypes.addressof(bits), o.bits_len + 1, 0)
        K.check(L.kyv_batch_wave_facts(self.h, ctypes.byref(o)))
        sk = K.ShapeKeysOut()
        K.check(L.kyv_batch_shape_keys(self.h, ctypes.byref(sk)))
        keys = np.zeros(self.n, dtype=np.uint64)
        paths = ctypes.create_string_buffer(sk.paths_len + 1)
        sk = K.ShapeKeysOut(keys.ctypes.data, keys.size, ctypes.addressof(paths), sk.paths_len + 1, 0)
        K.check(L.kyv_batch_shape_keys(self.h, ctypes.byref(sk)))
        shape = json.loads(paths.value.decode())
        return dict(json.loads(bits.value.decode()), facts=facts, hot=hot, order=order, shape_keys=keys,
                    shape_paths=shape["paths"], shape_bits=shape["bits"], shape_ordered=shape["ordered"])

    def meta_keys(self, device=None):
        L = K.lib()
        dev = -1 if device is None else int(device)
        o = K.MetaKeysOut()
        K.check(L.kyv_batch_meta_keys(self.h, dev, ctypes.byref(o)))
        rows = np.zeros((o.classes, self.n, 4), dtype=np.uint32)
        desc = ctypes.create_string_buffer(o.desc_len + 1)
        o = K.MetaKeysOut(rows.ctypes.data, rows.size, ctypes.addressof(desc), o.desc_len + 1, 0, 0)
        K.check(L.kyv_batch_meta_keys(self.h, dev, ctypes.byref(o)))
        d = json.loads(desc.value.decode())
        return {"rows": rows, "classes": d["classes"], "decoded": d["rows"]}

    def __del__(self):
        if getattr(self, "h", None):
            K.lib().kyv_batch_free(self.h)
            self.h = None


class Results:
    def __init__(self, ruleset, batch, h, copied):
        self.ruleset, self.batch, self.h = ruleset, batch, h
        L = K.lib()
        self.counts = {K.STATUS_NAMES[s]: L.kyv_results_count(h, s) for s in range(8)}
        self.kernel_ms = L.kyv_results_kernel_ms(h)
        self.upload_ms = L.kyv_results_batch_ms(h, 0)
        self.gmask_ms = L.kyv_results_batch_ms(h, 1)
        self.meta_keys_ms = L.kyv_results_batch_ms(h, 2)
        ph = (ctypes.c_double * 5)()
        L.kyv_results_phase_ms(h, ph, 5)
        self.phase_ms = dict(zip(("match", "cond", "walk", "compact", "hist"), list(ph)))
        self.alg_bytes = L.kyv_results_alg_bytes(h)
        ab = (ctypes.c_uint64 * 5)()
# ... 169 lines not shown
```

Before: 154.8 billion.

## Add per-wave column-empty facts so JIT kernels skip loads for absent lists

Adds a host-side per-wave bitmask (64 bits) marking array-list trie nodes that no resource in a 64-resource wave populates. The JIT-generated pattern and condition code then substitutes NONE for the column row when the bit is set, skipping the column gather for lists known to be empty. This removes global-memory column loads and downstream array walks for absent lists, at the cost of an extra per-wave 8-byte load, extra host work during column resolution, and a ternary in generated code.

```diff
diff --git a/__graft_entry__.py b/__graft_entry__.py
--- a/__graft_entry__.py
+++ b/__graft_entry__.py
@@ -30,6 +30,9 @@
                      for off in ("", "-off") for a in (False, True)]
             import pattern_vars_cases
             jobs += [("tests-patvars:%d" % i, False) for i in range(len(pattern_vars_cases.compiled_rulesets()))]
+            import col_facts_cases
+            for i in range(len(col_facts_cases.compiled_rulesets())):
+                jobs += [("tests-colfacts:%d" % i, False), ("tests-colfacts:%d" % i, True), ("tests-colfacts-off:%d" % i, False)]
         except Exception as e:
             print("build: test rulesets not compiled ahead of time: %s" % e, file=sys.stderr)
         ctx = __import__("multiprocessing").get_context("spawn")
@@ -88,6 +91,15 @@
     elif wl.startswith("tests-patvars:"):
         import pattern_vars_cases
         pols = pattern_vars_cases.compiled_rulesets()[int(wl.split(":")[1])]
+    elif wl.startswith("tests-colfacts"):
+        import col_facts_cases
+        pols = col_facts_cases.compiled_rulesets()[int(wl.split(":")[1])]
+        if wl.startswith("tests-colfacts-off:"):
+            os.environ["KYV_JIT_COLFACTS"] = "0"
+            try:
+                return E.Ruleset(pols).jit_compile(accounting=acct)
+            finally:
+                del os.environ["KYV_JIT_COLFACTS"]
     elif wl.startswith("tests-condpre"):
         import cond_preload_cases
         pols = cond_preload_cases.compiled_rulesets()[int(wl.split(":")[1])]
diff --git a/include/kyvgpu.h b/include/kyvgpu.h
--- a/include/kyvgpu.h
+++ b/include/kyvgpu.h
@@ -115,6 +115,12 @@
   size_t bits_len;
 } kyv_wave_facts_out;
 int kyv_batch_wave_facts(const kyv_batch* b, kyv_wave_facts_out* out);
+typedef struct kyv_col_facts_out {
+  uint64_t* rows; size_t rows_cap;
+  char* bits; size_t bits_cap;
+  size_t bits_len;
+} kyv_col_facts_out;
+int kyv_batch_col_facts(const kyv_batch* b, kyv_col_facts_out* out);
 typedef struct kyv_shape_keys_out {
   uint64_t* keys; size_t keys_cap;
   char* paths; size_t paths_cap;
diff --git a/kyverno_amd/_lib.py b/kyverno_amd/_lib.py
--- a/kyverno_amd/_lib.py
+++ b/kyverno_amd/_lib.py
@@ -65,6 +65,7 @@
     "kyv_comm_gathered_status", "kyv_comm_gathered_failures", "kyv_comm_gather_report", "kyv_comm_reduce_counts", "kyv_results_batch_ms",
     "kyv_calibrate_fetch", "kyv_batch_wave_facts", "kyv_col_entries_fit32", "kyv_results_plan",
     "kyv_results_plan_slices", "kyv_batch_shape_keys", "kyv_batch_meta_keys",
+    "kyv_batch_col_facts",
 ]
 
 
@@ -72,6 +73,11 @@
     _fields_ = [("facts", ctypes.c_void_p), ("facts_cap", ctypes.c_size_t), ("hot", ctypes.c_void_p),
                 ("hot_cap", ctypes.c_size_t), ("order", ctypes.c_void_p), ("order_cap", ctypes.c_size_t),
                 ("bits", ctypes.c_void_p), ("bits_cap", ctypes.c_size_t), ("bits_len", ctypes.c_size_t)]
+
+
+class ColFactsOut(ctypes.Structure):
+    _fields_ = [("rows", ctypes.c_void_p), ("rows_cap", ctypes.c_size_t), ("bits", ctypes.c_void_p),
+                ("bits_cap", ctypes.c_size_t), ("bits_len", ctypes.c_size_t)]
 
 
 class ShapeKeysOut(ctypes.Structure):
@@ -164,6 +170,7 @@
     L.kyv_batch_num_resources.restype = u32
     L.kyv_batch_stats_get.argtypes = [vp, ctypes.POINTER(BatchStats)]
     L.kyv_batch_wave_facts.argtypes = [vp, ctypes.POINTER(WaveFactsOut)]
+    L.kyv_batch_col_facts.argtypes = [vp, ctypes.POINTER(ColFactsOut)]
     L.kyv_batch_shape_keys.argtypes = [vp, ctypes.POINTER(ShapeKeysOut)]
     L.kyv_batch_meta_keys.argtypes = [vp, ctypes.c_int, ctypes.POINTER(MetaKeysOut)]
     L.kyv_eval.argtypes = [vp, vp, ctypes.POINTER(EvalOpts), ctypes.POINTER(vp)]
diff --git a/kyverno_amd/csrc/batch.cpp b/kyverno_amd/csrc/batch.cpp
--- a/kyverno_amd/csrc/batch.cpp
+++ b/kyverno_amd/csrc/batch.cpp
@@ -1187,6 +1187,8 @@
   uint32_t* next;
   const int8_t* space_bit;
   uint32_t notmaps = 0;
+  const int8_t* list_bit;
+  uint64_t present = 0;
   uint64_t entry(uint32_t x) const {
     return ((uint64_t)R[x].a << 32) | ((uint64_t)node_type(R[x]) << COL_TYPE_SHIFT) | x;
   }
@@ -1206,6 +1208,7 @@
       const auto& K = kids[t];
       auto hit = [&](uint32_t x, uint32_t kid) {
         if (colv) colv[(size_t)col_off[rs.trie[kid].col] + row] = entry(x);
+        if (list_bit[kid] >= 0) present |= 1ull << list_bit[kid];
         go(x, kid, row);
       };
       if (mn.b <= 2 * K.size() + 4) {
@@ -1329,9 +1332,12 @@
   b.col_off.assign(rs.ncols, 0);
   b.colv.clear();
   b.facts.assign((n + 63) / 64, WaveFacts{0u});
+  b.col_facts.assign((n + 63) / 64, ColFacts{0ull});
   if (rs.ncols == 0 || n == 0) return;
   std::vector<int8_t> space_bit(nsp, -1);
   for (size_t i = 0; i < rs.fact_spaces.size(); i++) space_bit[rs.fact_spaces[i]] = (int8_t)i;
+  std::vector<int8_t> list_bit(rs.trie.size(), -1);
+  for (size_t j = 0; j < rs.fact_lists.size() && j < COLFACT_BITS; j++) list_bit[rs.fact_lists[j]] = (int8_t)j;
   int T = std::max(1, threads);
   std::vector<std::vector<std::pair<uint32_t, uint32_t>>> kids(rs.trie.size());
   for (size_t t = 0; t < rs.trie.size(); t++) {
@@ -1353,8 +1359,10 @@
           if (!eligible(h)) continue;
           Resolver rv{rs, kids, b.nodes.data() + h.root, fill ? b.colv.data() : nullptr, b.col_off.data(), nexts[c].data(),
                       space_bit.data()};
+          rv.list_bit = list_bit.data();
           rv.go(0, 0, (uint32_t)r);
           if (fill && rv.notmaps) __atomic_fetch_or(&b.facts[r / 64].maps, rv.notmaps, __ATOMIC_RELAXED);
+          if (fill && rv.present) __atomic_fetch_or(&b.col_facts[r / 64].empty, rv.present, __ATOMIC_RELAXED);
         }
       }
     };
@@ -1401,11 +1409,18 @@
   for (auto& h : b.hdr) if (!eligible(h)) h.flags |= RF_MAGIC;
   const uint32_t defined = rs.fact_spaces.size() >= 32 ? 0xFFFFFFFFu : (1u << rs.fact_spaces.size()) - 1u;
   for (auto& f : b.facts) f.maps = ~f.maps & defined;
+  const uint64_t lists = rs.fact_lists.size() >= COLFACT_BITS ? ~0ull : (1ull << rs.fact_lists.size()) - 1ull;
+  for (auto& f : b.col_facts) f.empty = ~f.empty & lists;
 }
 
 uint32_t wave_maps_mask() {
   const char* e = getenv("KYV_FACT_MAPS");
   return e && atoi(e) == 0 ? 0u : 0xFFFFFFFFu;
+}
+
+uint64_t col_facts_mask() {
+  const char* e = getenv("KYV_FACT_COLS");
+  return e && atoi(e) == 0 ? 0ull : ~0ull;
 }
 
 std::string format_path(const Ruleset& rs, const Batch& b, uint32_t tmpl, const uint16_t* idx, const uint32_t* key) {
diff --git a/kyverno_amd/csrc/capi.cpp b/kyverno_amd/csrc/capi.cpp
--- a/kyverno_amd/csrc/capi.cpp
+++ b/kyverno_amd/csrc/capi.cpp
@@ -341,6 +341,51 @@
     }
     if (out->order) for (size_t p = 0; p < n; p++) out->order[p] = p < x.order.size() ? x.order[p] : (uint32_t)p;
     const std::string js = wave_fact_bits_json(*x.rs);
+    out->bits_len = js.size();
+    if (out->bits) {
+      if (out->bits_cap < js.size() + 1) return fail(KYV_EINVAL, "buffer too small");
+      memcpy(out->bits, js.c_str(), js.size() + 1);
+    }
+    return KYV_OK;
+  } catch (std::exception& e) {
+    return fail(KYV_EINTERNAL, e.what());
+  }
+}
+
+static std::string col_fact_bits_json(const Ruleset& rs) {
+  std::vector<std::string> node_path(rs.trie.size());
+  std::function<void(uint32_t, const std::string&)> go = [&](uint32_t t, const std::string& path) {
+    const Ruleset::TrieNode& T = rs.trie[t];
+    node_path[t] = path;
+    const std::string sep = path.empty() ? "" : ",";
+    if (T.star != NONE) go(T.star, path + sep + "\"[*]\"");
+    for (const auto& kv : T.kids) {
+      std::string q = "\"";
+      for (unsigned char ch : rs.dict.strs[kv.first]) {
+        if (ch == '"' || ch == '\\') { q += '\\'; q += (char)ch; }
+        else if (ch < 0x20) { char b[8]; snprintf(b, sizeof b, "\\u%04x", ch); q += b; }
+        else q += (char)ch;
+      }
+      go(kv.second, path + sep + q + "\"");
+    }
+  };
+  if (!rs.trie.empty()) go(0, "");
+  std::string js = "{\"lists\":[";
+  for (size_t i = 0; i < rs.fact_lists.size(); i++) js += (i ? ",[" : "[") + node_path[rs.fact_lists[i]] + "]";
+  return js + "]}";
+}
+
+int kyv_batch_col_facts(const kyv_batch* b, kyv_col_facts_out* out) {
+  if (!b || !out) return fail(KYV_EINVAL, "null argument");
+  try {
+    const Batch& x = *b->b;
+    const size_t nw = (x.hdr.size() + 63) / 64;
+    if (out->rows && out->rows_cap < nw) return fail(KYV_EINVAL, "buffer too small");
+    if (out->rows) {
+      const uint64_t m = col_facts_mask();
+      for (size_t w = 0; w < nw; w++) out->rows[w] = (w < x.col_facts.size() ? x.col_facts[w].empty : 0ull) & m;
+    }
+    const std::string js = col_fact_bits_json(*x.rs);
     out->bits_len = js.size();
     if (out->bits) {
       if (out->bits_cap < js.size() + 1) return fail(KYV_EINVAL, "buffer too small");
diff --git a/kyverno_amd/csrc/compiler.cpp b/kyverno_amd/csrc/compiler.cpp
--- a/kyverno_amd/csrc/compiler.cpp
+++ b/kyverno_amd/csrc/compiler.cpp
@@ -2646,6 +2646,7 @@
   if (!getenv("KYV_PSS_NOCOLS"))
     for (auto& rd : rs.rules) tb.pss_rule(rd);
   assign_wave_facts(rs);
+  assign_col_facts(rs);
   assign_meta_classes(rs);
 }
 
@@ -2665,6 +2666,12 @@
     if (map_child) spaces.insert(rs.col_rowspace[rs.pn_self[pn]]);
   }
   for (uint32_t s2 : spaces) if (rs.fact_spaces.size() < FACT_BITS) rs.fact_spaces.push_back(s2);
+}
+
+void assign_col_facts(Ruleset& rs) {
+  rs.fact_lists.clear();
+  for (uint32_t t = 0; t < rs.trie.size() && rs.fact_lists.size() < COLFACT_BITS; t++)
+    if (rs.trie[t].star != NONE && rs.trie[t].col != NONE) rs.fact_lists.push_back(t);
 }
 
 void assign_meta_classes(Ruleset& rs) {
diff --git a/kyverno_amd/csrc/jit.cpp b/kyverno_amd/csrc/jit.cpp
--- a/kyverno_amd/csrc/jit.cpp
+++ b/kyverno_amd/csrc/jit.cpp
@@ -33,6 +33,15 @@
 int jit_jc_chains_mode() {
   const char* e = getenv("KYV_JC_PRELOAD");
   return e ? (atoi(e) != 0) : jit_meta_keys_on() ? 1 : 0;
+}
+
+int jit_col_facts_mode() {
+  for (const char* n : {"KYV_JC_PRELOAD", "KYV_META_KEYS"}) {
+    const char* e = getenv(n);
+    if (e && atoi(e) == 0) return 0;
+  }
+  const char* e = getenv("KYV_JIT_COLFACTS");
+  return e ? (atoi(e) & 1) : 1;
 }
 
 namespace {
@@ -67,11 +76,27 @@
   std::vector<uint32_t> node_mbase;
   std::vector<int8_t> meta_pos;
 
-  explicit Gen(const Ruleset& r, int meta_keys_mode = -1)
+  const int colfacts;
+  std::map<uint32_t, uint32_t> empty_bit;
+  std::string fact_row(uint32_t col, const std::string& rowx, const std::string& ce) const {
+    auto it = empty_bit.find(col);
+    if (it == empty_bit.end()) return rowx;
+    return "((" + ce + " >> " + std::to_string(it->second) + "u) & 1ull) ? NONE : " + rowx;
+  }
+
+  explicit Gen(const Ruleset& r, int meta_keys_mode = -1, int colfacts_mode = -1)
       : rs(r), meta_keys(meta_keys_mode < 0 ? jit_meta_keys_on() : meta_keys_mode != 0), emitted(r.pnodes.size(), 0), slot_meta(r.pnodes.size(), -1), wild_src(r.pentries.size()),
         slot(r.pentries.size(), -1), slot_alen(r.pnodes.size(), -1),
         slot_elen(r.pentries.size(), -1), scope_of(r.pnodes.size()), scoped(r.pnodes.size(), 0),
-        node_mbase(r.pnodes.size(), NONE), meta_pos(r.pnodes.size(), -1) {}
+        node_mbase(r.pnodes.size(), NONE), meta_pos(r.pnodes.size(), -1),
+        colfacts(colfacts_mode < 0 ? jit_col_facts_mode() : colfacts_mode) {
+    if (colfacts & 1)
+      for (size_t j = 0; j < rs.fact_lists.size() && j < COLFACT_BITS; j++) {
+        const Ruleset::TrieNode& T = rs.trie[rs.fact_lists[j]];
+        empty_bit[T.col] = (uint32_t)j;
+        if (T.lencol != NONE) empty_bit[T.lencol] = (uint32_t)j;
+      }
+  }
 
   void mark_paths(uint32_t pn, uint32_t mbase, uint32_t k0, uint32_t k1, uint32_t k2, uint32_t k3, int depth) {
     if (pn == NONE || pn >= rs.pnodes.size() || depth > 4) return;
@@ -169,14 +194,15 @@
     }
   }
   const std::vector<uint32_t>& scope_cols(uint32_t root) { scope(root); return scope_of[root]; }
-  std::string preload(uint32_t root, const std::string& name, const std::string& rowx, const char* rd = "jself(w, ") {
+  std::string preload(uint32_t root, const std::string& name, const std::string& rowx, const char* rd = "jself(w, ",
+                      const char* ce = "w.ce") {
     scope(root);
     const auto& L = scope_of[root];
     std::ostringstream o;
     o << "uint64_t " << name << "[" << std::max<size_t>(1, L.size()) << "];";
     for (size_t i = 0; i < L.size(); i++) {
       if (L[i] & MK_COL) { o << meta_load(L, i, name, rowx); continue; }
-      o << " " << name << "[" << i << "] = " << rd << u(L[i]) << ", " << rowx << ");";
+      o << " " << name << "[" << i << "] = " << rd << u(L[i]) << ", " << fact_row(L[i], rowx, ce) << ");";
     }
     return o.str();
   }
@@ -629,7 +655,20 @@
   uint32_t cur_etpos = NONE;
   std::unordered_map<uint64_t, std::string> progs;
 
-  CondGen(const Ruleset& r, int mode) : rs(r), chains(mode < 0 ? jit_jc_chains_mode() != 0 : mode != 0) {}
+  CondGen(const Ruleset& r, int mode, int colfacts_mode)
+      : rs(r), colfacts(colfacts_mode), chains(mode < 0 ? jit_jc_chains_mode() != 0 : mode != 0) {
+    if (colfacts & 1)
+      for (size_t j = 0; j < rs.fact_lists.size() && j < COLFACT_BITS; j++) empty_bit[rs.fact_lists[j]] = (uint32_t)j;
+  }
+  const int colfacts;
+  std::string rsig() const { return (colfacts & 1) ? "uint32_t r, const uint64_t ce, " : "uint32_t r, "; }
+  std::string rarg() const { return (colfacts & 1) ? "(v, R, r, ce, " : "(v, R, r, "; }
+  std::map<uint32_t, uint32_t> empty_bit;
+  std::string fact_row(uint32_t tpos, const std::string& row) const {
+    auto it = empty_bit.find(tpos);
+    if (it == empty_bit.end()) return row;
+    return "(((ce >> " + std::to_string(it->second) + "u) & 1ull) ? NONE : " + row + ")";
+  }
   static std::string u(uint32_t x) { return std::to_string(x) + "u"; }
   std::string fresh(const char* p) { return std::string(p) + std::to_string(uid++); }
 
@@ -653,7 +692,7 @@
     if (x.lz.empty()) return x;
     V y{fresh("vi"), fresh("vt"), fresh("va"), x.row, x.tpos, false, {}};
     out << "  uint32_t " << y.i << ", " << y.t << ", " << y.a << ";\n"
-        << "  if (" << x.row << " != NONE) jc_field_e(jc_col(v, " << u(tcol(x.tpos)) << ", " << x.row << "), &" << y.i << ", &"
+        << "  if (" << x.row << " != NONE) jc_field_e(jc_col(v, " << u(tcol(x.tpos)) << ", " << fact_row(x.tpos, x.row) << "), &" << y.i << ", &"
         << y.t << ", &" << y.a << ");\n"
         << "  else {\n    " << y.i << " = " << x.i << ";\n";
     for (uint32_t key : x.lz)
@@ -690,7 +729,7 @@
     const std::string cnt = fresh("cn"), aa = fresh("aa"), eb = fresh("eb"), j = fresh("j");
     const uint32_t st = tstar(x.tpos);
     out << "  { uint32_t " << cnt << " = 0u, " << aa << " = 0u, " << eb << " = NONE;\n"
-        << "  if (" << (x.key ? "false" : "jc_arr(v, R, " + x.i + ", " + x.t + ", " + x.a + ", " + x.row + ", " +
+        << "  if (" << (x.key ? "false" : "jc_arr(v, R, " + x.i + ", " + x.t + ", " + x.a + ", " + (tlen(x.tpos) == NONE ? x.row : fact_row(x.tpos, x.row)) + ", " +
                                               (tlen(x.tpos) == NONE ? std::string("NONE") : u(tlen(x.tpos))) + ", &" + cnt +
                                               ", &" + aa + ", &" + eb + ")")
         << ") {\n" << on_arr << (unroll ? "  KYV_JC_UNROLL\n" : "")
@@ -828,7 +867,7 @@
     std::ostringstream save;
     save.swap(out);
     out << "static __device__ __forceinline__ int " << name
-        << "(const View& v, const Node* R, uint32_t r, uint32_t ei, uint32_t et, uint32_t ea, uint32_t erow, uint32_t* L, "
+        << "(const View& v, const Node* R, " << rsig() << "uint32_t ei, uint32_t et, uint32_t ea, uint32_t erow, uint32_t* L, "
            "bool* lst, uint32_t* cur, uint32_t* ln, uint32_t* lit) {\n"
            "  *lst = false; *cur = NONE; *ln = 0u; *lit = NONE;\n";
     uint32_t i = 1, orlit = NONE;
@@ -890,7 +929,7 @@
     std::ostringstream save;
     save.swap(out);
     out << "static __device__ __forceinline__ int " << name
-        << "(const View& v, const Node* R, uint32_t r, uint32_t ei, uint32_t et, uint32_t ea, uint32_t erow, "
+        << "(const View& v, const Node* R, " << rsig() << "uint32_t ei, uint32_t et, uint32_t ea, uint32_t erow, "
            "bool* lst, uint32_t* cur, uint32_t* ln, uint32_t* lit, uint32_t* sm, uint32_t* sf) {\n"
            "  *lst = false; *cur = NONE; *ln = 0u; *lit = NONE; (void)sm; (void)sf;\n";
     V x = root == JR_OBJECT ? decl("0u", "T_UNK", "0u", "r", 0u, false) : decl("ei", "et", "ea", "erow", etpos, false);
@@ -948,7 +987,7 @@
     const std::string l = fresh("jl"), cc = fresh("jc"), n = fresh("jn"), t = fresh("jt"), s = fresh("js"), m = fresh("sm"),
                       fb = fresh("sf");
     out << "  bool " << l << "; uint32_t " << cc << ", " << n << ", " << t << ", " << m << " = 0u, " << fb << " = 0u;\n"
-        << "  const int " << s << " = " << f << "(v, R, r, ei, et, ea, erow, &" << l << ", &" << cc << ", &" << n << ", &" << t
+        << "  const int " << s << " = " << f << rarg() << "ei, et, ea, erow, &" << l << ", &" << cc << ", &" << n << ", &" << t
         << ", &" << m << ", &" << fb << ");\n"
         << "  if (" << s << " == JS_FB) return CR_FB;\n  if (" << s << " == JS_NOTFOUND) return CP_ERROR;\n"
         << "  if (" << l << ") {\n";
@@ -1023,7 +1062,7 @@
         const std::string f = operand_fn(o, etpos);
         const std::string l = fresh("jl"), c = fresh("jc"), n = fresh("jn"), t = fresh("jt"), s = fresh("js");
         out << "  bool " << l << "; uint32_t " << c << ", " << n << ", " << t << ";\n"
-            << "  const int " << s << " = " << f << "(v, R, r, ei, et, ea, erow, " << slot << ", &" << l << ", &" << c
+            << "  const int " << s << " = " << f << rarg() << "ei, et, ea, erow, " << slot << ", &" << l << ", &" << c
             << ", &" << n << ", &" << t << ");\n";
         if (check) out << "  if (" << s << " == JS_FB) return CR_FB;\n  if (" << s << " == JS_NOTFOUND) return CP_ERROR;\n";
         else out << "  (void)" << s << ";\n";
@@ -1118,7 +1157,7 @@
     const std::string b = out.str();
     out.swap(save);
     defs << "static __device__ __forceinline__ int " << name
-         << "(const View& v, const Node* R, uint32_t r, uint32_t ei, uint32_t et, uint32_t ea, uint32_t erow, uint32_t* L) {\n"
+         << "(const View& v, const Node* R, " << rsig() << "uint32_t ei, uint32_t et, uint32_t ea, uint32_t erow, uint32_t* L) {\n"
          << "  (void)ei; (void)et; (void)ea; (void)erow;\n"
          << b << "}\n";
     progs[key] = name;
@@ -1130,7 +1169,7 @@
     out << "  do {\n";
     if (FE->scope == 2) out << "  if (jc_type(R, " << e.i << ", " << e.t << ") != N_MAP) return ST_ERROR | ST_MARK_SCOPE;\n";
     out << "  bool err = false;\n";
-    const std::string args = "(v, R, r, " + e.i + ", " + e.t + ", " + e.a + ", " + e.row + ", L)";
+    const std::string args = rarg() + e.i + ", " + e.t + ", " + e.a + ", " + e.row + ", L)";
     if (FE->pre != NONE) {
       const std::string f = prog_fn(FE->pre, e.tpos);
       out << "  { const int c = " << f << args << ";\n"
@@ -1288,7 +1327,7 @@
     out << "  if (hnn >= (1u << COL_TYPE_SHIFT)) return ST_FALLBACK;  // no path columns for this resource\n"
         << "  const Node* R = v.nodes + hroot;\n"
         << "  const uint32_t ei = NONE, et = T_UNK, ea = 0u, erow = NONE;\n";
-    const std::string args = "(v, R, r, ei, et, ea, erow, L)";
+    const std::string args = rarg() + "ei, et, ea, erow, L)";
     if (rd.pre != NONE) {
       const std::string f = prog_fn(rd.pre, NONE);
       out << "  { const int c = " << f << args << ";\n"
@@ -1321,7 +1360,8 @@
     }
     const std::string b = out.str();
     out.swap(save);
-    defs << "static __device__ __forceinline__ uint8_t jr" << k << "(const View& v, uint32_t r, uint32_t hroot, uint32_t hnn, uint32_t* L) {\n" << b << "}\n";
+    defs << "static __device__ __forceinline__ uint8_t jr" << k << "(const View& v, uint32_t r, uint32_t hroot, uint32_t hnn, uint32_t* L) {\n"
+         << ((colfacts & 1) ? "  const uint64_t ce = jc_empty(v, r);  // the wave's empty-list facts\n  (void)ce;\n" : "") << b << "}\n";
   }
 };
 
@@ -1384,13 +1424,15 @@
 }
 
 std::string jit_source(const Ruleset& rs, std::vector<uint8_t>* jit_rules, std::vector<uint8_t>* jit_cond,
-                       std::vector<uint16_t>* jit_shape, int meta_keys, int jc_chains) {
-  Gen g(rs, meta_keys);
+                       std::vector<uint16_t>* jit_shape, int meta_keys, int jc_chains, int col_facts) {
+  Gen g(rs, meta_keys, col_facts);
+  const bool cf = (g.colfacts & 1) != 0;
+  const std::string ce_par = cf ? ", const uint64_t ce" : "", ce_arg = cf ? ", ce" : "", ce_set = cf ? "  w.ce = ce;\n" : "";
   jit_rules->assign(rs.rules.size(), 0);
   if (jit_shape) jit_shape->assign(rs.rules.size(), 0);
   if (jit_cond) jit_cond->assign(rs.rules.size(), 0);
   const size_t cap = getenv("KYV_JIT_MAX_RULES") ? (size_t)atol(getenv("KYV_JIT_MAX_RULES")) : 1024;
-  CondGen cg(rs, jc_chains);
+  CondGen cg(rs, jc_chains, g.colfacts);
   std::vector<uint32_t> crules;
   const bool cond_on = !getenv("KYV_JIT_COND") || atoi(getenv("KYV_JIT_COND")) != 0;
   for (size_t k = 0; k < rs.rules.size() && cond_on && crules.size() < cap; k++) {
@@ -1613,13 +1655,13 @@
       if (rep_of[r] == r)
       src << "static __device__ __forceinline__ void root" << r
           << "(const View& v, const Node* R, const ResHeader* hp, uint32_t row, uint32_t mbase, bool rootmap, bool walk,\n"
-             "    PatOut& out, const uint32_t am) {\n"
-             "  " << g.preload(r, "pc", "row", "jc_col(v, ") << "\n"
+             "    PatOut& out, const uint32_t am" << ce_par << ") {\n"
+             "  " << g.preload(r, "pc", "row", "jc_col(v, ", "ce") << "\n"
           << g.dyn_preload(dyn_of(r)) <<
              "  if (!walk) return;\n"
              "#ifdef KYV_EXP_JIT_PRELOAD\n  { uint64_t x = 0; for (auto q : pc) x ^= q; out.status = x == 0x123456789ull ? ST_FAIL : ST_PASS; return; }\n#endif\n"
           << g.dyn_decode(dyn_of(r)) <<
-             "  JW w{v, R, hp, 0ull, 0ull, Keys{NONE, NONE}, 0ull, mbase, (uint8_t)ST_NONE, am" << (dyn_of(r) != NONE ? ", dv" : "") << "};\n"
+             "  JW w{v, R, hp, 0ull, 0ull, Keys{NONE, NONE}, 0ull, mbase, (uint8_t)ST_NONE, am" << (dyn_of(r) != NONE ? ", dv" : "") << "};\n" << ce_set <<
              "  Ret r = p" << r << "(w, 0u, rootmap ? (uint32_t)N_MAP : T_UNK, 0u, row, pc);\n"
              "  jfinish(w, r, out);\n"
              "}\n";
@@ -1671,7 +1713,7 @@
         const auto& L = g.scope_of[r];
         src << "static __device__ __forceinline__ void rootc" << r << "_" << gi
             << "(const View& v, const Node* R, const ResHeader* hp, uint32_t row, uint32_t mbase, bool rootmap, bool walk,\n"
-               "    PatOut& out, const uint64_t* jcc, const uint32_t am) {\n"
+               "    PatOut& out, const uint64_t* jcc, const uint32_t am" << ce_par << ") {\n"
                "  const uint32_t lane = threadIdx.x & 63u;\n"
                "  (void)lane;\n"
                "  uint64_t pc[" << std::max<size_t>(1, L.size()) << "];";
@@ -1679,13 +1721,13 @@
           auto it = cslot.find(L[i]);
           if (it != cslot.end()) src << " pc[" << i << "] = jcc[" << it->second * 64u << "u + lane];";
           else if (L[i] & Gen::MK_COL) src << Gen::meta_load(L, i, "pc", "row");
-          else src << " pc[" << i << "] = jc_col(v, " << Gen::u(L[i]) << ", row);";
+          else src << " pc[" << i << "] = jc_col(v, " << Gen::u(L[i]) << ", " << g.fact_row(L[i], "row", "ce") << ");";
         }
         src << "\n"
             << g.dyn_preload(dyn_of(r)) <<
                "  if (!walk) return;\n"
             << g.dyn_decode(dyn_of(r)) <<
-               "  JW w{v, R, hp, 0ull, 0ull, Keys{NONE, NONE}, 0ull, mbase, (uint8_t)ST_NONE, am" << (dyn_of(r) != NONE ? ", dv" : "") << "};\n"
+               "  JW w{v, R, hp, 0ull, 0ull, Keys{NONE, NONE}, 0ull, mbase, (uint8_t)ST_NONE, am" << (dyn_of(r) != NONE ? ", dv" : "") << "};\n" << ce_set <<
                "  Ret r = p" << r << "(w, 0u, rootmap ? (uint32_t)N_MAP : T_UNK, 0u, row, pc);\n"
                "  jfinish(w, r, out);\n"
                "}\n";
@@ -1704,6 +1746,7 @@
     src << "struct JitWalker" << gi << " {\n"
            "  bool rootmap;\n"
            "  uint32_t am;\n"
+        << (cf ? "  uint64_t ce;  // the wave's empty-list facts (walk_chunks sets it)\n  static constexpr bool kColFacts = true;\n" : "") <<
            "  __device__ __forceinline__ void run(const View& v, uint32_t root, bool walk, const Node* R, const ResHeader* hp,\n"
            "                                     uint32_t row, const RuleDesc& rd, PatOut& out) {\n"
            "    out.status = ST_NONE; out.idx = 0; out.tmpl = NONE; out.key0 = NONE; out.key1 = NONE;\n"
@@ -1716,12 +1759,12 @@
     if (roots.size() <= 256) {
       for (auto& br : by_rep) {
         for (uint32_t r : br.second) src << "      case " << r << "u:";
-        src << " root" << br.first << "(v, R, hp, row, rd.meta_sites, rootmap, walk, out, am); break;\n";
+        src << " root" << br.first << "(v, R, hp, row, rd.meta_sites, rootmap, walk, out, am" << ce_arg << "); break;\n";
       }
     } else {
       uint32_t si = 0;
       for (auto& br : by_rep) {
-        src << "      case " << si++ << "u: root" << br.first << "(v, R, hp, row, rd.meta_sites, rootmap, walk, out, am); break;\n";
+        src << "      case " << si++ << "u: root" << br.first << "(v, R, hp, row, rd.meta_sites, rootmap, walk, out, am" << ce_arg << "); break;\n";
       }
     }
     src << "      default: if (walk) out.status = ST_FALLBACK;\n"
@@ -1748,6 +1791,7 @@
              "    const uint32_t row = r < v.nres ? r : NONE;\n"
              "    const bool rootmap = (hflags & RF_ROOT_MAP) != 0;\n"
              "    const uint32_t am = wave_maps(v, w);\n"
+          << (cf ? "    const uint64_t ce = wave_cols(v, w).empty;\n    (void)ce;\n" : "") <<
              "    (void)lane; (void)hp; (void)rootmap; (void)hnn; (void)am;\n";
       if (!conds.empty()) src << "    __shared__ uint32_t jl[" << jc_lds << "];\n";
       if (ncslots) {
@@ -1768,7 +1812,7 @@
           src << "    if (";
           size_t j = 0;
           for (const auto& e : wm) src << (j++ ? " | " : "") << "(jsl[" << e.first << "] & " << e.second << "u)";
-          src << ") jcc[" << cslot[cu.first] * 64u << "u + lane] = jc_col(v, " << Gen::u(cu.first) << ", row);\n";
+          src << ") jcc[" << cslot[cu.first] * 64u << "u + lane] = jc_col(v, " << Gen::u(cu.first) << ", " << g.fact_row(cu.first, "row", "ce") << ");\n";
         }
       }
       for (size_t j = 0; j < part.size(); j++) {
@@ -1793,10 +1837,10 @@
         const uint32_t root = rule_roots[i].second[a];
         if (ncslots)
           src << "            case " << a << "u: rootc" << rep_of[root] << "_" << gi << "(vl, R, hp, row, " << Gen::u(rd.meta_sites)
-              << ", rootmap, wk, po, jcc, am); break;\n";
+              << ", rootmap, wk, po, jcc, am" << ce_arg << "); break;\n";
         else
           src << "            case " << a << "u: root" << rep_of[root] << "(vl, R, hp, row, " << Gen::u(rd.meta_sites)
-              << ", rootmap, wk, po, am); break;\n";
+              << ", rootmap, wk, po, am" << ce_arg << "); break;\n";
       }
       src << "            default: break;\n"
              "          }\n"
@@ -1860,8 +1904,9 @@
   }
   if (!shape_list.empty()) {
     src << "struct JitShapes {\n"
+        << (cf ? "  static constexpr bool kColFacts = true;  // run() takes the wave's empty-list facts (walk_shapes)\n" : "") <<
            "  __device__ __forceinline__ void run(const View& v, const ShapeOut& so, uint32_t r, bool active, uint32_t hflags,\n"
-           "                                     uint32_t hroot, uint32_t cls, const uint32_t am) {\n"
+           "                                     uint32_t hroot, uint32_t cls, const uint32_t am" << ce_par << ") {\n"
            "    const Node* R = v.nodes + hroot;\n"
            "    const ResHeader* hp = v.hdr + r;\n"
            "    const uint32_t row = r < v.nres ? r : NONE;\n"
@@ -1876,7 +1921,7 @@
              "        ShapeSink sink{so.rec + (size_t)" << S << " * v.nres + r};\n"
              "        uint8_t st = pair_walk_alts(true, 1u, gated && !magic, r, 0u, sink, [&](uint32_t, bool wk, PatOut& po) {\n"
              "          po.status = ST_NONE; po.idx = 0; po.tmpl = NONE; po.key0 = NONE; po.key1 = NONE;\n"
-             "          root" << shape_list[si].first << "(v, R, hp, row, " << Gen::u(shape_list[si].second) << ", rootmap, wk, po, am);\n"
+             "          root" << shape_list[si].first << "(v, R, hp, row, " << Gen::u(shape_list[si].second) << ", rootmap, wk, po, am" << ce_arg << ");\n"
              "        });\n"
              "        if (magic) st = ST_FALLBACK;\n"
              "        if (gated) { so.st[(size_t)" << S << " * v.nres + r] = st; KYV_ACCT_ADD(1, 1); }\n"
@@ -1945,7 +1990,7 @@
     src << "extern \"C\" __global__ void __launch_bounds__(64) __attribute__((amdgpu_waves_per_eu("
         << (gwpe[gi] == -2 ? "KYV_JIT_WPE_LIGHT" : "KYV_JIT_WPE") << ")))\n"
            "kyv_jit_walk_" << gi << "(const kyv::View* __restrict__ vp, kyv::DevOut o, kyv::WorkLists wl, kyv::ChunkMap cm) {\n"
-           "  kyv::JitWalker" << gi << " wk{false, 0u};\n"
+           "  kyv::JitWalker" << gi << " wk{false, 0u" << (cf ? ", 0ull" : "") << "};\n"
            "  kyv::walk_chunks(*vp, o, wl, cm, wk);\n"
            "}\n";
   src << "#ifndef KYV_JIT_WPE_FUSED\n#define KYV_JIT_WPE_FUSED 8\n#endif\n"
diff --git a/kyverno_amd/csrc/kyv_engine.hip b/kyverno_amd/csrc/kyv_engine.hip
--- a/kyverno_amd/csrc/kyv_engine.hip
+++ b/kyverno_amd/csrc/kyv_engine.hip
@@ -363,6 +363,7 @@
   const MetaKeyRow* view_meta = nullptr;
   const HotHdr* view_hot = nullptr;
   uint32_t view_fact_and = 0;
+  uint64_t view_col_and = 0;
   uint8_t* shape_st = nullptr;
   FailRec* shape_rec = nullptr;
   uint32_t* shape_gate = nullptr;
@@ -401,7 +402,7 @@
   DeviceResults* out = nullptr;
   uint8_t* base = nullptr;
   size_t bytes = 0;
-  size_t o_nodes, o_hdr, o_hot, o_facts, o_faux, o_soff, o_slen, o_sflags, o_sdur, o_sqty, o_sf64, o_heap, o_nsloff, o_nslkv, o_gate,
+  size_t o_nodes, o_hdr, o_hot, o_facts, o_cfacts, o_faux, o_soff, o_slen, o_sflags, o_sdur, o_sqty, o_sf64, o_heap, o_nsloff, o_nslkv, o_gate,
       o_colv, o_coloff, o_pe, o_supper = SIZE_MAX, o_srx = SIZE_MAX;
   uint32_t* gmask = nullptr;
   uint32_t gmask_words = 0;
@@ -456,6 +457,7 @@
   d->o_hdr = p.add(b.hdr);
   d->o_hot = p.add(b.hot);
   d->o_facts = p.add(b.facts);
+  d->o_cfacts = p.add(b.col_facts);
   d->o_faux = p.add(b.faux);
   d->o_soff = p.add(b.str_off);
   d->o_slen = p.add(b.str_len);
@@ -494,6 +496,7 @@
     v.hdr = (const ResHeader*)(bbase + db->o_hdr);
     v.hot = hot_plane_on() && b.hot.size() == b.hdr.size() ? (const HotHdr*)(bbase + db->o_hot) : nullptr;
     v.facts = b.facts.size() == (b.hdr.size() + 63) / 64 ? (const WaveFacts*)(bbase + db->o_facts) : nullptr;
+    v.col_facts = b.col_facts.size() == (b.hdr.size() + 63) / 64 ? (const ColFacts*)(bbase + db->o_cfacts) : nullptr;
     v.faux = (const FloatAux*)(bbase + db->o_faux);
     v.str_off = (const uint32_t*)(bbase + db->o_soff);
     v.str_len = (const uint32_t*)(bbase + db->o_slen);
@@ -518,6 +521,7 @@
     v.nodes = b.nodes.data(); v.hdr = b.hdr.data(); v.faux = b.faux.data();
     v.hot = hot_plane_on() && b.hot.size() == b.hdr.size() ? b.hot.data() : nullptr;
     v.facts = b.facts.size() == (b.hdr.size() + 63) / 64 ? b.facts.data() : nullptr;
+    v.col_facts = b.col_facts.size() == (b.hdr.size() + 63) / 64 ? b.col_facts.data() : nullptr;
     v.str_off = b.str_off.data(); v.str_len = b.str_len.data(); v.str_flags = b.str_flags.data();
     v.str_dur = b.str_dur.data(); v.str_qty = b.str_qty.data(); v.str_f64 = b.str_f64.data();
     v.heap = b.heap.data(); v.nsl_off = b.nsl_off.data(); v.nsl_kv = b.nsl_kv.data();
@@ -530,6 +534,7 @@
   v.gate_words = b.gate_words;
   v.nres = (uint32_t)b.hdr.size();
   v.fact_and = wave_maps_mask();
+  v.col_and = col_facts_mask();
   v.nrules = (uint32_t)rs.rules.size();
   if (dr) {
     v.rules = (const RuleDesc*)(rbase + dr->o_rules);
@@ -1006,7 +1011,9 @@
     try {
       rs.jit_meta_keys = jit_meta_keys_on() && !rs.meta_classes.empty();
       rs.jit_jc_chains = jit_jc_chains_mode();
-      std::string src = jit_source(rs, &rs.jit_rules, &rs.jit_cond, &rs.jit_shape, rs.jit_meta_keys ? 1 : 0, rs.jit_jc_chains);
+      rs.jit_col_facts = jit_col_facts_mode();
+      std::string src = jit_source(rs, &rs.jit_rules, &rs.jit_cond, &rs.jit_shape, rs.jit_meta_keys ? 1 : 0, rs.jit_jc_chains,
+                                   rs.jit_col_facts);
       rs.jit_nshapes = 0;
       for (auto x : rs.jit_shape) rs.jit_nshapes = std::max<uint32_t>(rs.jit_nshapes, x);
       bool any = false;
@@ -1076,7 +1083,8 @@
   std::lock_guard<std::mutex> lk(g_jit_mu);
   if (rs.jit_code_acct.empty()) {
     std::vector<uint8_t> jr, jc;
-    rs.jit_code_acct = jit_compile(jit_source(rs, &jr, &jc, nullptr, rs.jit_meta_keys ? 1 : 0, rs.jit_jc_chains), nullptr, true);
+    rs.jit_code_acct = jit_compile(jit_source(rs, &jr, &jc, nullptr, rs.jit_meta_keys ? 1 : 0, rs.jit_jc_chains, rs.jit_col_facts),
+                                   nullptr, true);
   }
   HIP_OK(hipModuleLoadData(&dr->amod, rs.jit_code_acct.data()));
   dr->afns.resize(dr->jfns.size());
@@ -1851,7 +1859,7 @@
     stream_get(&d.stream, &d.e0, &d.e1);
     HIP_OK(dmalloc(&d.view, sizeof(View)));
     HIP_OK(hipMemcpy(d.view, &v, sizeof(View), hipMemcpyHostToDevice));
-    d.view_hot = v.hot; d.view_fact_and = v.fact_and;
+    d.view_hot = v.hot; d.view_fact_and = v.fact_and; d.view_col_and = v.col_and;
     d.wl.nwaves = (uint32_t)((nres + WAVE - 1) / WAVE);
     const size_t nwv = d.wl.nwaves;
     const size_t budget = slice_budget();
@@ -1920,9 +1928,9 @@
     db->out = dd;
   }
   DeviceResults& d = *db->out;
-  if (d.view_hot != v.hot || d.view_fact_and != v.fact_and) {
+  if (d.view_hot != v.hot || d.view_fact_and != v.fact_and || d.view_col_and != v.col_and) {
     HIP_OK(hipMemcpy(d.view, &v, sizeof(View), hipMemcpyHostToDevice));
-    d.view_hot = v.hot; d.view_fact_and = v.fact_and;
+    d.view_hot = v.hot; d.view_fact_and = v.fact_and; d.view_col_and = v.col_and;
   }
   hipStream_t stream = d.stream;
   const bool use_jit = jit_mode == JIT_ON || (jit_mode == JIT_AUTO && nres >= JIT_AUTO_MIN_RESOURCES);
diff --git a/kyverno_amd/csrc/kyv_eval.h b/kyverno_amd/csrc/kyv_eval.h
--- a/kyverno_amd/csrc/kyv_eval.h
+++ b/kyverno_amd/csrc/kyv_eval.h
@@ -78,6 +78,8 @@
   uint32_t nres;
   const WaveFacts* facts;
   uint32_t fact_and;
+  const ColFacts* col_facts;
+  uint64_t col_and;
   const FloatAux* faux;
   const uint32_t* str_off;
   const uint32_t* str_len;
diff --git a/kyverno_amd/csrc/kyv_fused.h b/kyverno_amd/csrc/kyv_fused.h
--- a/kyverno_amd/csrc/kyv_fused.h
+++ b/kyverno_amd/csrc/kyv_fused.h
@@ -64,7 +64,8 @@
       cls = h.kclass;
     }
     (void)hnn;
-    f.run(v, so, r, active, hflags, hroot, cls, wave_maps(v, w));
+    if constexpr (takes_col_facts<Shapes>::value) f.run(v, so, r, active, hflags, hroot, cls, wave_maps(v, w), wave_cols(v, w).empty);
+    else f.run(v, so, r, active, hflags, hroot, cls, wave_maps(v, w));
   }
 }
 
diff --git a/kyverno_amd/csrc/kyv_host.h b/kyverno_amd/csrc/kyv_host.h
--- a/kyverno_amd/csrc/kyv_host.h
+++ b/kyverno_amd/csrc/kyv_host.h
@@ -126,10 +126,12 @@
   std::vector<uint32_t> pn_len;
   std::vector<uint32_t> pe_len;
   std::vector<uint32_t> fact_spaces;
+  std::vector<uint32_t> fact_lists;
   std::vector<MetaClass> meta_classes;
   std::vector<int8_t> meta_class_of;
   bool jit_meta_keys = false;
   int jit_jc_chains = 0;
+  int jit_col_facts = 0;
   bool jit_tried = false;
   std::vector<uint8_t> jit_rules;
   std::vector<uint8_t> jit_cond;
@@ -174,6 +176,7 @@
   bulk_vector<uint64_t> colv;
   std::vector<uint32_t> col_off, rs_rows;
   std::vector<WaveFacts> facts;
+  std::vector<ColFacts> col_facts;
   std::vector<void*> dev;
   ~Batch();
 };
@@ -221,17 +224,21 @@
 void derive_strings(Batch& b, size_t from, int threads);
 void build_path_trie(Ruleset& rs);
 void assign_wave_facts(Ruleset& rs);
+void assign_col_facts(Ruleset& rs);
 void assign_meta_classes(Ruleset& rs);
 bool jit_meta_keys_on();
 std::vector<MetaKeyRow> meta_key_rows_host(const Ruleset& rs, const Batch& b);
 std::vector<MetaKeyRow> meta_key_rows_device(const Batch& b, int device);
 size_t meta_key_plane_bytes(const Batch& b);
 uint32_t wave_maps_mask();
+uint64_t col_facts_mask();
+int jit_col_facts_mode();
 void assign_glob_masks(Ruleset& rs);
 void assign_cond_sets(Ruleset& rs);
 int jit_jc_chains_mode();
 std::string jit_source(const Ruleset& rs, std::vector<uint8_t>* jit_rules, std::vector<uint8_t>* jit_cond = nullptr,
-                       std::vector<uint16_t>* jit_shape = nullptr, int meta_keys = -1, int jc_chains = -1);
+                       std::vector<uint16_t>* jit_shape = nullptr, int meta_keys = -1, int jc_chains = -1,
+                       int col_facts = -1);
 bool jit_shape_eligible(const Ruleset& rs, uint32_t k);
 constexpr uint32_t JIT_MAX_SHAPES = 64;
 std::vector<char> jit_compile(const std::string& src, double* seconds, bool acct = false);
diff --git a/kyverno_amd/csrc/kyv_jcond.h b/kyverno_amd/csrc/kyv_jcond.h
--- a/kyverno_amd/csrc/kyv_jcond.h
+++ b/kyverno_amd/csrc/kyv_jcond.h
@@ -12,6 +12,9 @@
   KYV_ACCT_ADDK(2u, 0, 8);
   const uint32_t off = sld32(v.col_off + col);
   return gcol(v.colv, off, row);
+}
+__device__ __forceinline__ uint64_t jc_empty(const View& v, uint32_t r) {
+  return wave_cols(v, __builtin_amdgcn_readfirstlane(r >> 6)).empty;
 }
 __device__ __forceinline__ kyv_u32x4 jc_meta(const View& v, uint32_t cls, uint32_t row) {
   if (row == NONE) return kyv_u32x4{0u, NONE, NONE, NONE};
diff --git a/kyverno_amd/csrc/kyv_layout.h b/kyverno_amd/csrc/kyv_layout.h
--- a/kyverno_amd/csrc/kyv_layout.h
+++ b/kyverno_amd/csrc/kyv_layout.h
@@ -105,6 +105,12 @@
   uint32_t maps;
 };
 static_assert(sizeof(WaveFacts) == 4, "wave facts row size");
+
+constexpr uint32_t COLFACT_BITS = 64;
+struct ColFacts {
+  uint64_t empty;
+};
+static_assert(sizeof(ColFacts) == 8, "column facts row size");
 
 enum MatchMode : uint8_t { MM_NONE = 0, MM_PLAIN = 1, MM_ANY = 2, MM_ALL = 3,
                            MM_EXC_ALL = 4 };
diff --git a/kyverno_amd/csrc/kyv_wave.h b/kyverno_amd/csrc/kyv_wave.h
--- a/kyverno_amd/csrc/kyv_wave.h
+++ b/kyverno_amd/csrc/kyv_wave.h
@@ -69,6 +69,16 @@
 __device__ __forceinline__ uint32_t wave_maps(const View& v, uint32_t w) {
   return v.facts ? (sld32(&v.facts[w].maps) & v.fact_and) : 0u;
 }
+__device__ __forceinline__ ColFacts wave_cols(const View& v, uint32_t w) {
+  ColFacts f{0ull};
+  if (v.col_facts) {
+    f = sld(v.col_facts + w);
+    f.empty &= v.col_and;
+  }
+  return f;
+}
+template <class W, class = void> struct takes_col_facts { static constexpr bool value = false; };
+template <class W> struct takes_col_facts<W, decltype((void)W::kColFacts)> { static constexpr bool value = W::kColFacts; };
 __device__ __forceinline__ uint32_t ghot_flags(const View& v, const ResHeader* hp) {
   KYV_ACCT_ADD(0, 4);
   return v.hot ? gld32(&v.hot[hp - v.hdr].flags) : gld32(&hp->flags);
@@ -657,6 +667,7 @@
   uint8_t ost;
   uint32_t am;
   const Val* dyn = nullptr;
+  uint64_t ce = 0ull;
 };
 template <uint8_t OP, uint8_t FLAGS, uint8_t GLOB, uint32_t GI1 = 0>
 __device__ __forceinline__ bool jatom(const View& v, const Val& x, uint32_t pat, uint32_t lit, int64_t dur, int64_t qlo,
@@ -851,6 +862,7 @@
     }
     wk.rootmap = (it.x & ITEM_ROOT_MAP) != 0;
     wk.am = wave_maps(v, w);
+    if constexpr (takes_col_facts<Walker>::value) wk.ce = wave_cols(v, w).empty;
     const uint32_t alts = rd.kind == RK_PATTERN ? 1u : min(rd.nalts, (uint32_t)MAX_ALTS);
     WaveSink sink{o.stage + sld32(o.rbase + (k - o.rule_lo)) + (size_t)w * WAVE * alts, 0u, rd.uses_meta != 0};
     uint8_t st = pair_walk(v, rd, active, r, k, v.nodes + it.y, wk, sink);
diff --git a/kyverno_amd/engine.py b/kyverno_amd/engine.py
--- a/kyverno_amd/engine.py
+++ b/kyverno_amd/engine.py
@@ -113,6 +113,16 @@
         shape = json.loads(paths.value.decode())
         return dict(json.loads(bits.value.decode()), facts=facts, hot=hot, order=order, shape_keys=keys,
                     shape_paths=shape["paths"], shape_bits=shape["bits"], shape_ordered=shape["ordered"])
+
+    def col_facts(self):
+        L = K.lib()
+        o = K.ColFactsOut()
+        K.check(L.kyv_batch_col_facts(self.h, ctypes.byref(o)))
+        rows = np.zeros((self.n + 63) // 64, dtype=np.uint64)
+        bits = ctypes.create_string_buffer(o.bits_len + 1)
+        o = K.ColFactsOut(rows.ctypes.data, rows.size, ctypes.addressof(bits), o.bits_len + 1, 0)
+        K.check(L.kyv_batch_col_facts(self.h, ctypes.byref(o)))
+        return dict(json.loads(bits.value.decode()), rows=rows)
 
     def meta_keys(self, device=None):
         L = K.lib()
```

Result: faster. 160.6 billion (median of 6 runs) (+3.7%).
